# Shao-Group/aletsch

Measured on AMD Instinct MI355X. Metric: bundles/sec, higher is better.
Workload: dtype f64

## Files before the change

aletsch_amd/csrc/decomp_device.h:

```cpp
#pragma once
#include "decomp_common.h"
#ifdef ALD_EMU
#include <cstdio>
#include <cstdlib>
namespace ald { inline int32_t *emu_fail_line = nullptr; }
#endif

#ifndef ALD_CLASS_ID
#error "compile with -DALD_CLASS_ID=<0..13> (one translation unit per size class)"
#endif
#if defined(__HIP__) || defined(__clang__)
  #define ALD_UNROLL _Pragma("unroll")
#else
  #define ALD_UNROLL _Pragma("GCC unroll 16")
#endif
#define ALD_CAT2(a, b) a##b
#define ALD_CAT(a, b) ALD_CAT2(a, b)
#ifdef ALD_RAW_VARIANT
#define ALD_CLASS_NS ALD_CAT(ald_r, ALD_CLASS_ID)
#else
#define ALD_CLASS_NS ALD_CAT(ald_c, ALD_CLASS_ID)
#endif

namespace ALD_CLASS_NS {
using namespace ald;
#ifdef ALD_EMU_COUNT
static long g_cnt_router = 0, g_cnt_unsweep = 0, g_cnt_star[34] = {0}, g_cnt_rdeg[34] = {0}, g_cnt_build = 0, g_cnt_pre[3] = {0}, g_cnt_fix[8] = {0}, g_cnt_fix_declined = 0, g_cnt_x22[3] = {0}, g_cnt_x22s[5] = {0};
struct CntPrinter { ~CntPrinter() { if(g_cnt_unsweep) { fprintf(stderr, "[emu-count] class %d: unsplittable sweeps %ld router runs %ld (of which reach build(): %ld; prepared at level 0/1/2: %ld %ld %ld)\n", ALD_CLASS_ID, g_cnt_unsweep, g_cnt_router, g_cnt_build, g_cnt_pre[0], g_cnt_pre[1], g_cnt_pre[2]);
    fprintf(stderr, "[emu-count]   stars by fan size:"); for(int i = 0; i < 34; i++) if(g_cnt_star[i]) fprintf(stderr, " %d:%ld", i, g_cnt_star[i]); fprintf(stderr, "\n");
    fprintf(stderr, "[emu-count]   stars through the fixed-size form:"); for(int i = 0; i < 8; i++) if(g_cnt_fix[i]) fprintf(stderr, " %d:%ld", i, g_cnt_fix[i]); fprintf(stderr, " declined:%ld\n", g_cnt_fix_declined);
    fprintf(stderr, "[emu-count]   extends: %ld through the fixed 2x2 form: %ld declined: %ld\n", g_cnt_x22[2], g_cnt_x22[0], g_cnt_x22[1]);
    fprintf(stderr, "[emu-count]   fixed 2x2 form: strand to i' from o*: %ld to o' from i*: %ld to z from i*: %ld to z from o*: %ld insert_between acted: %ld\n", g_cnt_x22s[0], g_cnt_x22s[1], g_cnt_x22s[2], g_cnt_x22s[3], g_cnt_x22s[4]);
    fprintf(stderr, "[emu-count]   router runs by degree:"); for(int i = 0; i < 34; i++) if(g_cnt_rdeg[i]) fprintf(stderr, " %d:%ld", i, g_cnt_rdeg[i]); fprintf(stderr, "\n"); } } }; static CntPrinter g_cnt_printer;
#endif

enum { MAXV = ClassDims<ALD_CLASS_ID>::MAXV, MAXE = ClassDims<ALD_CLASS_ID>::MAXE, NW = ClassDims<ALD_CLASS_ID>::NW };
typedef uint16_t IDX;
static constexpr IDX NIL = (IDX)0xFFFF;
#if ALD_CLASS_ID == ALD_HUGE_CLASS
typedef uint32_t EID;
enum { EID_LIMIT = 0x7FFFFFF0 };
#else
typedef uint16_t EID;
enum { EID_LIMIT = 0xFFF0 };
#endif
typedef ColdLayoutT<MAXV, MAXE, NW, 0> CL;
#ifndef ALD_KEEP
  #define ALD_KEEP (ALD_CLASS_ID >= ALD_FIRST_GLOBAL_CLASS ? 1 : 0)
#endif
#ifndef ALD_KEEP_TRIV
  #define ALD_KEEP_TRIV ALD_KEEP
#endif
enum { LP = 16, ARENA_I = 96, ARENA_D = 48, SCR_I = 4 * LP + ARENA_I, SCR_D = 2 * LP + ARENA_D };

struct Hot {
    struct alignas(8) Link { IDX es, et, inx, onx; };
    struct alignas(16) EdgeHot { double w; Link lk; };
    EdgeHot  ed[MAXE];
    EID      eid[MAXE];
    struct alignas(8) VertexHot { IDX in_head, out_head, in_deg, out_deg; };
    VertexHot vx[MAXV];
    uint8_t  nz[MAXV];
    uint8_t  hflag[MAXE];
};
struct HotCtx {
    ALD_GLOBAL uint8_t *cold;
    ALD_GLOBAL const KernelArgs *args;
    double   ro_ratio;
    int32_t  ro_type, ro_degree, ro_npairs, tmp0;
    int32_t  ev_all;
#if ALD_KEEP
    uint32_t ev_dirty[(MAXV + 31) / 32];
  #if ALD_KEEP_TRIV
    int32_t  tv_all; uint32_t tv_dirty[(MAXV + 31) / 32];
  #endif
#endif
    int32_t  g, V0, gstrand;
    int32_t  nv, next_id, slot_hw, free_head, free_cnt, status, any_strand, hs_dirty, n_paths, n_iters, n_trace;
    uint32_t sp_used, hl_used; int32_t hl_n;
    int32_t  s_next;
    double   p_min_w, p_min_cov, p_ratio[8]; int32_t p_max_exons, p_trace_cap;
    int32_t  pw_lds, park_lds;
    int32_t  sinkp, special_linked;
    int32_t  maybe_triv;
    int32_t  maybe_broken;
    double   sw_best_r, sw_hit_r; int32_t sw_best_v, sw_hit, sw_vend, sw_dom_base; uint32_t sw_need_lo, sw_need_hi;
    int32_t  sw_ncand;
    int32_t  scr_i[SCR_I]; double scr_d[SCR_D];
#ifdef ALD_PROF
    unsigned long long prof[32];
#endif
};

#if ALD_CLASS_ID >= ALD_FIRST_GLOBAL_CLASS
#define ALD_MERGED_WALKS 1
#endif
#if defined(ALD_EMU)
static thread_local Hot g_H;
static thread_local HotCtx g_HC;
#define H g_H
#define HC g_HC
#elif ALD_CLASS_ID >= ALD_FIRST_GLOBAL_CLASS
__shared__ ALD_GLOBAL Hot *g_Hp;
__shared__ HotCtx g_HC;
#define H (*g_Hp)
#define HC g_HC
#define ALD_HOT_IN_SLAB 1
#else
__shared__ Hot g_H;
__shared__ HotCtx g_HC;
#define H g_H
#define HC g_HC
#endif

struct ColdVertex { double vw; int32_t lpos, rpos, vtype, v2v, memo, pad_; };
struct alignas(64) ColdEdge {
    double   med, eabd, econf, s0abd;
    uint64_t mask[NW];
    int32_t  mei, ecount, s0id;
    uint32_t sp_off, sp_len;
    uint8_t  estrand;
};
static_assert(sizeof(ColdVertex) == CL::VX_BYTES && sizeof(ColdEdge) == CL::ED_BYTES, "slab layout out of sync");
struct Cold {
    ALD_GLOBAL ColdVertex *vx;
    ALD_GLOBAL ColdEdge *ed;
    ALD_GLOBAL int32_t *sp_id; ALD_GLOBAL double *sp_abd;
    ALD_GLOBAL int32_t *hl, *hl_off, *hl_len, *hl_capk, *hl_cnt;
    ALD_GLOBAL int32_t *wi; ALD_GLOBAL double *wd;
    ALD_GLOBAL unsigned long long *po;
    static constexpr int32_t po_cap = CL::PO_CAP;
    static constexpr uint32_t sp_cap = CL::SP_CAP, hl_cap = CL::HL_CAP;
    static constexpr int32_t hl_maxlists = CL::HL_MAXLISTS, w_cap = CL::W_CAP;
};
ALD_INL Cold cold_view()
{
    ALD_GLOBAL uint8_t *b = HC.cold; Cold C;
    C.vx = (ALD_GLOBAL ColdVertex*)(b + CL::o_vx); C.ed = (ALD_GLOBAL ColdEdge*)(b + CL::o_ed);
    C.sp_id = (ALD_GLOBAL int32_t*)(b + CL::o_spid); C.sp_abd = (ALD_GLOBAL double*)(b + CL::o_spabd);
    C.hl = (ALD_GLOBAL int32_t*)(b + CL::o_hl); C.hl_off = (ALD_GLOBAL int32_t*)(b + CL::o_hloff); C.hl_len = (ALD_GLOBAL int32_t*)(b + CL::o_hllen);
    C.hl_capk = (ALD_GLOBAL int32_t*)(b + CL::o_hlcapk); C.hl_cnt = (ALD_GLOBAL int32_t*)(b + CL::o_hlcnt);
    C.wi = (ALD_GLOBAL int32_t*)(b + CL::o_wi); C.wd = (ALD_GLOBAL double*)(b + CL::o_wd);
    C.po = (ALD_GLOBAL unsigned long long*)(b + CL::o_po);
    return C;
}
#define COLD const Cold C = cold_view()

#if defined(ALD_PROF) && !defined(ALD_EMU)
  #define PROF_DECL unsigned long long prof_t_ = __builtin_readcyclecounter()
  #define PROF_ADD(k) do { unsigned long long t1_ = __builtin_readcyclecounter(); if(lane_id() == 0) HC.prof[k] += t1_ - prof_t_; prof_t_ = t1_; } while(0)
  #define PROF_RESET() (prof_t_ = __builtin_readcyclecounter())
#else
  #define PROF_DECL do {} while(0)
  #define PROF_ADD(k) do {} while(0)
  #define PROF_RESET() do {} while(0)
#endif
enum { PF_LOAD = 0, PF_BROKEN, PF_TRIV_EVAL, PF_TRIV_MUT, PF_SMALL_EVAL, PF_SMALL_MUT, PF_UNSPLIT, PF_COLLECT0, PF_G_BALANCE, PF_G_DP, PF_G_SPLITMERGE, PF_G_COLLECT, PF_FINISH,
       PF_T_BALANCE, PF_T_PAIRS, PF_T_SETUP, PF_T_MERGE_LOAD, PF_T_MERGE_ADD, PF_T_MERGE_ISECT, PF_T_MERGE_MASK, PF_T_MERGE_SUMS, PF_T_MERGE_KILL, PF_T_HS, PF_T_TAIL,
       PF_S5_DUP, PF_S5_BODY, PF_S5_RELINK, PF_S6_WALK, PF_S6_LINK, PF_S7, PF_SM_KILL, PF_SM_REEVAL, PF_COUNT };

ALD_INL void fail_(int st, int line)
{
#ifdef ALD_EMU
    if(HC.status == 0 && getenv("ALD_EMU_VERBOSE")) fprintf(stderr, "[emu] graph %d: status %d raised at decomp_device.h:%d\n", HC.g, st, line);
    if(HC.status == 0 && ald::emu_fail_line) ald::emu_fail_line[HC.g] = line;
#endif
    if(HC.status == 0) HC.status = st;
}
#define fail(st) fail_((st), __LINE__)
#define ALD_UNLIKELY(x) __builtin_expect(!!(x), 0)
ALD_FN void trace_emit(int code, int a, int b, double v)
{
    int cap = HC.p_trace_cap;
    ALD_GLOBAL const KernelArgs *A = HC.args;
    int k = HC.n_trace++;
    if(k < cap) { int64_t o = (int64_t)HC.g * cap + k; A->out.trace_codes[3 * o] = code; A->out.trace_codes[3 * o + 1] = a; A->out.trace_codes[3 * o + 2] = b; A->out.trace_vals[o] = v; }
}
#ifdef ALD_PROF
ALD_INL bool tracing_u() { return false; }
ALD_INL bool tracing() { return false; }
#else
ALD_INL bool tracing_u() { return uni(HC.p_trace_cap) > 0; }
ALD_INL bool tracing() { return HC.p_trace_cap > 0; }
#endif
ALD_INL void trace(int code, int a, int b, double v) { HC.n_iters++; if(tracing()) trace_emit(code, a, b, v); }
#ifndef ALD_NO_SEXT_LINKS
ALD_INL int slot_or_neg(IDX h) { return MAXE < 32768 ? (int)(int16_t)h : (h == NIL ? -1 : (int)h); }
#else
ALD_INL int slot_or_neg(IDX h) { return h == NIL ? -1 : (int)h; }
#endif
ALD_INL int u_first_in(int v) { return uni(slot_or_neg(H.vx[v].in_head)); }
ALD_INL int u_first_out(int v) { return uni(slot_or_neg(H.vx[v].out_head)); }
ALD_INL int u_next_in(int e) { return uni(slot_or_neg(H.ed[e].lk.inx)); }
ALD_INL int u_next_out(int e) { return uni(slot_or_neg(H.ed[e].lk.onx)); }
ALD_INL int first_in(int v) { return slot_or_neg(H.vx[v].in_head); }
ALD_INL int first_out(int v) { return slot_or_neg(H.vx[v].out_head); }
ALD_INL int next_in(int e) { return slot_or_neg(H.ed[e].lk.inx); }
ALD_INL int next_out(int e) { return slot_or_neg(H.ed[e].lk.onx); }
ALD_INL double in_weights(int v) { double w = 0; for(int e = first_in(v); e >= 0; e = next_in(e)) w += H.ed[e].w; return w; }
ALD_INL double out_weights(int v) { double w = 0; for(int e = first_out(v); e >= 0; e = next_out(e)) w += H.ed[e].w; return w; }

ALD_INL uint32_t tkey(uint32_t p) { return (int)p == HC.sinkp ? 0xFFFFu : p; }
ALD_INL int vlog(int p) { return p < HC.V0 - 1 ? p : (p == HC.sinkp ? HC.nv - 1 : p - 1); }
ALD_INL uint64_t lkw(int e) { return uni(*(const uint64_t*)&H.ed[e].lk); }
ALD_INL int lk_next(uint32_t f) { return slot_or_neg((IDX)f); }
ALD_INL void ev_mark(int v)
{
#if ALD_KEEP
  #ifdef ALD_EMU
    HC.ev_dirty[v >> 5] |= 1u << (v & 31);
    #if ALD_KEEP_TRIV
    HC.tv_dirty[v >> 5] |= 1u << (v & 31);
    #endif
  #else
    __hip_atomic_fetch_or(&HC.ev_dirty[v >> 5], 1u << (v & 31), __ATOMIC_RELAXED, __HIP_MEMORY_SCOPE_WAVEFRONT);
    #if ALD_KEEP_TRIV
    __hip_atomic_fetch_or(&HC.tv_dirty[v >> 5], 1u << (v & 31), __ATOMIC_RELAXED, __HIP_MEMORY_SCOPE_WAVEFRONT);
    #endif
  #endif
#else
    (void)v;
#endif
}
ALD_INL void star_tail_sync() { if(ALD_KEEP) wsync_mem(); else wsync(); }
ALD_INL void ev_mark_all()
{
#if ALD_KEEP
    HC.ev_all = 1;
    #if ALD_KEEP_TRIV
    HC.tv_all = 1;
    #endif
#endif
}
ALD_INL void ev_clear_marks(int vend)
{
#if ALD_KEEP
    const int words = (vend + 31) / 32;
    HC.ev_all = 0;
    for(int base = 0; base < words; base += ALD_WAVE) { const int k = base + lane_id(); HC.ev_dirty[k < words ? k : words - 1] = 0; }
#else
    (void)vend;
#endif
}
ALD_INL void tv_clear_marks(int nv_now)
{
#if ALD_KEEP && ALD_KEEP_TRIV
    const int words = (nv_now + 31) / 32;
    HC.tv_all = 0;
    for(int base = 0; base < words; base += ALD_WAVE) { const int k = base + lane_id(); HC.tv_dirty[k < words ? k : words - 1] = 0; }
#else
    (void)nv_now;
#endif
}
ALD_INL void ev_degree(int v, int before, int after, bool out)
{
#if ALD_KEEP
    ev_mark(v);
    if((before <= 1) == (after <= 1)) return;
    if(!HC.special_linked && (out ? v == 0 : v == HC.sinkp)) { ev_mark_all(); return; }
    int guard = MAXE;
    for(int e = out ? slot_or_neg(H.vx[v].out_head) : slot_or_neg(H.vx[v].in_head); e >= 0 && guard-- > 0; e = out ? slot_or_neg(H.ed[e].lk.onx) : slot_or_neg(H.ed[e].lk.inx))
        ev_mark(out ? (int)H.ed[e].lk.et : (int)H.ed[e].lk.es);
#else
    (void)v; (void)before; (void)after; (void)out;
#endif
}
ALD_INL void link_in(int v, int e)
{
    v = uni(v); e = uni(e);
    if(v == uni(HC.sinkp) && !uni(HC.special_linked)) { const int dg = uni((int)H.vx[v].in_deg); H.vx[v].in_deg = (IDX)(dg + 1); ev_degree(v, dg, dg + 1, false); return; }
    const uint32_t ks = uni(H.ed[e].lk.es), kid = uni(H.eid[e]);
    IDX *pp = &H.vx[v].in_head; IDX cur = *pp;
    for(int guard = MAXE; uni(cur != NIL) && guard > 0; guard--) {
        const uint64_t w = *(const uint64_t*)&H.ed[cur].lk; const uint32_t cs = (uint32_t)(w & 0xFFFF);
        bool stop = cs > ks; if(uni(cs == ks)) stop = H.eid[cur] > kid;
        if(uni(stop)) break;
        pp = &H.ed[cur].lk.inx; cur = (IDX)((w >> 32) & 0xFFFF);
    }
    H.ed[e].lk.inx = cur; *pp = (IDX)e;
    { const int dg = uni((int)H.vx[v].in_deg); H.vx[v].in_deg = (IDX)(dg + 1); ev_degree(v, dg, dg + 1, false); }
}
ALD_INL void link_out(int v, int e)
{
    v = uni(v); e = uni(e);
    if(v == 0 && !uni(HC.special_linked)) { const int dg = uni((int)H.vx[v].out_deg); H.vx[v].out_deg = (IDX)(dg + 1); ev_degree(v, dg, dg + 1, true); return; }
    const uint32_t sk = (uint32_t)uni(HC.sinkp);
    uint32_t kt = uni(H.ed[e].lk.et); const uint32_t kid = uni(H.eid[e]);
    if(kt == sk) kt = 0xFFFFu;
    IDX *pp = &H.vx[v].out_head; IDX cur = *pp;
    for(int guard = MAXE; uni(cur != NIL) && guard > 0; guard--) {
        const uint64_t w = *(const uint64_t*)&H.ed[cur].lk; uint32_t ct = (uint32_t)((w >> 16) & 0xFFFF); if(ct == sk) ct = 0xFFFFu;
        bool stop = ct > kt; if(uni(ct == kt)) stop = H.eid[cur] > kid;
        if(uni(stop)) break;
        pp = &H.ed[cur].lk.onx; cur = (IDX)(w >> 48);
    }
    H.ed[e].lk.onx = cur; *pp = (IDX)e;
    { const int dg = uni((int)H.vx[v].out_deg); H.vx[v].out_deg = (IDX)(dg + 1); ev_degree(v, dg, dg + 1, true); }
}
ALD_INL void link_out_after(int v, int e, int hint)
{
    v = uni(v); e = uni(e); hint = uni(hint);
    if(v == 0 && !uni(HC.special_linked)) { const int dg = uni((int)H.vx[v].out_deg); H.vx[v].out_deg = (IDX)(dg + 1); ev_degree(v, dg, dg + 1, true); return; }
    const uint32_t sk = (uint32_t)uni(HC.sinkp);
    uint32_t kt = uni(H.ed[e].lk.et); const uint32_t kid = uni(H.eid[e]);
    if(kt == sk) kt = 0xFFFFu;
    IDX *pp = &H.ed[hint].lk.onx; IDX cur = *pp;
    for(int guard = MAXE; uni(cur != NIL) && guard > 0; guard--) {
        const uint64_t w = *(const uint64_t*)&H.ed[cur].lk; uint32_t ct = (uint32_t)((w >> 16) & 0xFFFF); if(ct == sk) ct = 0xFFFFu;
        bool stop = ct > kt; if(uni(ct == kt)) stop = H.eid[cur] > kid;
        if(uni(stop)) break;
        pp = &H.ed[cur].lk.onx; cur = (IDX)(w >> 48);
    }
    H.ed[e].lk.onx = cur; *pp = (IDX)e;
    { const int dg = uni((int)H.vx[v].out_deg); H.vx[v].out_deg = (IDX)(dg + 1); ev_degree(v, dg, dg + 1, true); }
}
ALD_INL void unlink_in(int v, int e)
{
    v = uni(v); e = uni(e);
    if(v == uni(HC.sinkp) && !uni(HC.special_linked)) { const int dg = uni((int)H.vx[v].in_deg); H.vx[v].in_deg = (IDX)(dg - 1); ev_degree(v, dg, dg - 1, false); return; }
    IDX *pp = &H.vx[v].in_head; IDX cur = *pp; int guard = MAXE;
    while(uni((int)cur != e && cur != NIL) && guard-- > 0) { pp = &H.ed[cur].lk.inx; cur = *pp; }
    if(ALD_UNLIKELY(uni((int)cur != e))) { fail(ALD_ST_INVARIANT + ALD_INV_OTHER); return; }
    *pp = H.ed[e].lk.inx;
    { int dg = (int)uni(H.vx[v].in_deg) - 1; H.vx[v].in_deg = (IDX)dg; ev_degree(v, dg + 1, dg, false); if(dg <= 1) { HC.maybe_triv = 1; if(dg == 0) HC.maybe_broken = 1; } }
}
ALD_INL void unlink_out(int v, int e)
{
    v = uni(v); e = uni(e);
    if(v == 0 && !uni(HC.special_linked)) { const int dg = uni((int)H.vx[v].out_deg); H.vx[v].out_deg = (IDX)(dg - 1); ev_degree(v, dg, dg - 1, true); return; }
    IDX *pp = &H.vx[v].out_head; IDX cur = *pp; int guard = MAXE;
    while(uni((int)cur != e && cur != NIL) && guard-- > 0) { pp = &H.ed[cur].lk.onx; cur = *pp; }
    if(ALD_UNLIKELY(uni((int)cur != e))) { fail(ALD_ST_INVARIANT + ALD_INV_OTHER); return; }
    *pp = H.ed[e].lk.onx;
    { int dg = (int)uni(H.vx[v].out_deg) - 1; H.vx[v].out_deg = (IDX)dg; ev_degree(v, dg + 1, dg, true); if(dg <= 1) { HC.maybe_triv = 1; if(dg == 0) HC.maybe_broken = 1; } }
}
ALD_INL void relink_in(int v, int e, uint32_t ks)
{
    v = uni(v); e = uni(e);
    ev_mark(v);
    if(v == uni(HC.sinkp) && !uni(HC.special_linked)) return;
    int last = -1, pe = -1, ip = -1; bool seen = false, placed = false;
    int guard = MAXE;
    for(int cur = u_first_in(v); cur >= 0 && guard-- > 0; ) {
        uint64_t w = lkw(cur); int nx = lk_next((uint32_t)((w >> 32) & 0xFFFF));
        if(cur == e) { pe = last; seen = true; if(placed) break; }
        else { if(!placed && (uint32_t)(w & 0xFFFF) > ks) { ip = last; placed = true; if(seen) break; } last = cur; }
        cur = nx;
    }
    if(ALD_UNLIKELY(!seen)) { fail(ALD_ST_INVARIANT + ALD_INV_OTHER); return; }
    if(!placed) ip = last;
    if(ip == pe) return;
    IDX nxe = uni(H.ed[e].lk.inx);
    if(pe < 0) H.vx[v].in_head = nxe; else H.ed[pe].lk.inx = nxe;
    if(ip < 0) { H.ed[e].lk.inx = uni(H.vx[v].in_head); H.vx[v].in_head = (IDX)e; } else { H.ed[e].lk.inx = uni(H.ed[ip].lk.inx); H.ed[ip].lk.inx = (IDX)e; }
}
ALD_INL void relink_out(int v, int e, uint32_t kt)
{
    v = uni(v); e = uni(e);
    ev_mark(v);
    if(v == 0 && !uni(HC.special_linked)) return;
    const uint32_t sk = (uint32_t)uni(HC.sinkp);
    int last = -1, pe = -1, ip = -1; bool seen = false, placed = false;
    int guard = MAXE;
    for(int cur = u_first_out(v); cur >= 0 && guard-- > 0; ) {
        uint64_t w = lkw(cur); int nx = lk_next((uint32_t)(w >> 48));
        if(cur == e) { pe = last; seen = true; if(placed) break; }
        else { uint32_t ct = (uint32_t)((w >> 16) & 0xFFFF); if(ct == sk) ct = 0xFFFFu; if(!placed && ct > kt) { ip = last; placed = true; if(seen) break; } last = cur; }
        cur = nx;
    }
    if(ALD_UNLIKELY(!seen)) { fail(ALD_ST_INVARIANT + ALD_INV_OTHER); return; }
    if(!placed) ip = last;
    if(ip == pe) return;
    IDX nxe = uni(H.ed[e].lk.onx);
    if(pe < 0) H.vx[v].out_head = nxe; else H.ed[pe].lk.onx = nxe;
    if(ip < 0) { H.ed[e].lk.onx = uni(H.vx[v].out_head); H.vx[v].out_head = (IDX)e; } else { H.ed[e].lk.onx = uni(H.ed[ip].lk.onx); H.ed[ip].lk.onx = (IDX)e; }
}
ALD_INL void relink_in_lane(int v, int e, uint32_t ks)
{
    ev_mark(v);
    if(v == HC.sinkp && !HC.special_linked) return;
    int last = -1, pe = -1, ip = -1; bool seen = false, placed = false;
    int guard = MAXE;
    for(int cur = first_in(v); cur >= 0 && guard-- > 0; ) {
        const uint64_t w = *(const uint64_t*)&H.ed[cur].lk; const int nx = lk_next((uint32_t)((w >> 32) & 0xFFFF));
        if(cur == e) { pe = last; seen = true; if(placed) break; }
        else { if(!placed && (uint32_t)(w & 0xFFFF) > ks) { ip = last; placed = true; if(seen) break; } last = cur; }
        cur = nx;
    }
    if(ALD_UNLIKELY(!seen)) { fail(ALD_ST_INVARIANT + ALD_INV_OTHER); return; }
    if(!placed) ip = last;
    if(ip == pe) return;
    const IDX nxe = H.ed[e].lk.inx;
    if(pe < 0) H.vx[v].in_head = nxe; else H.ed[pe].lk.inx = nxe;
    if(ip < 0) { H.ed[e].lk.inx = H.vx[v].in_head; H.vx[v].in_head = (IDX)e; } else { H.ed[e].lk.inx = H.ed[ip].lk.inx; H.ed[ip].lk.inx = (IDX)e; }
}
ALD_INL void relink_out_lane(int v, int e, uint32_t kt)
{
    ev_mark(v);
    if(v == 0 && !HC.special_linked) return;
    const uint32_t sk = (uint32_t)HC.sinkp;
    int last = -1, pe = -1, ip = -1; bool seen = false, placed = false;
    int guard = MAXE;
    for(int cur = first_out(v); cur >= 0 && guard-- > 0; ) {
        const uint64_t w = *(const uint64_t*)&H.ed[cur].lk; const int nx = lk_next((uint32_t)(w >> 48));
        if(cur == e) { pe = last; seen = true; if(placed) break; }
        else { uint32_t ct = (uint32_t)((w >> 16) & 0xFFFF); if(ct == sk) ct = 0xFFFFu; if(!placed && ct > kt) { ip = last; placed = true; if(seen) break; } last = cur; }
        cur = nx;
    }
    if(ALD_UNLIKELY(!seen)) { fail(ALD_ST_INVARIANT + ALD_INV_OTHER); return; }
    if(!placed) ip = last;
    if(ip == pe) return;
    const IDX nxe = H.ed[e].lk.onx;
    if(pe < 0) H.vx[v].out_head = nxe; else H.ed[pe].lk.onx = nxe;
    if(ip < 0) { H.ed[e].lk.onx = H.vx[v].out_head; H.vx[v].out_head = (IDX)e; } else { H.ed[e].lk.onx = H.ed[ip].lk.onx; H.ed[ip].lk.onx = (IDX)e; }
}
ALD_INL void clear_vertex(int x)
{
    ev_mark(x);
#if defined(ALD_EMU)
    H.vx[x].in_head = NIL; H.vx[x].out_head = NIL; H.vx[x].in_deg = 0; H.vx[x].out_deg = 0; H.nz[x] = 0;
#else
    unsigned lo = 0xFFFFFFFFu, hi = 0u;
    asm volatile("" : "+v"(lo), "+v"(hi));
    static_assert(sizeof(Hot::VertexHot) == 8 && NIL == 0xFFFF, "vertex record layout");
    union { uint64_t u; Hot::VertexHot v; } z; z.u = ((uint64_t)hi << 32) | lo;
    H.vx[x] = z.v;
    H.nz[x] = 0;
#endif
}
ALD_INL int free_slots() { return uni(HC.free_cnt) + (MAXE - uni(HC.slot_hw)); }
ALD_INL int add_edge_i(int s, int t)
{
    s = uni(s); t = uni(t);
    int e; int fh = uni(HC.free_head), hw = uni(HC.slot_hw);
    if(fh >= 0) { e = fh; IDX nx = uni(H.ed[e].lk.onx); HC.free_head = nx == NIL ? -1 : (int)nx; HC.free_cnt--; }
    else if(hw < MAXE) { e = hw; HC.slot_hw = hw + 1; }
    else { fail(ALD_ST_CAPACITY); return -1; }
    int id = uni(HC.next_id); HC.next_id = id + 1;
    if(ALD_UNLIKELY(id >= EID_LIMIT)) { fail(ALD_ST_CAPACITY); return -1; }
    H.ed[e].lk.es = (IDX)s; H.ed[e].lk.et = (IDX)t; H.eid[e] = (EID)id; H.hflag[e] = 0; H.ed[e].w = 0;
    link_out(s, e); link_in(t, e);
    return e;
}
ALD_INL void kill_edge_i(int e)
{
    e = uni(e);
    unlink_out(uni(H.ed[e].lk.es), e); unlink_in(uni(H.ed[e].lk.et), e);
    H.ed[e].lk.es = NIL;
    { int fh = uni(HC.free_head); H.ed[e].lk.onx = fh < 0 ? NIL : (IDX)fh; HC.free_head = e; HC.free_cnt = uni(HC.free_cnt) + 1; }
}
ALD_INL void kill_edge_wave(int e)
{
    e = uni(e);
    const uint64_t w = *(const uint64_t*)&H.ed[e].lk;
    const bool special = HC.special_linked != 0; const int sinkp = HC.sinkp;
    for(int side = lane_id(); side < 2; side += ALD_WAVE) {
        const bool out = (side == 0);
        const int v = out ? (int)(w & 0xFFFF) : (int)((w >> 16) & 0xFFFF);
        const IDX nxe = out ? (IDX)(w >> 48) : (IDX)((w >> 32) & 0xFFFF);
        const bool counted = !special && (out ? v == 0 : v == sinkp);
        IDX *deg = out ? &H.vx[v].out_deg : &H.vx[v].in_deg;
        if(!counted) {
            IDX *pp = out ? &H.vx[v].out_head : &H.vx[v].in_head; IDX cur = *pp; int guard = MAXE;
            while((int)cur != e && cur != NIL && guard-- > 0) { pp = out ? &H.ed[cur].lk.onx : &H.ed[cur].lk.inx; cur = *pp; }
            if(ALD_UNLIKELY((int)cur != e)) { fail(ALD_ST_INVARIANT + ALD_INV_OTHER); continue; }
            *pp = nxe;
        }
        const int dg = (int)*deg - 1; *deg = (IDX)dg;
        ev_degree(v, dg + 1, dg, out);
        if(!counted && dg <= 1) { HC.maybe_triv = 1; if(dg == 0) HC.maybe_broken = 1; }
    }
    wsync();
    if(lane_id() == 0) {
        H.ed[e].lk.es = NIL;
        const int fh = uni(HC.free_head); H.ed[e].lk.onx = fh < 0 ? NIL : (IDX)fh; HC.free_head = e; HC.free_cnt = uni(HC.free_cnt) + 1;
    }
}
ALD_FN int add_edge(int s, int t) { return add_edge_i(uni(s), uni(t)); }
ALD_FN void kill_edge(int e) { kill_edge_i(uni(e)); }
ALD_FN void move_edge(int e, int x, int y)
{
    e = uni(e); x = uni(x); y = uni(y);
    unlink_out(uni(H.ed[e].lk.es), e); unlink_in(uni(H.ed[e].lk.et), e);
    H.ed[e].lk.es = (IDX)x; H.ed[e].lk.et = (IDX)y;
    link_out(x, e); link_in(y, e);
}

ALD_INL void strand_degree(int v, int vs[6])
{
    COLD;
    for(int k = 0; k < 6; k++) vs[k] = 0;
    for(int e = first_in(v); e >= 0; e = next_in(e)) vs[C.ed[e].estrand]++;
    for(int e = first_out(v); e >= 0; e = next_out(e)) vs[C.ed[e].estrand + 3]++;
}
ALD_INL bool mixed_strand_vertex(int v)
{
    if(!HC.any_strand) return false;
    int vs[6]; strand_degree(v, vs);
    return (vs[1] + vs[4] >= 1) && (vs[2] + vs[5] >= 1);
}
ALD_INL void borrow_edge_strand(const Cold &C, int e1, int e2) { int s2 = C.ed[e2].estrand; if(s2 == 0) return; C.ed[e1].estrand = (uint8_t)s2; }

ALD_FN bool intersect_samples(int e1, int e2, int z)
{
    e1 = uni(e1); e2 = uni(e2); z = uni(z);
    COLD;
    const uint32_t n1 = uni(C.ed[e1].sp_len), n2 = uni(C.ed[e2].sp_len);
    if(n1 == 1 && n2 == 1) {
        int a = uni(C.ed[e1].s0id), b = uni(C.ed[e2].s0id); double x = uni(C.ed[e1].s0abd), y = uni(C.ed[e2].s0abd);
        if(a == b) { double c = (y < x) ? y : x; C.ed[z].sp_off = 0; C.ed[z].sp_len = 1; C.ed[z].ecount = 1; C.ed[z].eabd = 0.0 + c; C.ed[z].s0id = a; C.ed[z].s0abd = c; }
        else { C.ed[z].sp_off = 0; C.ed[z].sp_len = 0; C.ed[z].ecount = 0; C.ed[z].eabd = 0; C.ed[z].s0id = 0; C.ed[z].s0abd = 0; }
        return true;
    }
    const uint32_t o1 = uni(C.ed[e1].sp_off), o2 = uni(C.ed[e2].sp_off);
    const int i1 = uni(C.ed[e1].s0id), i2 = uni(C.ed[e2].s0id); const double a1 = uni(C.ed[e1].s0abd), a2 = uni(C.ed[e2].s0abd);
    const uint32_t need = n1 < n2 ? n1 : n2;
    const uint32_t o = HC.sp_used;
    if(ALD_UNLIKELY(o + need > C.sp_cap)) { fail(ALD_ST_CAPACITY); return false; }
    uint32_t i = 0, j = 0, k = 0; double abd = 0; int first_id = 0; double first_abd = 0;
    while(i < n1 && j < n2) {
        int a = n1 == 1 ? i1 : uni(C.sp_id[o1 + i]), b = n2 == 1 ? i2 : uni(C.sp_id[o2 + j]);
        if(a < b) i++; else if(b < a) j++;
        else { double x = n1 == 1 ? a1 : uni(C.sp_abd[o1 + i]), y = n2 == 1 ? a2 : uni(C.sp_abd[o2 + j]); double c = (y < x) ? y : x;
               C.sp_id[o + k] = a; C.sp_abd[o + k] = c; abd += c; if(k == 0) { first_id = a; first_abd = c; } k++; i++; j++; }
    }
    C.ed[z].sp_len = k; C.ed[z].ecount = (int32_t)k; C.ed[z].eabd = abd; C.ed[z].s0id = first_id; C.ed[z].s0abd = first_abd;
    if(k >= 2) { C.ed[z].sp_off = o; HC.sp_used = o + k; } else C.ed[z].sp_off = 0;
    return true;
}
ALD_FN double common_abd(int e1, int e2)
{
    e1 = uni(e1); e2 = uni(e2);
    COLD;
    const uint32_t o1 = uni(C.ed[e1].sp_off), n1 = uni(C.ed[e1].sp_len), o2 = uni(C.ed[e2].sp_off), n2 = uni(C.ed[e2].sp_len);
    const int i1 = uni(C.ed[e1].s0id), i2 = uni(C.ed[e2].s0id); const double a1 = uni(C.ed[e1].s0abd), a2 = uni(C.ed[e2].s0abd);
    uint32_t i = 0, j = 0; double c = 0;
    while(i < n1 && j < n2) {
        int a = n1 == 1 ? i1 : uni(C.sp_id[o1 + i]), b = n2 == 1 ? i2 : uni(C.sp_id[o2 + j]);
        if(a < b) i++; else if(b < a) j++;
        else { double x = n1 == 1 ? a1 : uni(C.sp_abd[o1 + i]), y = n2 == 1 ? a2 : uni(C.sp_abd[o2 + j]); double mn = (y < x) ? y : x, mx = (x < y) ? y : x; c += 0.99 * mn + 0.01 * mx; i++; j++; }
    }
    return c;
}

ALD_FN void hs_refresh_flags()
{
    if(!HC.hs_dirty) return;
    HC.maybe_triv = 1; ev_mark_all();
    COLD;
    for(int e = 0; e < HC.slot_hw; e++) H.hflag[e] = 0;
    int nl = HC.hl_n;
    for(int k = 0; k < nl; k++) {
        ALD_GLOBAL int32_t *v = C.hl + uni(C.hl_off[k]); int n = uni(C.hl_len[k]);
        for(int i = 0; i < n; i++) {
            int e = v[i]; if(e < 0) continue;
            uint8_t f = HF_OCC;
            if(i >= 1 && v[i - 1] != -1) f |= HF_LEXT;
            if(i + 1 < n && v[i + 1] != -1) f |= HF_REXT;
            H.hflag[e] |= f;
        }
    }
    HC.hs_dirty = 0;
}
ALD_FN void hs_remove_lists(int e)
{
    e = uni(e);
    int nl = HC.hl_n;
    COLD;
    for(int k = 0; k < nl; k++) { ALD_GLOBAL int32_t *v = C.hl + uni(C.hl_off[k]); int n = uni(C.hl_len[k]); for(int i = 0; i < n; i++) if(v[i] == e) { v[i] = -1; HC.hs_dirty = 1; } }
}
ALD_FN void hs_replace1_lists(int x, int e)
{
    x = uni(x); e = uni(e);
    int nl = HC.hl_n;
    COLD;
    for(int k = 0; k < nl; k++) { ALD_GLOBAL int32_t *v = C.hl + uni(C.hl_off[k]); int n = uni(C.hl_len[k]); for(int i = 0; i < n; i++) if(v[i] == x) { v[i] = e; HC.hs_dirty = 1; } }
}
ALD_FN void hs_replace2_lists(int x, int y, int e)
{
    x = uni(x); y = uni(y); e = uni(e);
    int nl = HC.hl_n;
    COLD;
    for(int k = 0; k < nl; k++) {
        ALD_GLOBAL int32_t *v = C.hl + uni(C.hl_off[k]); int n = uni(C.hl_len[k]); int w = 0;
        for(int i = 0; i < n; i++) {
            if(i + 1 < n && v[i] == x && v[i + 1] == y) { v[w++] = e; i++; HC.hs_dirty = 1; }
            else v[w++] = v[i];
        }
        C.hl_len[k] = w;
    }
}
ALD_FN void hs_insert_between_lists(int x, int y, int e)
{
    x = uni(x); y = uni(y); e = uni(e);
    int nl = HC.hl_n;
    COLD;
    for(int k = 0; k < nl; k++) {
        int n = uni(C.hl_len[k]); ALD_GLOBAL int32_t *v = C.hl + uni(C.hl_off[k]);
        int cnt = 0;
        for(int i = 0; i + 1 < n; i++) if(v[i] == x && v[i + 1] == y) cnt++;
        if(cnt == 0) continue;
        if(n + cnt > uni(C.hl_capk[k])) {
            uint32_t ncap = (uint32_t)(n + cnt) * 2u + 4u, o = HC.hl_used;
            if(ALD_UNLIKELY(o + ncap > C.hl_cap)) { fail(ALD_ST_CAPACITY); return; }
            for(int i = 0; i < n; i++) C.hl[o + i] = v[i];
            HC.hl_used = o + ncap; C.hl_off[k] = (int32_t)o; C.hl_capk[k] = (int32_t)ncap; v = C.hl + o;
        }
        int w = n + cnt - 1;
        for(int i = n - 1; i >= 0; i--) {
            v[w--] = v[i];
            if(i >= 1 && v[i - 1] == x && v[i] == y) v[w--] = e;
        }
        C.hl_len[k] = n + cnt; HC.hs_dirty = 1;
    }
}
ALD_INL void hs_remove(int e) { if(uni(HC.hl_n) != 0) hs_remove_lists(e); }
ALD_INL void hs_replace1(int x, int e) { if(uni(HC.hl_n) != 0) hs_replace1_lists(x, e); }
ALD_INL void hs_replace2(int x, int y, int e) { if(uni(HC.hl_n) != 0) hs_replace2_lists(x, y, e); }
ALD_INL void hs_insert_between(int x, int y, int e) { if(uni(HC.hl_n) != 0) hs_insert_between_lists(x, y, e); }
ALD_FN bool hs_dominate(int e, int side)
{
    e = uni(e); side = uni(side);
    COLD;
    int nl = HC.hl_n;
    ALD_GLOBAL int32_t *x1 = C.wi, *x2 = C.wi + C.w_cap / 4; int n1 = 0, n2 = 0; const int cap = C.w_cap / 8;
    for(int k = 0; k < nl; k++) {
        ALD_GLOBAL int32_t *v = C.hl + uni(C.hl_off[k]); int n = uni(C.hl_len[k]);
        if(side == 2) {
            for(int i = 0; i + 1 < n; i++) {
                if(v[i] != e) continue;
                if(v[i + 1] == -1) continue;
                int a = v[i + 1], b = (i + 2 < n) ? v[i + 2] : -1;
                if(i == 0 || v[i - 1] == -1) { if(n1 < cap) { x1[2 * n1] = a; x1[2 * n1 + 1] = b; n1++; } else fail(ALD_ST_CAPACITY); }
                else { if(n2 + 2 <= cap) { x2[2 * n2] = a; x2[2 * n2 + 1] = -1; n2++; if(i + 2 < n) { x2[2 * n2] = a; x2[2 * n2 + 1] = b; n2++; } } else fail(ALD_ST_CAPACITY); }
            }
        } else {
            for(int i = 1; i < n; i++) {
                if(v[i] != e) continue;
                if(v[i - 1] == -1) continue;
                int a = v[i - 1], b = (i - 2 >= 0) ? v[i - 2] : -1;
                if(i == n - 1 || v[i + 1] == -1) { if(n1 < cap) { x1[2 * n1] = a; x1[2 * n1 + 1] = b; n1++; } else fail(ALD_ST_CAPACITY); }
                else { if(n2 + 2 <= cap) { x2[2 * n2] = a; x2[2 * n2 + 1] = -1; n2++; if(i - 2 >= 0) { x2[2 * n2] = a; x2[2 * n2 + 1] = b; n2++; } } else fail(ALD_ST_CAPACITY); }
            }
        }
    }
    for(int i = 0; i < n1; i++) { bool f = false; for(int j = 0; j < n2 && !f; j++) f = (x2[2 * j] == x1[2 * i] && x2[2 * j + 1] == x1[2 * i + 1]); if(!f) return false; }
    return true;
}

ALD_FN int split_edge(int ei, double w)
{
    ei = uni(ei); w = uni(w);
    if(ALD_UNLIKELY(!(w >= HC.p_min_w - kSMIN))) { fail(ALD_ST_INVARIANT + ALD_INV_WEIGHT); return -1; }
    double ww = uni(H.ed[ei].w);
    if(fabs(ww - w) <= kSMIN) return ei;
    int s = uni(H.ed[ei].lk.es), t = uni(H.ed[ei].lk.et);
    int p2 = add_edge(s, t);
    if(p2 < 0) return -1;
    COLD;
    double www = ww - w;
    double mw = HC.p_min_w;
    if(www <= mw) www = mw;
    H.ed[ei].w = www; H.ed[p2].w = w;
    C.ed[p2].estrand = uni(C.ed[ei].estrand); C.ed[p2].ecount = uni(C.ed[ei].ecount); C.ed[p2].eabd = uni(C.ed[ei].eabd); C.ed[p2].econf = uni(C.ed[ei].econf);
    C.ed[p2].sp_off = uni(C.ed[ei].sp_off); C.ed[p2].sp_len = uni(C.ed[ei].sp_len); C.ed[p2].s0id = uni(C.ed[ei].s0id); C.ed[p2].s0abd = uni(C.ed[ei].s0abd);
    for(int k = 0; k < NW; k++) C.ed[p2].mask[k] = uni(C.ed[ei].mask[k]);
    C.ed[p2].mei = uni(C.ed[ei].mei); C.ed[p2].med = uni(C.ed[ei].med) * w / ww;
    return p2;
}
ALD_INL int merge_adjacent_edges_i(int x, int y, double ww)
{
    const double mw = HC.p_min_w;
    if(ALD_UNLIKELY(!(ww >= mw - kSMIN))) { fail(ALD_ST_INVARIANT + ALD_INV_WEIGHT); return -1; }
    if(x < 0 || y < 0) return -1;
    if(H.ed[x].lk.et != uni(H.ed[y].lk.es)) { int t = x; x = y; y = t; }
    const int xs = uni(H.ed[x].lk.es), xt = uni(H.ed[x].lk.et), yt = uni(H.ed[y].lk.et);
    if((int)uni(H.ed[y].lk.es) != xt) return -1;
    PROF_DECL;
    COLD;
    const double wx = uni(H.ed[x].w), wy = uni(H.ed[y].w);
    const bool sx = !(fabs(wx - ww) <= kSMIN), sy = !(fabs(wy - ww) <= kSMIN);
    const double medx = uni(C.ed[x].med), medy = uni(C.ed[y].med), cx = uni(C.ed[x].econf), cy = uni(C.ed[y].econf), vwt = uni(C.vx[xt].vw);
    const int meix = uni(C.ed[x].mei), meiy = uni(C.ed[y].mei), cntx = uni(C.ed[x].ecount), cnty = uni(C.ed[y].ecount), lt = uni(C.vx[xt].lpos), rt = uni(C.vx[xt].rpos), ov = uni(C.vx[xt].v2v);
    const int stx = uni(C.ed[x].estrand), sty = uni(C.ed[y].estrand);
    if(ALD_UNLIKELY(uni(HC.next_id) >= EID_LIMIT)) { fail(ALD_ST_CAPACITY); return -1; }
    if(sx) { HC.next_id++; double r = wx - ww; if(r <= mw) r = mw; H.ed[x].w = r; }
    if(sy) { HC.next_id++; double r = wy - ww; if(r <= mw) r = mw; H.ed[y].w = r; }
    const double wx0 = sx ? ww : wx, wy0 = sy ? ww : wy;
    const double medx1 = sx ? medx * ww / wx : medx, medy1 = sy ? medy * ww / wy : medy;
    PROF_ADD(PF_T_MERGE_LOAD);
    int n = add_edge_i(xs, yt);
    PROF_ADD(PF_T_MERGE_ADD);
    if(n < 0) return -1;
    if(ALD_UNLIKELY(!(fabs(wx0 - wy0) <= kSMIN))) { fail(ALD_ST_INVARIANT + ALD_INV_MERGE_EQUAL); return -1; }
    H.ed[n].w = wx0 * 0.5 + wy0 * 0.5;
    if(ALD_UNLIKELY(!(cntx > 0 && cnty > 0))) { fail(ALD_ST_INVARIANT + ALD_INV_COUNT); return -1; }
    if(!intersect_samples(x, y, n)) return -1;
    PROF_ADD(PF_T_MERGE_ISECT);
    C.ed[n].econf = cx + cy;
    C.ed[n].estrand = (uint8_t)(sty != 0 ? sty : stx);
    for(int k = 0; k < NW; k++) C.ed[n].mask[k] = uni(C.ed[x].mask[k]) | uni(C.ed[y].mask[k]);
// ... 280 lines not shown
            if(m1 > m2) { if(A) fw[0] = fw[0] + m1 - m2; else wcen = wcen + m1 - m2; }
            else if(m1 < m2) { if(A) wcen = wcen + m2 - m1; else fw[0] = fw[0] + m2 - m1; }
            const double wc = wcen;
            for(int j = 0; j < n; j++) { double w2 = fw[j]; fw[j] = A ? (wc <= w2 ? wc : w2) : (w2 <= wc ? w2 : wc); }
        }
        int small = 0;
#ifndef ALD_STAR_NO_SMALL
        if(!bad && n <= STAR_SMALL) {
            small = 1;
            for(int i = 0; i < n; i++) { int k = i; const uint32_t id = uni(H.eid[fe[i]]); while(k > 0 && (uint32_t)uni(H.eid[fe[ord[k - 1]]]) > id) { ord[k] = ord[k - 1]; k--; } ord[k] = i; }
            double mdc = 0;
            for(int q = 0; q < n; q++) { inv[ord[q]] = q; const double w = fw[ord[q]]; if(ALD_UNLIKELY(!(w >= mw - kSMIN))) bad = ALD_ST_INVARIANT + ALD_INV_WEIGHT; mdc = (q == 0) ? w : mdc + w; }
            dctx[0] = mdc;
            for(int j = 0; j < n; j++) H.ed[fe[j]].w = fw[j];
        }
#endif
        ctx[SW_N] = n; ctx[SW_C] = c; ctx[SW_FAR] = A ? (int)uni(H.ed[c].lk.es) : (int)uni(H.ed[c].lk.et); ctx[SW_FAIL] = bad; ctx[SW_FAILQ] = -1; ctx[SW_SERIAL] = 0; ctx[SW_SMALL] = small;
    }
    wsync();
    const int n = uni(ctx[SW_N]), c = uni(ctx[SW_C]), far = uni(ctx[SW_FAR]);
#ifdef ALD_EMU_COUNT
    g_cnt_star[n < 33 ? n : 33]++;
#endif
    if(uni(ctx[SW_FAIL])) { if(lane == 0) fail(ctx[SW_FAIL]); wsync(); return; }
    PROF_ADD(PF_T_BALANCE);
    if(!uni(ctx[SW_SMALL])) {
    for(int j = lane; j < n; j += ALD_WAVE) {
        const uint32_t id = H.eid[fe[j]]; int r = 0;
        for(int k = 0; k < n; k++) r += ((uint32_t)H.eid[fe[k]] < id) ? 1 : 0;
        ord[r] = j; inv[j] = r;
    }
    wsync();
    if(lane == 0) {
        double mdc = 0; int bad = 0;
        for(int q = 0; q < n; q++) { double w = fw[ord[q]]; if(ALD_UNLIKELY(!(w >= mw - kSMIN))) bad = ALD_ST_INVARIANT + ALD_INV_WEIGHT; mdc = (q == 0) ? w : mdc + w; }
        dctx[0] = mdc;
        if(bad) ctx[SW_FAIL] = bad;
    }
    for(int j = lane; j < n; j += ALD_WAVE) H.ed[fe[j]].w = fw[j];
    wsync();
    if(uni(ctx[SW_FAIL])) { if(lane == 0) fail(ctx[SW_FAIL]); wsync(); return; }
    }
    PROF_ADD(PF_T_SETUP);
    const int id0 = uni(HC.next_id);
    const int meic = uni(meic_v), cntc = uni(cntc_v), stc = uni(stc_v), idc = uni(idc_v);
    const uint32_t nsc = uni(nsc_v);
    const int lt = uni(lt_v), rt = uni(rt_v), ov = uni(ov_v);
    #define SW_REPLAY(q_, wcur_, sc_, rem_, nid_, dead_) \
        double wcur_ = dctx[0], rem_ = 0; bool sc_ = false, dead_ = false; int nid_ = id0; \
        for(int qq = 0; qq <= (q_); qq++) { \
            if(qq > 0) { if(!sc_) dead_ = true; wcur_ = rem_; nid_ += 1; } \
            const double w2_ = fw[ord[qq]]; \
            sc_ = !(fabs(wcur_ - w2_) <= kSMIN); \
            rem_ = wcur_; if(sc_) { nid_ += 1; rem_ = wcur_ - w2_; if(rem_ <= mw) rem_ = mw; } \
        }
    double pf_med = 0, pf_conf = 0, pf_abd = 0; int pf_mei = 0, pf_st = 0, pf_cnt = 0, pf_id = 0; uint32_t pf_ns = 0; uint64_t pf_mask0 = 0;
    double rp_wcur = 0; bool rp_sc = false, rp_dead = false; int rp_nid = 0;
    for(int q = lane; q < n; q += ALD_WAVE) {
        SW_REPLAY(q, wcur, sc, rem, nid, dead);
        const int j = ord[q]; const double ww = fw[j];
        rp_wcur = wcur; rp_sc = sc; rp_dead = dead; rp_nid = nid;
#ifndef ALD_EMU
        { const int f = fe[j]; pf_med = C.ed[f].med; pf_conf = C.ed[f].econf; pf_abd = C.ed[f].s0abd; pf_mei = C.ed[f].mei; pf_st = C.ed[f].estrand; pf_cnt = C.ed[f].ecount;
          pf_id = C.ed[f].s0id; pf_ns = C.ed[f].sp_len; pf_mask0 = C.ed[f].mask[0]; }
#endif
        double sfan = 0;
        for(int k = 0; k < n; k++) if(inv[k] >= q) sfan += fw[k];
        double sc_side = 0; sc_side += sc ? rem : wcur; if(sc) sc_side += ww;
        sq[q] = A ? (sc_side + sfan) * 0.5 : (sfan + sc_side) * 0.5;
        oth[q] = A ? (int)H.ed[fe[j]].lk.et : (int)H.ed[fe[j]].lk.es;
    }
    wsync();
    PROF_ADD(PF_T_MERGE_LOAD);
    if(lane == 0) {
        double vwt = vw_early, wcur = dctx[0]; bool sc = false;
        for(int q = 0; q < n; q++) {
            const double ww = fw[ord[q]];
            sc = !(fabs(wcur - ww) <= kSMIN);
            const double wc0 = sc ? ww : wcur;
            const double r1 = A ? vwt * (wc0 + ww) * 0.5 / sq[q] : vwt * (ww + wc0) * 0.5 / sq[q];
            vwt = vwt - r1; sq[q] = r1;
            if(sc) { double rem = wcur - ww; if(rem <= mw) rem = mw; wcur = rem; }
        }
        C.vx[x].vw = vwt;
        ctx[SW_SERIAL] = sc ? 0 : 1;
    }
    wsync();
    PROF_ADD(PF_T_MERGE_SUMS);
    bool dup = false;
    for(int q = lane; q < n; q += ALD_WAVE) { const int o = oth[q]; for(int k = 0; k < q; k++) if(oth[k] == o) dup = true; }
    const bool any_dup = wballot(dup) != 0;
    bool multi = false, broken = false;
#ifdef ALD_PROF
    { unsigned long long t1_ = __builtin_readcyclecounter(); if(lane_id() == 0) HC.prof[PF_S5_DUP] += t1_ - prof_t_; }
    unsigned long long prof_s5_ = __builtin_readcyclecounter();
#endif
    for(int q = lane; q < n; q += ALD_WAVE) {
#ifdef ALD_EMU
        SW_REPLAY(q, wcur, sc, rem, nid, dead);
        (void)rem;
#else
        const double wcur = rp_wcur; const bool sc = rp_sc, dead = rp_dead; const int nid = rp_nid;
#endif
        const int j = ord[q], f = fe[j]; const double ww = fw[j];
        const double wc0 = sc ? ww : wcur;
        const double medc1 = sc ? medc * ww / wcur : medc;
        const double r1 = sq[q];
#ifdef ALD_EMU
        pf_med = C.ed[f].med; pf_conf = C.ed[f].econf; pf_abd = C.ed[f].s0abd; pf_mei = C.ed[f].mei; pf_st = C.ed[f].estrand; pf_cnt = C.ed[f].ecount;
        pf_id = C.ed[f].s0id; pf_ns = C.ed[f].sp_len; pf_mask0 = C.ed[f].mask[0];
#endif
        const double medf = pf_med, cf = pf_conf;
        const int meif = pf_mei, stf = pf_st, cntf = pf_cnt;
        const uint32_t nsf = pf_ns; const int idf = pf_id; const double abf = pf_abd;
        {
            int code = 0;
            if(dead) code = ALD_ST_INVARIANT + ALD_INV_DEGREE;
            else if(nid - (sc ? 1 : 0) >= EID_LIMIT) code = ALD_ST_CAPACITY;
            else if(!(cntc > 0 && cntf > 0)) code = ALD_ST_INVARIANT + ALD_INV_COUNT;
            inv[q] = code; if(ALD_UNLIKELY(code)) broken = true;
        }
        if(nsc == 1 && nsf == 1) {
            if(idf == idc) { const double xa = A ? abc : abf, ya = A ? abf : abc; const double mn = (ya < xa) ? ya : xa; C.ed[f].sp_off = 0; C.ed[f].ecount = 1; C.ed[f].eabd = 0.0 + mn; C.ed[f].s0abd = mn; }
            else { C.ed[f].sp_off = 0; C.ed[f].sp_len = 0; C.ed[f].ecount = 0; C.ed[f].eabd = 0; C.ed[f].s0id = 0; C.ed[f].s0abd = 0; }
        } else multi = true;
        C.ed[f].econf = A ? cc + cf : cf + cc;
        { const int sty = A ? stf : stc, stx = A ? stc : stf; C.ed[f].estrand = (uint8_t)(sty != 0 ? sty : stx); }
        for(int k = 0; k < NW; k++) { uint64_t mk = (NW <= 2 ? cmask_pf[NW <= 2 ? k : 0] : C.ed[c].mask[k]) | (k == 0 ? pf_mask0 : C.ed[f].mask[k]); if(ov >= 0 && (ov >> 6) == k) mk |= (1ull << (ov & 63)); C.ed[f].mask[k] = mk; }
        const int mi = A ? rt - lt + meic + meif : rt - lt + meif + meic;
        C.ed[f].med = A ? mi * r1 + medc1 + medf : mi * r1 + medf + medc1; C.ed[f].mei = mi;
        H.eid[f] = (EID)nid; H.ed[f].w = A ? wc0 * 0.5 + ww * 0.5 : ww * 0.5 + wc0 * 0.5;
        if(A) H.ed[f].lk.es = (IDX)far; else H.ed[f].lk.et = (IDX)far;
#ifdef ALD_PROF
        { unsigned long long t1_ = __builtin_readcyclecounter(); if(lane_id() == 0) HC.prof[PF_S5_BODY] += t1_ - prof_s5_; prof_s5_ = t1_; }
#endif
        if(!any_dup) { if(A) relink_in_lane(oth[q], f, (uint32_t)far); else relink_out_lane(oth[q], f, tkey((uint32_t)far)); }
#ifdef ALD_PROF
        { unsigned long long t1_ = __builtin_readcyclecounter(); if(lane_id() == 0) HC.prof[PF_S5_RELINK] += t1_ - prof_s5_; prof_s5_ = t1_; }
#endif
    }
    const bool any_multi = wballot(multi) != 0;
    if(ALD_UNLIKELY(wballot(broken) != 0)) {
        wsync();
        if(lane == 0) for(int q = 0; q < n; q++) if(inv[q]) {
            int code = inv[q];
            if(code == ALD_ST_INVARIANT + ALD_INV_COUNT) for(int qq = 0; qq <= q; qq++) if(!(fw[ord[qq]] <= DBL_MAX)) code = ALD_ST_INVARIANT + ALD_INV_MERGE_EQUAL;
            fail(code); break;
        }
        wsync();
        return;
    }
    const bool counted = A ? (far == 0 && !uni(HC.special_linked)) : (far == (int)uni(HC.sinkp) && !uni(HC.special_linked));
    const bool consumed = uni(ctx[SW_SERIAL]) != 0;
    if(lane == 0 && consumed) { if(A) unlink_out(far, c); else unlink_in(far, c); }
    wsync();
    PROF_ADD(PF_T_MERGE_MASK);
    if(ALD_UNLIKELY(!consumed)) { if(lane == 0) fail(ALD_ST_INVARIANT + (!(dctx[0] <= DBL_MAX) ? ALD_INV_MERGE_EQUAL : ALD_INV_DEGREE)); wsync(); return; }
    int32_t *pred = inv, *succ = (int32_t*)sq, *srt = (int32_t*)sq + STAR_MAX;
    if(!counted) {
        for(int q = lane; q < n; q += ALD_WAVE) {
            const uint32_t key = A ? tkey((uint32_t)oth[q]) : (uint32_t)oth[q];
            int last = -1, cur = A ? first_out(far) : first_in(far), guard = MAXE;
            while(cur >= 0 && guard-- > 0) {
                const uint64_t w = *(const uint64_t*)&H.ed[cur].lk;
                const uint32_t kc = A ? tkey((uint32_t)((w >> 16) & 0xFFFF)) : (uint32_t)(w & 0xFFFF);
                if(kc > key) break;
                last = cur; cur = A ? lk_next((uint32_t)(w >> 48)) : lk_next((uint32_t)((w >> 32) & 0xFFFF));
            }
            int r = 0;
            for(int k = 0; k < n; k++) { const uint32_t kk = A ? tkey((uint32_t)oth[k]) : (uint32_t)oth[k]; r += (kk < key || (kk == key && k < q)) ? 1 : 0; }
            pred[q] = last; succ[q] = cur; srt[r] = q;
        }
        wsync();
#ifdef ALD_PROF
        { unsigned long long t1_ = __builtin_readcyclecounter(); if(lane_id() == 0) HC.prof[PF_S6_WALK] += t1_ - prof_t_; }
#endif
        for(int r = lane; r < n; r += ALD_WAVE) {
            const int q = srt[r], f = fe[ord[q]];
            const bool first_of_gap = (r == 0) || pred[srt[r - 1]] != pred[q], last_of_gap = (r + 1 >= n) || pred[srt[r + 1]] != pred[q];
            const IDX nx = last_of_gap ? (succ[q] < 0 ? NIL : (IDX)succ[q]) : (IDX)fe[ord[srt[r + 1]]];
            if(A) H.ed[f].lk.onx = nx; else H.ed[f].lk.inx = nx;
            if(first_of_gap) { if(pred[q] < 0) { if(A) H.vx[far].out_head = (IDX)f; else H.vx[far].in_head = (IDX)f; } else { if(A) H.ed[pred[q]].lk.onx = (IDX)f; else H.ed[pred[q]].lk.inx = (IDX)f; } }
        }
    }
    star_tail_sync();
#ifdef ALD_PROF
    unsigned long long prof_s7_ = __builtin_readcyclecounter();
#endif
    if(lane == 0) {
        { const int dg = A ? (int)uni(H.vx[far].out_deg) : (int)uni(H.vx[far].in_deg); if(A) H.vx[far].out_deg = (IDX)(dg + n); else H.vx[far].in_deg = (IDX)(dg + n); ev_degree(far, dg, dg + n, A); }
        if(any_dup || any_multi || uni(HC.hl_n) != 0) for(int q = 0; q < n; q++) {
            const int f = fe[ord[q]];
            if(any_dup) { if(A) relink_in(oth[q], f, (uint32_t)far); else relink_out(oth[q], f, tkey((uint32_t)far)); }
            if(any_multi) { const uint32_t nsf = uni(C.ed[f].sp_len); if(!(nsc == 1 && nsf == 1)) { if(!(A ? intersect_samples(c, f, f) : intersect_samples(f, c, f))) break; } }
            if(A) hs_replace2(c, f, f); else hs_replace2(f, c, f);
            if(n == 1) hs_replace1(c, f);
        }
        HC.next_id = (int)uni(H.eid[fe[ord[n - 1]]]) + 1;
        if(n >= 2) hs_remove(c);
        H.ed[c].lk.es = NIL; H.hflag[c] = 0;
        { int fh = uni(HC.free_head); H.ed[c].lk.onx = fh < 0 ? NIL : (IDX)fh; HC.free_head = c; HC.free_cnt = uni(HC.free_cnt) + 1; }
        clear_vertex(x);
    }
    wsync();
#ifdef ALD_PROF
    { unsigned long long t1_ = __builtin_readcyclecounter(); if(lane_id() == 0) HC.prof[PF_S7] += t1_ - prof_s7_; }
#endif
    PROF_ADD(PF_T_MERGE_ADD);
#if defined(ALD_PROF) && defined(ALD_PROF_STAR_BY_SIZE)
    { unsigned long long t1_ = __builtin_readcyclecounter(); if(lane_id() == 0) HC.prof[n == 1 ? PF_T_PAIRS : n == 2 ? PF_T_MERGE_ISECT : n == 3 ? PF_T_MERGE_KILL : n == 4 ? PF_S6_LINK : PF_FINISH] += t1_ - prof_star0_; }
#endif
    #undef SW_REPLAY
}
ALD_INL void star_wave_in(int x) { star_wave_body<true>(uni(x)); }
ALD_INL void star_wave_out(int x) { star_wave_body<false>(uni(x)); }
#ifndef ALD_EMU
template<bool A> ALD_INL void star_reg(int x)
{
    COLD;
    PROF_DECL;
    const int lane = lane_id();
    const double mw = HC.p_min_w;
#if defined(ALD_PROF) && defined(ALD_PROF_STAR_BY_SIZE)
    const unsigned long long prof_star0_ = __builtin_readcyclecounter();
#endif
    const Hot::VertexHot vrx = H.vx[x];
    const int c = uni(slot_or_neg(A ? vrx.in_head : vrx.out_head));
    const int n = uni((int)(A ? vrx.out_deg : vrx.in_deg));
    int f = c;
    { int e = uni(slot_or_neg(A ? vrx.out_head : vrx.in_head));
      for(int k = 0; k < n && e >= 0; k++) { if(lane == k) f = e; e = A ? u_next_out(e) : u_next_in(e); } }
    const bool act = lane < n;
    const double w0 = H.ed[f].w; const uint64_t lw = *(const uint64_t*)&H.ed[f].lk; const int id = (int)H.eid[f];
    const int oth = A ? (int)((lw >> 16) & 0xFFFF) : (int)(lw & 0xFFFF);
    const uint64_t lwc = lkw(c);
    const int far = A ? (int)(lwc & 0xFFFF) : (int)((lwc >> 16) & 0xFFFF);
    double wcen = H.ed[c].w;
    bool badw = !(wcen >= mw - kSMIN) || wballot(act && !(w0 >= mw - kSMIN)) != 0;
    double sfan0 = 0;
    for(int k = 0; k < n; k++) sfan0 += wread(w0, k);
    double fw;
    {
        double scen0 = 0; scen0 += wcen;
        const double w_in = A ? scen0 : sfan0, w_out = A ? sfan0 : scen0;
        const double bw = sqrt(w_in * w_out);
        const double r_in = bw / w_in, r_out = bw / w_out;
        double m_cen = 0, m_fan = 0;
        { double wy = wcen * (A ? r_in : r_out); if(wy < mw) { m_cen += mw - wy; wy = mw; } wcen = wy; }
        fw = w0 * (A ? r_out : r_in);
        const bool clamped = act && fw < mw; const double deficit = mw - fw;
        if(clamped) fw = mw;
        { uint64_t m = wballot(clamped); while(m) { const int l = ffs64(m); m &= m - 1; m_fan += wread(deficit, l); } }
        const double m1 = A ? m_cen : m_fan, m2 = A ? m_fan : m_cen;
        if(m1 > m2) { if(A) { if(lane == 0) fw = fw + m1 - m2; } else wcen = wcen + m1 - m2; }
        else if(m1 < m2) { if(A) wcen = wcen + m2 - m1; else { if(lane == 0) fw = fw + m2 - m1; } }
        const double wc = wcen;
        fw = A ? (wc <= fw ? wc : fw) : (fw <= wc ? fw : wc);
    }
    PROF_ADD(PF_T_BALANCE);
    int inv = 0;
    for(int k = 0; k < n; k++) { const int idk = wread(id, k); inv += ((uint32_t)idk < (uint32_t)id) ? 1 : 0; }
    double mdc = 0;
    for(int q = 0; q < n; q++) {
        const int src = ffs64(wballot(act && inv == q));
        const double pw = wread(fw, src < 0 ? 0 : src);
        if(!(pw >= mw - kSMIN)) badw = true;
        mdc = (q == 0) ? pw : mdc + pw;
    }
    if(ALD_UNLIKELY(uni(badw))) { if(lane == 0) fail(ALD_ST_INVARIANT + ALD_INV_WEIGHT); wsync(); return; }
    PROF_ADD(PF_T_SETUP);
    const double medc = C.ed[c].med, cc = C.ed[c].econf, abc = C.ed[c].s0abd, vw0 = C.vx[x].vw;
    const int meic_v = C.ed[c].mei, cntc_v = C.ed[c].ecount, stc_v = C.ed[c].estrand, idc_v = C.ed[c].s0id;
    const uint32_t nsc_v = C.ed[c].sp_len;
    const int lt_v = C.vx[x].lpos, rt_v = C.vx[x].rpos, ov_v = C.vx[x].v2v;
    uint64_t cmask_pf[NW <= 2 ? NW : 1];
    if(NW <= 2) for(int k = 0; k < NW; k++) cmask_pf[k] = C.ed[c].mask[k];
    const double pf_med = C.ed[f].med, pf_conf = C.ed[f].econf, pf_abd = C.ed[f].s0abd;
    const int pf_mei = C.ed[f].mei, pf_st = C.ed[f].estrand, pf_cnt = C.ed[f].ecount, pf_id = C.ed[f].s0id;
    const uint32_t pf_ns = C.ed[f].sp_len; const uint64_t pf_mask0 = C.ed[f].mask[0];
    double mysfan = 0;
    for(int k = 0; k < n; k++) { const double fwk = wread(fw, k); const int invk = wread(inv, k); if(invk >= inv) mysfan += fwk; }
    const int id0 = uni(HC.next_id);
    double vwt = vw0, wcur = mdc, rem = 0; bool sc = false; int nid = id0;
    int failq = -1, failcode = 0;
    double my_wcur = 0, my_r1 = 0; bool my_sc = false; int my_nid = 0;
    for(int q = 0; q < n; q++) {
        const int src0 = ffs64(wballot(act && inv == q)), src = src0 < 0 ? 0 : src0;
        const double ww = wread(fw, src);
        if(q > 0) { if(!sc && failq < 0) { failq = q; failcode = ALD_ST_INVARIANT + ALD_INV_DEGREE; } wcur = rem; nid += 1; }
        sc = uni(!(fabs(wcur - ww) <= kSMIN));
        rem = wcur; if(sc) { nid += 1; rem = wcur - ww; if(rem <= mw) rem = mw; }
        if(failq < 0 && nid - (sc ? 1 : 0) >= EID_LIMIT) { failq = q; failcode = ALD_ST_CAPACITY; }
        const double sfan = wread(mysfan, src);
        double sc_side = 0; sc_side += sc ? rem : wcur; if(sc) sc_side += ww;
        const double sum = A ? (sc_side + sfan) * 0.5 : (sfan + sc_side) * 0.5;
        const double wc0 = sc ? ww : wcur;
        const double r1 = A ? vwt * (wc0 + ww) * 0.5 / sum : vwt * (ww + wc0) * 0.5 / sum;
        vwt = vwt - r1;
        if(lane == src) { my_wcur = wcur; my_sc = sc; my_nid = nid; my_r1 = r1; }
    }
    const bool consumed = !sc;
    const int nid_last = nid;
    PROF_ADD(PF_T_MERGE_SUMS);
    const int meic = uni(meic_v), cntc = uni(cntc_v), stc = uni(stc_v), idc = uni(idc_v);
    const uint32_t nsc = uni(nsc_v);
    const int lt = uni(lt_v), rt = uni(rt_v), ov = uni(ov_v);
    {
        int cq = -1;
        if(!(cntc > 0)) cq = 0;
        else { uint64_t m = wballot(act && !(pf_cnt > 0)); while(m) { const int l = ffs64(m); m &= m - 1; const int ql = wread(inv, l); if(cq < 0 || ql < cq) cq = ql; } }
        int code = 0;
        if(failq >= 0 && (cq < 0 || failq <= cq)) code = failcode; else if(cq >= 0) code = ALD_ST_INVARIANT + ALD_INV_COUNT;
        if(ALD_UNLIKELY(code != 0)) {
            if(code == ALD_ST_INVARIANT + ALD_INV_COUNT && !(rem <= DBL_MAX)) {
                for(int q = 0; q <= cq; q++) { const int s0 = ffs64(wballot(act && inv == q)); const double pw = wread(fw, s0 < 0 ? 0 : s0); if(!(pw <= DBL_MAX)) code = ALD_ST_INVARIANT + ALD_INV_MERGE_EQUAL; }
            }
            if(lane == 0) { C.vx[x].vw = vwt; fail(code); } wsync(); return;
        }
    }
    if(lane == 0) C.vx[x].vw = vwt;
    if(ALD_UNLIKELY(!consumed)) { if(lane == 0) fail(ALD_ST_INVARIANT + (!(rem <= DBL_MAX) ? ALD_INV_MERGE_EQUAL : ALD_INV_DEGREE)); wsync(); return; }
    bool dup = false;
    for(int k = 0; k < n; k++) { const int othk = wread(oth, k); if(act && lane != k && othk == oth) dup = true; }
    const bool any_dup = wballot(dup) != 0;
    int32_t *fem = (int32_t*)HC.scr_i, *othm = fem + STAR_MAX, *pred = fem + 2 * STAR_MAX, *succ = fem + 3 * STAR_MAX, *srt = (int32_t*)HC.scr_d;
    bool multi = false;
    if(act) {
        const double ww = fw, wc0 = my_sc ? ww : my_wcur;
        const double medc1 = my_sc ? medc * ww / my_wcur : medc;
        if(nsc == 1 && pf_ns == 1) {
            if(pf_id == idc) { const double xa = A ? abc : pf_abd, ya = A ? pf_abd : abc; const double mn = (ya < xa) ? ya : xa; C.ed[f].sp_off = 0; C.ed[f].ecount = 1; C.ed[f].eabd = 0.0 + mn; C.ed[f].s0abd = mn; }
            else { C.ed[f].sp_off = 0; C.ed[f].sp_len = 0; C.ed[f].ecount = 0; C.ed[f].eabd = 0; C.ed[f].s0id = 0; C.ed[f].s0abd = 0; }
        } else multi = true;
        C.ed[f].econf = A ? cc + pf_conf : pf_conf + cc;
        { const int sty = A ? pf_st : stc, stx = A ? stc : pf_st; C.ed[f].estrand = (uint8_t)(sty != 0 ? sty : stx); }
        for(int k = 0; k < NW; k++) { uint64_t mk = (NW <= 2 ? cmask_pf[NW <= 2 ? k : 0] : C.ed[c].mask[k]) | (k == 0 ? pf_mask0 : C.ed[f].mask[k]); if(ov >= 0 && (ov >> 6) == k) mk |= (1ull << (ov & 63)); C.ed[f].mask[k] = mk; }
        const int mi = A ? rt - lt + meic + pf_mei : rt - lt + pf_mei + meic;
        C.ed[f].med = A ? mi * my_r1 + medc1 + pf_med : mi * my_r1 + pf_med + medc1; C.ed[f].mei = mi;
        H.eid[f] = (EID)my_nid; H.ed[f].w = A ? wc0 * 0.5 + ww * 0.5 : ww * 0.5 + wc0 * 0.5;
        if(A) H.ed[f].lk.es = (IDX)far; else H.ed[f].lk.et = (IDX)far;
        if(!any_dup) { if(A) relink_in_lane(oth, f, (uint32_t)far); else relink_out_lane(oth, f, tkey((uint32_t)far)); }
        fem[inv] = f; othm[inv] = oth;
    }
    const bool any_multi = wballot(multi) != 0;
    PROF_ADD(PF_T_MERGE_LOAD);
    const bool counted = A ? (far == 0 && !uni(HC.special_linked)) : (far == (int)uni(HC.sinkp) && !uni(HC.special_linked));
    if(lane == 0) { if(A) unlink_out(far, c); else unlink_in(far, c); }
    wsync();
    PROF_ADD(PF_T_MERGE_MASK);
    if(!counted) {
        const uint32_t key = A ? tkey((uint32_t)oth) : (uint32_t)oth;
        int r = 0;
        for(int k = 0; k < n; k++) { const uint32_t kk = (uint32_t)wread((int)key, k); const int invk = wread(inv, k); r += (kk < key || (kk == key && invk < inv)) ? 1 : 0; }
        if(act) {
            int last = -1, cur = A ? first_out(far) : first_in(far), guard = MAXE;
            while(cur >= 0 && guard-- > 0) {
                const uint64_t w = *(const uint64_t*)&H.ed[cur].lk;
                const uint32_t kc = A ? tkey((uint32_t)((w >> 16) & 0xFFFF)) : (uint32_t)(w & 0xFFFF);
                if(kc > key) break;
                last = cur; cur = A ? lk_next((uint32_t)(w >> 48)) : lk_next((uint32_t)((w >> 32) & 0xFFFF));
            }
            pred[inv] = last; succ[inv] = cur; srt[r] = inv;
        }
        wsync();
#if defined(ALD_PROF) && !defined(ALD_PROF_STAR_BY_SIZE)
        PROF_ADD(PF_S6_WALK);
#endif
        for(int r2 = lane; r2 < n; r2 += ALD_WAVE) {
            const int q = srt[r2], fq = fem[q];
            const bool first_of_gap = (r2 == 0) || pred[srt[r2 - 1]] != pred[q], last_of_gap = (r2 + 1 >= n) || pred[srt[r2 + 1]] != pred[q];
            const IDX nx = last_of_gap ? (succ[q] < 0 ? NIL : (IDX)succ[q]) : (IDX)fem[srt[r2 + 1]];
            if(A) H.ed[fq].lk.onx = nx; else H.ed[fq].lk.inx = nx;
            if(first_of_gap) { if(pred[q] < 0) { if(A) H.vx[far].out_head = (IDX)fq; else H.vx[far].in_head = (IDX)fq; } else { if(A) H.ed[pred[q]].lk.onx = (IDX)fq; else H.ed[pred[q]].lk.inx = (IDX)fq; } }
        }
    }
    star_tail_sync();
#if defined(ALD_PROF) && !defined(ALD_PROF_STAR_BY_SIZE)
    PROF_ADD(PF_S6_LINK);
#endif
    if(lane == 0) {
        { const int dg = A ? (int)uni(H.vx[far].out_deg) : (int)uni(H.vx[far].in_deg); if(A) H.vx[far].out_deg = (IDX)(dg + n); else H.vx[far].in_deg = (IDX)(dg + n); ev_degree(far, dg, dg + n, A); }
        if(any_dup || any_multi || uni(HC.hl_n) != 0) for(int q = 0; q < n; q++) {
            const int fq = fem[q];
            if(any_dup) { if(A) relink_in(othm[q], fq, (uint32_t)far); else relink_out(othm[q], fq, tkey((uint32_t)far)); }
            if(any_multi) { const uint32_t nsf = uni(C.ed[fq].sp_len); if(!(nsc == 1 && nsf == 1)) { if(!(A ? intersect_samples(c, fq, fq) : intersect_samples(fq, c, fq))) break; } }
            if(A) hs_replace2(c, fq, fq); else hs_replace2(fq, c, fq);
            if(n == 1) hs_replace1(c, fq);
        }
        HC.next_id = nid_last + 1;
        if(n >= 2) hs_remove(c);
        H.ed[c].lk.es = NIL; H.hflag[c] = 0;
        { int fh = uni(HC.free_head); H.ed[c].lk.onx = fh < 0 ? NIL : (IDX)fh; HC.free_head = c; HC.free_cnt = uni(HC.free_cnt) + 1; }
        clear_vertex(x);
    }
    wsync();
    PROF_ADD(PF_T_MERGE_ADD);
#if defined(ALD_PROF) && defined(ALD_PROF_STAR_BY_SIZE)
    { unsigned long long t1_ = __builtin_readcyclecounter(); if(lane_id() == 0) HC.prof[n == 1 ? PF_T_PAIRS : n == 2 ? PF_T_MERGE_ISECT : n == 3 ? PF_T_MERGE_KILL : n == 4 ? PF_S6_LINK : PF_FINISH] += t1_ - prof_star0_; }
#endif
}
#endif
#ifndef ALD_STARFIX_MAX
  #if ((ALD_CLASS_ID >= 2 && ALD_CLASS_ID <= 9) || ALD_CLASS_ID == 11 || ALD_CLASS_ID == 12) && !defined(ALD_STARFIX_ROOMY_OFF)
    #define ALD_STARFIX_MAX 4
  #else
    #define ALD_STARFIX_MAX 2
  #endif
#endif
template<int K, int N, class T> struct PickFrom { ALD_INL T get(const T (&a)[N], int i, T v) { return PickFrom<K + 1, N, T>::get(a, i, i == K ? a[K] : v); } };
template<int N, class T> struct PickFrom<N, N, T> { ALD_INL T get(const T (&)[N], int, T v) { return v; } };
template<int N, class T> ALD_INL T pick(const T (&a)[N], int i) { return PickFrom<1, N, T>::get(a, i, a[0]); }
#ifdef ALD_STARFIX_CALL
template<bool A, int N> ALD_FN bool star_fixed(int x)
#else
template<bool A, int N> ALD_INL bool star_fixed(int x)
#endif
{
    COLD;
    PROF_DECL;
    const int lane = lane_id();
    const double mw = HC.p_min_w;
    const Hot::VertexHot vrx = H.vx[x];
    const int c = uni(slot_or_neg(A ? vrx.in_head : vrx.out_head));
    int bad = (c < 0) ? 1 : 0;
    const int cs = c >= 0 ? c : 0;
    int fe[N], oth[N]; double fw[N]; uint32_t id[N];
    {
        int e = slot_or_neg(A ? vrx.out_head : vrx.in_head);
        ALD_UNROLL for(int k = 0; k < N; k++) {
            if(e < 0) bad = 1;
            const int es = e >= 0 ? e : 0;
            const double w = H.ed[es].w; const uint64_t lw = *(const uint64_t*)&H.ed[es].lk;
            fe[k] = es; fw[k] = w; id[k] = H.eid[es];
            oth[k] = A ? (int)((lw >> 16) & 0xFFFF) : (int)(lw & 0xFFFF);
            e = A ? lk_next((uint32_t)(lw >> 48)) : lk_next((uint32_t)((lw >> 32) & 0xFFFF));
        }
        if(e >= 0) bad = 1;
    }
    const uint64_t lwc = *(const uint64_t*)&H.ed[cs].lk;
    const int far = uni(A ? (int)(lwc & 0xFFFF) : (int)((lwc >> 16) & 0xFFFF));
    const int c_next = A ? lk_next((uint32_t)(lwc >> 48)) : lk_next((uint32_t)((lwc >> 32) & 0xFFFF));
    bool dupf = false;
    ALD_UNROLL for(int k = 0; k < N; k++) { ALD_UNROLL for(int k2 = 0; k2 < N; k2++) if(k2 < k && oth[k] == oth[k2]) dupf = true; }
    dupf = uni(dupf);
    double wcen = H.ed[cs].w;
    if(!(wcen >= mw - kSMIN)) bad = 1;
    double sfan0 = 0;
    ALD_UNROLL for(int k = 0; k < N; k++) { if(!(fw[k] >= mw - kSMIN)) bad = 1; sfan0 += fw[k]; }
    {
        double scen0 = 0; scen0 += wcen;
        const double w_in = A ? scen0 : sfan0, w_out = A ? sfan0 : scen0;
        const double bw = sqrt(w_in * w_out);
        const double r_in = bw / w_in, r_out = bw / w_out;
        double m_cen = 0, m_fan = 0;
        { double wy = wcen * (A ? r_in : r_out); if(wy < mw) { m_cen += mw - wy; wy = mw; } wcen = wy; }
        ALD_UNROLL for(int k = 0; k < N; k++) { double wy = fw[k] * (A ? r_out : r_in); if(wy < mw) { m_fan += mw - wy; wy = mw; } fw[k] = wy; }
        const double m1 = A ? m_cen : m_fan, m2 = A ? m_fan : m_cen;
        if(m1 > m2) { if(A) fw[0] = fw[0] + m1 - m2; else wcen = wcen + m1 - m2; }
        else if(m1 < m2) { if(A) wcen = wcen + m2 - m1; else fw[0] = fw[0] + m2 - m1; }
        const double wc = wcen;
        ALD_UNROLL for(int k = 0; k < N; k++) { const double w2 = fw[k]; fw[k] = A ? (wc <= w2 ? wc : w2) : (w2 <= wc ? w2 : wc); }
    }
    const double medc = C.ed[cs].med, cc = C.ed[cs].econf, abc = C.ed[cs].s0abd, vw0 = C.vx[x].vw;
    const int meic_v = C.ed[cs].mei, cntc_v = C.ed[cs].ecount, stc_v = C.ed[cs].estrand, idc_v = C.ed[cs].s0id;
    const uint32_t nsc_v = C.ed[cs].sp_len;
    const int lt_v = C.vx[x].lpos, rt_v = C.vx[x].rpos, ov_v = C.vx[x].v2v;
    uint64_t cmask_pf[NW <= 2 ? NW : 1];
    if(NW <= 2) { ALD_UNROLL for(int k = 0; k < (NW <= 2 ? NW : 1); k++) cmask_pf[k] = C.ed[cs].mask[k]; }
#ifndef ALD_EMU
    double pf_med, pf_conf, pf_abd; int pf_mei, pf_st, pf_cnt, pf_id; uint32_t pf_ns; uint64_t pf_mask0;
    { const int f = pick<N>(fe, lane < N ? lane : 0); pf_med = C.ed[f].med; pf_conf = C.ed[f].econf; pf_abd = C.ed[f].s0abd; pf_mei = C.ed[f].mei; pf_st = C.ed[f].estrand;
      pf_cnt = C.ed[f].ecount; pf_id = C.ed[f].s0id; pf_ns = C.ed[f].sp_len; pf_mask0 = C.ed[f].mask[0]; }
#endif
    int inv[N];
    ALD_UNROLL for(int k = 0; k < N; k++) { int r = 0; ALD_UNROLL for(int k2 = 0; k2 < N; k2++) r += (id[k2] < id[k]) ? 1 : 0; inv[k] = r; }
    double pw[N]; int fq[N], oq[N];
    ALD_UNROLL for(int q = 0; q < N; q++) { double w = fw[0]; int f = fe[0], o = oth[0]; ALD_UNROLL for(int k = 1; k < N; k++) if(inv[k] == q) { w = fw[k]; f = fe[k]; o = oth[k]; } pw[q] = w; fq[q] = f; oq[q] = o; }
    double mdc = 0;
    ALD_UNROLL for(int q = 0; q < N; q++) { if(!(pw[q] >= mw - kSMIN)) bad = 1; mdc = (q == 0) ? pw[q] : mdc + pw[q]; }
    const int id0 = uni(HC.next_id);
    double wcur_q[N], rem_q[N]; int sc_q[N], nid_q[N];
    {
        double wcur = mdc, rem = 0; bool sc = false; int nid = id0;
        ALD_UNROLL for(int q = 0; q < N; q++) {
            if(q > 0) { if(!sc) bad = 1; wcur = rem; nid += 1; }
            sc = !(fabs(wcur - pw[q]) <= kSMIN);
            rem = wcur; if(sc) { nid += 1; rem = wcur - pw[q]; if(rem <= mw) rem = mw; }
            if(nid - (sc ? 1 : 0) >= EID_LIMIT) bad = 1;
            wcur_q[q] = wcur; rem_q[q] = rem; sc_q[q] = sc ? 1 : 0; nid_q[q] = nid;
        }
        if(sc) bad = 1;
    }
    double r1_q[N]; double vwt = vw0;
    ALD_UNROLL for(int q = 0; q < N; q++) {
        double sfan = 0;
        ALD_UNROLL for(int k = 0; k < N; k++) if(inv[k] >= q) sfan += fw[k];
        const bool sc = sc_q[q] != 0; const double ww = pw[q], wcur = wcur_q[q];
        double sc_side = 0; sc_side += sc ? rem_q[q] : wcur; if(sc) sc_side += ww;
        const double sum = A ? (sc_side + sfan) * 0.5 : (sfan + sc_side) * 0.5;
        const double wc0 = sc ? ww : wcur;
        const double r1 = A ? vwt * (wc0 + ww) * 0.5 / sum : vwt * (ww + wc0) * 0.5 / sum;
        vwt = vwt - r1; r1_q[q] = r1;
    }
    const bool counted = uni(A ? (far == 0 && !HC.special_linked) : (far == HC.sinkp && !HC.special_linked));
    uint32_t key[N]; int pred[N], succ[N]; int pc = -1;
    ALD_UNROLL for(int k = 0; k < N; k++) { key[k] = A ? tkey((uint32_t)oth[k]) : (uint32_t)oth[k]; pred[k] = -1; succ[k] = -1; }
    if(!counted) {
        int placed[N]; ALD_UNROLL for(int k = 0; k < N; k++) placed[k] = 0;
        bool seen_c = false; int last = -1, guard = MAXE;
        int cur = A ? first_out(far) : first_in(far);
        while(uni(cur >= 0) && guard-- > 0) {
            const uint64_t w = *(const uint64_t*)&H.ed[cur].lk;
            const int nx = A ? lk_next((uint32_t)(w >> 48)) : lk_next((uint32_t)((w >> 32) & 0xFFFF));
            if(cur == cs) { pc = last; seen_c = true; }
            else {
                const uint32_t kc = A ? tkey((uint32_t)((w >> 16) & 0xFFFF)) : (uint32_t)(w & 0xFFFF);
                ALD_UNROLL for(int k = 0; k < N; k++) if(!placed[k] && kc > key[k]) { placed[k] = 1; pred[k] = last; succ[k] = cur; }
                last = cur;
            }
            bool all = seen_c; ALD_UNROLL for(int k = 0; k < N; k++) all = all && placed[k];
            if(uni(all)) break;
            cur = nx;
        }
        ALD_UNROLL for(int k = 0; k < N; k++) if(!placed[k]) pred[k] = last;
        if(!seen_c || guard <= 0) bad = 1;
    }
    const int meic = uni(meic_v), cntc = uni(cntc_v), stc = uni(stc_v), idc = uni(idc_v), lt = uni(lt_v), rt = uni(rt_v), ov = uni(ov_v);
    const uint32_t nsc = uni(nsc_v);
    if(!(cntc > 0)) bad = 1;
    {
        bool cnt_bad = false;
#ifdef ALD_EMU
        for(int k = 0; k < N; k++) if(!(C.ed[fe[k]].ecount > 0)) cnt_bad = true;
#else
        cnt_bad = lane < N && !(pf_cnt > 0);
#endif
#ifdef ALD_EMU_COUNT
        if(cnt_bad || bad) g_cnt_fix_declined++; else { g_cnt_star[N]++; g_cnt_fix[N]++; }
#endif
        if(wballot(cnt_bad) != 0 || uni(bad) != 0) return false;
    }
    bool multi = false;
    for(int j = lane; j < N; j += ALD_WAVE) {
        const int q = pick<N>(inv, j), f = pick<N>(fe, j), o = pick<N>(oth, j);
        const double ww = pick<N>(fw, j), wcur = pick<N>(wcur_q, q), r1 = pick<N>(r1_q, q);
        const bool sc = pick<N>(sc_q, q) != 0; const int nid = pick<N>(nid_q, q);
        const double wc0 = sc ? ww : wcur;
        const double medc1 = sc ? medc * ww / wcur : medc;
#ifdef ALD_EMU
        const double pf_med = C.ed[f].med, pf_conf = C.ed[f].econf, pf_abd = C.ed[f].s0abd; const int pf_mei = C.ed[f].mei, pf_st = C.ed[f].estrand, pf_id = C.ed[f].s0id;
        const uint32_t pf_ns = C.ed[f].sp_len; const uint64_t pf_mask0 = C.ed[f].mask[0];
#endif
        if(nsc == 1 && pf_ns == 1) {
            if(pf_id == idc) { const double xa = A ? abc : pf_abd, ya = A ? pf_abd : abc; const double mn = (ya < xa) ? ya : xa; C.ed[f].sp_off = 0; C.ed[f].ecount = 1; C.ed[f].eabd = 0.0 + mn; C.ed[f].s0abd = mn; }
            else { C.ed[f].sp_off = 0; C.ed[f].sp_len = 0; C.ed[f].ecount = 0; C.ed[f].eabd = 0; C.ed[f].s0id = 0; C.ed[f].s0abd = 0; }
        } else multi = true;
        C.ed[f].econf = A ? cc + pf_conf : pf_conf + cc;
        { const int sty = A ? pf_st : stc, stx = A ? stc : pf_st; C.ed[f].estrand = (uint8_t)(sty != 0 ? sty : stx); }
        for(int k = 0; k < NW; k++) { uint64_t mk = (NW <= 2 ? cmask_pf[NW <= 2 ? k : 0] : C.ed[cs].mask[k]) | (k == 0 ? pf_mask0 : C.ed[f].mask[k]); if(ov >= 0 && (ov >> 6) == k) mk |= (1ull << (ov & 63)); C.ed[f].mask[k] = mk; }
        const int mi = A ? rt - lt + meic + pf_mei : rt - lt + pf_mei + meic;
        C.ed[f].med = A ? mi * r1 + medc1 + pf_med : mi * r1 + pf_med + medc1; C.ed[f].mei = mi;
        H.eid[f] = (EID)nid; H.ed[f].w = A ? wc0 * 0.5 + ww * 0.5 : ww * 0.5 + wc0 * 0.5;
        if(A) H.ed[f].lk.es = (IDX)far; else H.ed[f].lk.et = (IDX)far;
        if(!dupf) { if(A) relink_in_lane(o, f, (uint32_t)far); else relink_out_lane(o, f, tkey((uint32_t)far)); }
        if(!counted) {
            const uint32_t kj = pick<N>(key, j); const int pj = pick<N>(pred, j), sj = pick<N>(succ, j);
            int rj = 0; ALD_UNROLL for(int k = 0; k < N; k++) rj += (key[k] < kj || (key[k] == kj && inv[k] < q)) ? 1 : 0;
            int prv_pred = -2, nxt_pred = -2, nxt_f = -1;
            ALD_UNROLL for(int k = 0; k < N; k++) { int rk = 0; ALD_UNROLL for(int k2 = 0; k2 < N; k2++) rk += (key[k2] < key[k] || (key[k2] == key[k] && inv[k2] < inv[k])) ? 1 : 0;
                if(rk == rj - 1) prv_pred = pred[k]; if(rk == rj + 1) { nxt_pred = pred[k]; nxt_f = fe[k]; } }
            const bool first_of_gap = prv_pred != pj, last_of_gap = nxt_pred != pj;
            const IDX nx = last_of_gap ? (sj < 0 ? NIL : (IDX)sj) : (IDX)nxt_f;
            if(A) H.ed[f].lk.onx = nx; else H.ed[f].lk.inx = nx;
            if(first_of_gap) { if(pj < 0) { if(A) H.vx[far].out_head = (IDX)f; else H.vx[far].in_head = (IDX)f; } else { if(A) H.ed[pj].lk.onx = (IDX)f; else H.ed[pj].lk.inx = (IDX)f; } }
        }
    }
    const bool any_multi = wballot(multi) != 0;
    star_tail_sync();
    if(lane == 0) {
        IDX *deg = A ? &H.vx[far].out_deg : &H.vx[far].in_deg;
        const int dg = (int)*deg - 1;
        if(!counted) {
            bool taken = false; ALD_UNROLL for(int k = 0; k < N; k++) if(pred[k] == pc) taken = true;
            if(!taken) { const IDX nx = c_next < 0 ? NIL : (IDX)c_next; if(pc < 0) { if(A) H.vx[far].out_head = nx; else H.vx[far].in_head = nx; } else { if(A) H.ed[pc].lk.onx = nx; else H.ed[pc].lk.inx = nx; } }
            if(dg <= 1) { HC.maybe_triv = 1; if(dg == 0) HC.maybe_broken = 1; }
        }
        *deg = (IDX)(dg + N); ev_degree(far, dg + 1, dg + N, A);
        C.vx[x].vw = vwt;
        if(dupf || any_multi || uni(HC.hl_n) != 0) {
            ALD_UNROLL for(int q = 0; q < N; q++) {
                const int f = uni(fq[q]);
                if(dupf) { if(A) relink_in(uni(oq[q]), f, (uint32_t)far); else relink_out(uni(oq[q]), f, tkey((uint32_t)far)); }
                if(any_multi) { const uint32_t nsf = uni(C.ed[f].sp_len); if(!(uni(nsc) == 1 && nsf == 1)) { if(!(A ? intersect_samples(cs, f, f) : intersect_samples(f, cs, f))) break; } }
                if(A) hs_replace2(cs, f, f); else hs_replace2(f, cs, f);
            }
        }
        HC.next_id = nid_q[N - 1] + 1;
        hs_remove(cs);
        H.ed[cs].lk.es = NIL; H.hflag[cs] = 0;
        { int fh = uni(HC.free_head); H.ed[cs].lk.onx = fh < 0 ? NIL : (IDX)fh; HC.free_head = cs; HC.free_cnt = uni(HC.free_cnt) + 1; }
        clear_vertex(x);
    }
    wsync();
    PROF_ADD(PF_T_MERGE_ADD);
    return true;
}
template<bool A> ALD_INL bool star_fixed_any(int x, int n)
{
#if ALD_STARFIX_MAX >= 2
    if(n == 2) return uni(star_fixed<A, 2>(x));
#endif
#if ALD_STARFIX_MAX >= 3
    if(n == 3) return uni(star_fixed<A, 3>(x));
#endif
#if ALD_STARFIX_MAX >= 4
    if(n == 4) return uni(star_fixed<A, 4>(x));
#endif
    return false;
}
ALD_INL void decompose_trivial_vertex_wave(int x)
{
    x = uni(x);
    const int nin = uni(H.vx[x].in_deg), nout = uni(H.vx[x].out_deg);
#if ALD_STARFIX_MAX >= 2
    if(nin == 1 && nout >= 2 && nout <= ALD_STARFIX_MAX) { if(star_fixed_any<true>(x, nout)) return; }
    else if(nout == 1 && nin >= 2 && nin <= ALD_STARFIX_MAX) { if(star_fixed_any<false>(x, nin)) return; }
#endif
#ifdef ALD_STAR_SEQ_MAX
    if((nin == 1 && nout >= 1 && nout <= ALD_STAR_SEQ_MAX) || (nout == 1 && nin >= 1 && nin <= ALD_STAR_SEQ_MAX)) { if(lane_id() == 0) decompose_trivial_vertex(x); wsync(); return; }
#endif
#if !defined(ALD_EMU) && !defined(ALD_STAR_SCRATCH_FORM)
    if(nin == 1 && nout >= 1 && nout <= STAR_MAX) star_reg<true>(x);
    else if(nout == 1 && nin >= 1 && nin <= STAR_MAX) star_reg<false>(x);
#else
    if(nin == 1 && nout >= 1 && nout <= STAR_MAX) star_wave_in(x);
    else if(nout == 1 && nin >= 1 && nin <= STAR_MAX) star_wave_out(x);
#endif
    else { if(lane_id() == 0) decompose_trivial_vertex(x); wsync(); }
}

template<bool SMALL> ALD_INL void decompose_vertex_extend_body(int root, int n)
{
    COLD;
    const Pairs P = pairs_at(SMALL, false);
    int32_t *a = P.a, *b = P.b; double *w = P.w;
    const int deg = (int)uni(H.vx[root].in_deg) + (int)uni(H.vx[root].out_deg);
    const Arena AR = arena_at(SMALL);
    if(ALD_UNLIKELY(4 * deg > AR.cap_i || deg > AR.cap_d || deg > C.w_cap / 16)) { fail(ALD_ST_CAPACITY); return; }
    int nloc = 0; int32_t *loc_e = AR.i;
    for(int e = u_first_in(root); e >= 0; e = u_next_in(e)) { loc_e[nloc++] = e; }
    int nin = nloc;
    for(int e = u_first_out(root); e >= 0; e = u_next_out(e)) { loc_e[nloc++] = e; }
    int32_t *mdeg = AR.i + deg;
    int32_t *evx = AR.i + 2 * deg;
    double *mweight = AR.d;
    for(int i = 0; i < nloc; i++) { mdeg[i] = 0; evx[i] = -1; mweight[i] = 0; }
    const double mw = HC.p_min_w;
    double total_weight = 0;
    for(int i = 0; i < n; i++) {
        if(ALD_UNLIKELY(!(w[i] >= mw - kSMIN))) { fail(ALD_ST_INVARIANT + ALD_INV_WEIGHT); return; }
        int u1 = PLOC(a[i]), u2 = PLOC(b[i]);
        total_weight += w[i];
        if(mdeg[u1] == 0) mweight[u1] = w[i]; else mweight[u1] += w[i];
        if(mdeg[u2] == 0) mweight[u2] = w[i]; else mweight[u2] += w[i];
        mdeg[u1]++; mdeg[u2]++;
    }
    int rlen = uni(C.vx[root].rpos) - uni(C.vx[root].lpos);
    double vertex_weight = uni(C.vx[root].vw) * rlen;
    for(int i = 0; i < nloc; i++) mweight[i] = mweight[i] / total_weight * vertex_weight;
    int m = HC.nv, nn = m;
    for(int i = 0; i < nloc; i++) { if(ALD_UNLIKELY(mdeg[i] == 0)) { fail(ALD_ST_INVARIANT + ALD_INV_OTHER); return; } if(mdeg[i] >= 2) evx[i] = nn++; }
    int newedges = 0;
    for(int i = 0; i < n; i++) { int u1 = PLOC(a[i]), u2 = PLOC(b[i]); if(mdeg[u1] == 1 && mdeg[u2] == 1) evx[u1] = nn++; else if(mdeg[u1] >= 2 && mdeg[u2] >= 2) newedges++; }
    if(ALD_UNLIKELY(nn > MAXV || free_slots() < newedges)) { fail(ALD_ST_CAPACITY); return; }
    HC.maybe_broken = 1; HC.maybe_triv = 1; ev_mark_all();
    for(int i = m; i < nn; i++) { H.vx[i].in_head = NIL; H.vx[i].out_head = NIL; H.vx[i].in_deg = 0; H.vx[i].out_deg = 0; H.nz[i] = 1; C.vx[i].vw = 0; C.vx[i].lpos = 0; C.vx[i].rpos = 0; C.vx[i].vtype = -1; C.vx[i].v2v = -1; }
    HC.nv = nn;
    for(int i = 0; i < nin; i++) {
        int k = evx[i]; if(k < 0) continue; int e = loc_e[i];
        int p = uni(C.vx[uni(H.ed[e].lk.es)].rpos);
        move_edge(e, uni(H.ed[e].lk.es), k); C.vx[k].lpos = p; C.vx[k].rpos = p; C.vx[k].vtype = -1; C.vx[k].vw = 0; C.vx[k].v2v = -2;
    }
    for(int i = nin; i < nloc; i++) {
        int k = evx[i]; if(k < 0) continue; int e = loc_e[i];
        int p = uni(C.vx[uni(H.ed[e].lk.et)].lpos);
        move_edge(e, k, uni(H.ed[e].lk.et)); C.vx[k].lpos = p; C.vx[k].rpos = p; C.vx[k].vtype = -1; C.vx[k].vw = 0; C.vx[k].v2v = -2;
    }
    int rv = uni(C.vx[root].v2v);
    for(int i = 0; i < n; i++) {
        int e1 = PSLOT(a[i]), e2 = PSLOT(b[i]); int u1 = PLOC(a[i]), u2 = PLOC(b[i]); double ww = w[i];
        if(mdeg[u1] == 1 && mdeg[u2] >= 2) {
            borrow_edge_strand(C, e1, e2);
            move_edge(e1, uni(H.ed[e1].lk.es), evx[u2]);
            if(rv >= 0) C.ed[e1].mask[(rv >> 6)] |= (1ull << (rv & 63));
            C.ed[e1].med += mweight[u1]; C.ed[e1].mei += rlen;
        } else if(mdeg[u2] == 1) {
            if(ALD_UNLIKELY(evx[u1] < 0)) { fail(ALD_ST_INVARIANT + ALD_INV_OTHER); return; }
            borrow_edge_strand(C, e2, e1);
            move_edge(e2, evx[u1], uni(H.ed[e2].lk.et));
            if(rv >= 0) C.ed[e2].mask[(rv >> 6)] |= (1ull << (rv & 63));
            C.ed[e2].med += mweight[u2]; C.ed[e2].mei += rlen;
        } else {
            int z = add_edge(evx[u1], evx[u2]);
            if(z < 0) return;
            H.ed[z].w = ww;
            if(ALD_UNLIKELY(!(C.ed[e1].ecount > 0 && uni(C.ed[e2].ecount) > 0))) { fail(ALD_ST_INVARIANT + ALD_INV_COUNT); return; }
            if(!intersect_samples(e1, e2, z)) return;
            if(ALD_UNLIKELY(C.ed[z].ecount <= 0)) { fail(ALD_ST_INVARIANT + ALD_INV_COUNT); return; }
            C.ed[z].econf = 0; C.ed[z].estrand = 0;
            for(int k = 0; k < NW; k++) C.ed[z].mask[k] = 0;
            if(rv >= 0) C.ed[z].mask[(rv >> 6)] |= (1ull << (rv & 63));
            C.ed[z].med = ww / total_weight * vertex_weight; C.ed[z].mei = rlen;
            borrow_edge_strand(C, z, e1); borrow_edge_strand(C, z, e2);
            hs_insert_between(e1, e2, z);
            if(HC.status) return;
        }
    }
    if(ALD_UNLIKELY(H.vx[root].in_deg != 0 || uni(H.vx[root].out_deg) != 0)) { fail(ALD_ST_INVARIANT + ALD_INV_DEGREE); return; }
    H.nz[root] = 0;
    double jump = HC.p_ratio[7];
    if(jump > 1.0) {
        int32_t *order = (int32_t*)(C.wi + 3 * (C.w_cap / 8)); int no = 0;
        for(int part = 0; part < 2; part++) {
            int lo = part == 0 ? 0 : nin, hi = part == 0 ? nin : nloc; int first = no;
            for(int i = lo; i < hi; i++) if(evx[i] >= 0) {
                int k = evx[i]; uint32_t id = uni(H.eid[loc_e[i]]); int j = no - 1;
                while(j >= first && uni(H.eid[mdeg[j]]) > id) { order[j + 1] = order[j]; mdeg[j + 1] = mdeg[j]; j--; }
                order[j + 1] = k; mdeg[j + 1] = loc_e[i]; no++;
            }
        }
        for(int q = 0; q < no; q++) { resolve_single_trivial_vertex(order[q], jump); if(HC.status) return; }
    }
}

ALD_FN void decompose_vertex_extend_small(int root, int n) { decompose_vertex_extend_body<true>(uni(root), uni(n)); }
template<bool LDS> ALD_INL void copy_pairs(bool from_parked, bool to_parked, int n)
{
    const Pairs S = pairs_at(LDS, from_parked), D = pairs_at(LDS, to_parked);
    for(int i = 0; i < n; i++) { D.a[i] = S.a[i]; D.b[i] = S.b[i]; D.w[i] = S.w[i]; }
}
ALD_FN void decompose_vertex_extend_any(int root, int n)
{
    root = uni(root); n = uni(n);
    if(uni(HC.pw_lds) != 0) {
        const Pairs S = pairs_at(true, false), D = pairs_at(false, false);
        if(ALD_UNLIKELY(n > D.cap)) { fail(ALD_ST_CAPACITY); return; }
        for(int i = 0; i < n; i++) { D.a[i] = S.a[i]; D.b[i] = S.b[i]; D.w[i] = S.w[i]; }
        HC.pw_lds = 0;
    }
    decompose_vertex_extend_body<false>(root, n);
}
ALD_INL void decompose_vertex_extend(int root, int n)
{
    root = uni(root); n = uni(n);
    const int deg = (int)uni(H.vx[root].in_deg) + (int)uni(H.vx[root].out_deg);
    if(uni(HC.pw_lds) != 0 && 4 * deg <= ARENA_I && deg <= ARENA_D && !(uni(HC.p_ratio[7]) > 1.0)) decompose_vertex_extend_small(root, n);
    else decompose_vertex_extend_any(root, n);
}
#ifndef ALD_NO_EXTEND22
ALD_FN bool intersect_would_hold(int e1, int e2)
{
    e1 = uni(e1); e2 = uni(e2);
    COLD;
    const uint32_t n1 = uni(C.ed[e1].sp_len), n2 = uni(C.ed[e2].sp_len);
    const int i1 = uni(C.ed[e1].s0id), i2 = uni(C.ed[e2].s0id);
    if(n1 == 1 && n2 == 1) return i1 == i2;
    const uint32_t o1 = uni(C.ed[e1].sp_off), o2 = uni(C.ed[e2].sp_off);
    const uint32_t need = n1 < n2 ? n1 : n2;
    if(uni(HC.sp_used) + need > C.sp_cap) return false;
    uint32_t i = 0, j = 0, k = 0;
    while(i < n1 && j < n2) {
        int a = n1 == 1 ? i1 : uni(C.sp_id[o1 + i]), b = n2 == 1 ? i2 : uni(C.sp_id[o2 + j]);
        if(a < b) i++; else if(b < a) j++; else { k++; i++; j++; }
    }
    return k > 0;
}
ALD_FN bool extend_22(int root)
{
    root = uni(root);
    COLD;
    const int lane = lane_id();
    int bad = 0;
    if(uni(HC.pw_lds) == 0 || uni(HC.p_ratio[7]) > 1.0) bad = 1;
    const Hot::VertexHot vrx = H.vx[root];
    int ge[4], gfar[4];
    {
        int e = slot_or_neg(vrx.in_head);
        ALD_UNROLL for(int k = 0; k < 2; k++) {
            if(e < 0) bad = 1;
            const int es = e >= 0 ? e : 0; const uint64_t lw = *(const uint64_t*)&H.ed[es].lk;
            ge[k] = es; gfar[k] = (int)(lw & 0xFFFF); e = lk_next((uint32_t)((lw >> 32) & 0xFFFF));
        }
        if(e >= 0) bad = 1;
        e = slot_or_neg(vrx.out_head);
        ALD_UNROLL for(int k = 2; k < 4; k++) {
            if(e < 0) bad = 1;
            const int es = e >= 0 ? e : 0; const uint64_t lw = *(const uint64_t*)&H.ed[es].lk;
            ge[k] = es; gfar[k] = (int)((lw >> 16) & 0xFFFF); e = lk_next((uint32_t)(lw >> 48));
        }
        if(e >= 0) bad = 1;
    }
    const int lt_v = C.vx[root].lpos, rt_v = C.vx[root].rpos, rv_v = C.vx[root].v2v; const double vw_v = C.vx[root].vw;
#ifndef ALD_EMU
    double pf_med, pf_abd; int pf_mei, pf_st, pf_cnt, pf_id, pf_pos; uint32_t pf_ns; uint64_t pf_mask0;
    { const int l4 = lane < 4 ? lane : 0; const int f = pick<4>(ge, l4), fv = pick<4>(gfar, l4);
      pf_med = C.ed[f].med; pf_abd = C.ed[f].s0abd; pf_mei = C.ed[f].mei; pf_st = C.ed[f].estrand; pf_cnt = C.ed[f].ecount; pf_id = C.ed[f].s0id; pf_ns = C.ed[f].sp_len; pf_mask0 = C.ed[f].mask[0];
      pf_pos = l4 < 2 ? C.vx[fv].rpos : C.vx[fv].lpos; }
#endif
    const Pairs P = pairs_at(true, false);
    const int a0 = P.a[0], a1 = P.a[1], a2 = P.a[2], b0 = P.b[0], b1 = P.b[1], b2 = P.b[2];
    const double w0 = P.w[0], w1 = P.w[1], w2 = P.w[2];
    const int la0 = PLOC(a0), la1 = PLOC(a1), la2 = PLOC(a2), lb0 = PLOC(b0) - 2, lb1 = PLOC(b1) - 2, lb2 = PLOC(b2) - 2;
    if((unsigned)la0 > 1u || (unsigned)la1 > 1u || (unsigned)la2 > 1u || (unsigned)lb0 > 1u || (unsigned)lb1 > 1u || (unsigned)lb2 > 1u) bad = 1;
    if(PSLOT(a0) != (la0 ? ge[1] : ge[0]) || PSLOT(a1) != (la1 ? ge[1] : ge[0]) || PSLOT(a2) != (la2 ? ge[1] : ge[0])) bad = 1;
    if(PSLOT(b0) != (lb0 ? ge[3] : ge[2]) || PSLOT(b1) != (lb1 ? ge[3] : ge[2]) || PSLOT(b2) != (lb2 ? ge[3] : ge[2])) bad = 1;
    const int c0 = uni((la0 << 1) | lb0), c1 = uni((la1 << 1) | lb1), c2 = uni((la2 << 1) | lb2);
    if(c0 == c1 || c0 == c2 || c1 == c2) bad = 1;
    const int cm = (6 - c0 - c1 - c2) & 3;
    const int ip = cm >> 1, op = 2 + (cm & 1), is = 1 - ip, os = 5 - op;
    const int cz = (is << 1) | (os - 2), ci = (ip << 1) | (os - 2), co = (is << 1) | (op - 2);
    const double mw = HC.p_min_w;
    if(!(w0 >= mw - kSMIN) || !(w1 >= mw - kSMIN) || !(w2 >= mw - kSMIN)) bad = 1;
    double total_weight = 0; total_weight += w0; total_weight += w1; total_weight += w2;
    const double wz = c0 == cz ? w0 : (c1 == cz ? w1 : w2), wi = c0 == ci ? w0 : (c1 == ci ? w1 : w2), wo = c0 == co ? w0 : (c1 == co ? w1 : w2);
    const int m = uni(HC.nv), fh = uni(HC.free_head), hw = uni(HC.slot_hw), id = uni(HC.next_id);
    if(m + 2 > MAXV || (fh < 0 && hw >= MAXE) || id >= EID_LIMIT) bad = 1;
    const int z = fh >= 0 ? fh : (hw < MAXE ? hw : 0);
    const bool dupi = uni(gfar[0] == gfar[1]), dupo = uni(gfar[2] == gfar[3]);
    const int rlen = uni(rt_v) - uni(lt_v), rv = uni(rv_v);
    const double vertex_weight = uni(vw_v) * rlen;
#ifdef ALD_EMU
    const int e_is = ge[is], e_os = ge[os], e_ip = ge[ip], e_op = ge[op];
    const int st_is = C.ed[e_is].estrand, st_os = C.ed[e_os].estrand, cnt_is = C.ed[e_is].ecount, cnt_os = C.ed[e_os].ecount, id_is = C.ed[e_is].s0id, id_os = C.ed[e_os].s0id;
    const uint32_t ns_is = C.ed[e_is].sp_len, ns_os = C.ed[e_os].sp_len; const double abd_is = C.ed[e_is].s0abd, abd_os = C.ed[e_os].s0abd;
#else
    const int e_is = uni(pick<4>(ge, is)), e_os = uni(pick<4>(ge, os)), e_ip = uni(pick<4>(ge, ip)), e_op = uni(pick<4>(ge, op));
    const int st_is = wread(pf_st, is), st_os = wread(pf_st, os), cnt_is = wread(pf_cnt, is), cnt_os = wread(pf_cnt, os), id_is = wread(pf_id, is), id_os = wread(pf_id, os);
    const uint32_t ns_is = (uint32_t)wread((int)pf_ns, is), ns_os = (uint32_t)wread((int)pf_ns, os); const double abd_is = wread(pf_abd, is), abd_os = wread(pf_abd, os);
#endif
    if(!(cnt_is > 0 && cnt_os > 0)) bad = 1;
    const bool inline_sp = (ns_is == 1 && ns_os == 1);
    if(inline_sp) { if(id_is != id_os) bad = 1; }
    else if(!bad && !uni(intersect_would_hold(e_is, e_os))) bad = 1;
    const bool zfirst = uni(pick<4>(gfar, op) == uni(HC.sinkp));
#ifdef ALD_EMU_COUNT
    if(bad) g_cnt_x22[1]++; else { g_cnt_x22[0]++; if(st_os != 0) g_cnt_x22s[0]++; if(st_is != 0) g_cnt_x22s[1]++; if(st_os == 0 && st_is != 0) g_cnt_x22s[2]++; if(st_os != 0 && st_is == 0) g_cnt_x22s[3]++; }
#endif
    if(wballot(bad != 0) != 0) return false;
    for(int j = lane; j < 4; j += ALD_WAVE) {
        const bool in_side = j < 2, star = (j == is) || (j == os);
        const int e = pick<4>(ge, j), fv = pick<4>(gfar, j);
        const int nvx = in_side ? (star ? m : m + 1) : (star ? m + 1 : m);
#ifdef ALD_EMU
        const double pf_med = C.ed[e].med; const int pf_mei = C.ed[e].mei, pf_pos = in_side ? C.vx[fv].rpos : C.vx[fv].lpos; const uint64_t pf_mask0 = C.ed[e].mask[0];
#endif
        if(star) {
            C.vx[nvx].lpos = pf_pos; C.vx[nvx].rpos = pf_pos; C.vx[nvx].vtype = -1; C.vx[nvx].vw = 0; C.vx[nvx].v2v = -2;
        } else {
            const int sp = in_side ? st_os : st_is;
            if(sp != 0) C.ed[e].estrand = (uint8_t)sp;
            if(rv >= 0) { const int k = rv >> 6; C.ed[e].mask[k] = (k == 0 ? pf_mask0 : C.ed[e].mask[k]) | (1ull << (rv & 63)); }
            const double mweight = (in_side ? wi : wo) / total_weight * vertex_weight;
            C.ed[e].med = pf_med + mweight; C.ed[e].mei = pf_mei + rlen;
        }
        if(in_side) {
            H.ed[e].lk.inx = star ? NIL : (IDX)z;
            if(!dupi) { H.ed[e].lk.et = (IDX)nvx; relink_out_lane(fv, e, (uint32_t)nvx); }
        } else {
            H.ed[e].lk.onx = (star || zfirst) ? NIL : (IDX)z;
            if(!dupo) { H.ed[e].lk.es = (IDX)nvx; relink_in_lane(fv, e, (uint32_t)nvx); }
        }
    }
    star_tail_sync();
    if(lane == 0) {
        if(dupi) { ALD_UNROLL for(int k = 0; k < 2; k++) { const int nk = (k == is) ? m : m + 1; H.ed[ge[k]].lk.et = (IDX)nk; relink_out(gfar[k], ge[k], (uint32_t)nk); } }
        if(dupo) { ALD_UNROLL for(int k = 2; k < 4; k++) { const int nk = (k == os) ? m + 1 : m; H.ed[ge[k]].lk.es = (IDX)nk; relink_in(gfar[k], ge[k], (uint32_t)nk); } }
        if(fh >= 0) { const IDX nx = uni(H.ed[z].lk.onx); HC.free_head = nx == NIL ? -1 : (int)nx; HC.free_cnt = uni(HC.free_cnt) - 1; }
        else HC.slot_hw = hw + 1;
        HC.next_id = id + 1;
        H.ed[z].lk.es = (IDX)m; H.ed[z].lk.et = (IDX)(m + 1); H.ed[z].lk.inx = NIL; H.ed[z].lk.onx = zfirst ? (IDX)e_op : NIL;
        H.eid[z] = (EID)id; H.hflag[z] = 0; H.ed[z].w = wz;
        H.vx[m].in_head = (IDX)e_is; H.vx[m].out_head = zfirst ? (IDX)z : (IDX)e_op; H.vx[m].in_deg = 1; H.vx[m].out_deg = 2; H.nz[m] = 1;
        H.vx[m + 1].in_head = (IDX)e_ip; H.vx[m + 1].out_head = (IDX)e_os; H.vx[m + 1].in_deg = 2; H.vx[m + 1].out_deg = 1; H.nz[m + 1] = 1;
        HC.nv = m + 2; HC.maybe_broken = 1; HC.maybe_triv = 1; ev_mark_all();
        if(inline_sp) { const double c = (abd_os < abd_is) ? abd_os : abd_is; C.ed[z].sp_off = 0; C.ed[z].sp_len = 1; C.ed[z].ecount = 1; C.ed[z].eabd = 0.0 + c; C.ed[z].s0id = id_is; C.ed[z].s0abd = c; }
        else intersect_samples(e_is, e_os, z);
        C.ed[z].econf = 0; C.ed[z].estrand = (uint8_t)(st_os != 0 ? st_os : st_is);
        for(int k = 0; k < NW; k++) C.ed[z].mask[k] = (rv >= 0 && (rv >> 6) == k) ? (1ull << (rv & 63)) : 0ull;
        C.ed[z].med = wz / total_weight * vertex_weight; C.ed[z].mei = rlen;
#ifdef ALD_EMU_COUNT
        { const int32_t d0 = HC.hs_dirty; HC.hs_dirty = 0; hs_insert_between(e_is, e_os, z); if(HC.hs_dirty) g_cnt_x22s[4]++; HC.hs_dirty |= d0; }
#else
        hs_insert_between(e_is, e_os, z);
#endif
        clear_vertex(root);
    }
    wsync();
    return true;
}
#endif
ALD_FN void decompose_vertex_extend_wave(int root, int n)
{
    root = uni(root); n = uni(n);
#ifdef ALD_EMU_COUNT
    g_cnt_x22[2]++;
#endif
#ifndef ALD_NO_EXTEND22
    if(n == 3 && uni(H.vx[root].in_deg) == 2 && uni(H.vx[root].out_deg) == 2) { if(uni(extend_22(root))) return; }
#endif
    if(lane_id() == 0) decompose_vertex_extend(root, n);
    wsync();
}

ALD_INL int classify_trivial_fastpath(int x, bool fast)
{
    int d1 = H.vx[x].in_deg, d2 = H.vx[x].out_deg;
    if(d1 != 1 && d2 != 1) return -1;
    int e1 = first_in(x), e2 = first_out(x);
    if(d1 == 1) { int s = H.ed[e1].lk.es; if(H.vx[s].out_deg == 1) return 1; if(fast) { if(!(H.hflag[e1] & HF_OCC)) return 1; return -2; } }
    if(d2 == 1) { int t = H.ed[e2].lk.et; if(H.vx[t].in_deg == 1) return 1; if(fast) { if(!(H.hflag[e2] & HF_OCC)) return 1; return -2; } }
    return 2;
}
ALD_FN int classify_trivial_vertex(int x, bool fast)
{
    x = uni(x); fast = uni(fast);
    int d1 = uni(H.vx[x].in_deg), d2 = uni(H.vx[x].out_deg);
    if(d1 != 1 && d2 != 1) return -1;
    int e1 = u_first_in(x), e2 = u_first_out(x);
    if(d1 == 1) { int s = uni(H.ed[e1].lk.es); if(H.vx[s].out_deg == 1) return 1; if(fast && hs_dominate(e1, 1)) return 1; }
    if(d2 == 1) { int t = uni(H.ed[e2].lk.et); if(H.vx[t].in_deg == 1) return 1; if(fast && hs_dominate(e2, 2)) return 1; }
    return 2;
}
ALD_INL double compute_balance_ratio(int v, bool &ok)
{
#ifndef ALD_MERGED_WALKS
    double w1 = in_weights(v), w2 = out_weights(v);
#else
    double w1 = 0, w2 = 0;
    {
        int a = first_in(v), b = first_out(v);
        while((a >= 0) | (b >= 0)) {
            const int ea = a >= 0 ? a : 0, eb = b >= 0 ? b : 0;
            const double wa = H.ed[ea].w, wb = H.ed[eb].w; const IDX na = H.ed[ea].lk.inx, nb = H.ed[eb].lk.onx;
            if(a >= 0) { w1 += wa; a = na == NIL ? -1 : (int)na; }
            if(b >= 0) { w2 += wb; b = nb == NIL ? -1 : (int)nb; }
        }
    }
#endif
    ok = (w1 >= kSMIN) && (w2 >= kSMIN);
    if(w1 >= w2) return w1 / w2; else return w2 / w1;
}
ALD_FN bool resolve_single_trivial_vertex(int i, double jump_ratio)
{
    i = uni(i); jump_ratio = uni(jump_ratio);
    if(H.vx[i].in_deg == 0 || H.vx[i].out_deg == 0) return false;
    if(H.vx[i].in_deg >= 2 && H.vx[i].out_deg >= 2) return false;
    if(mixed_strand_vertex(i)) return false;
    if(classify_trivial_vertex(i, false) != 1) return false;
    bool ok; double r = compute_balance_ratio(i, ok);
    if(ALD_UNLIKELY(!ok)) { fail(ALD_ST_INVARIANT + ALD_INV_WEIGHT); return false; }
    if(r >= jump_ratio) return false;
    trace(OP_TRIVIAL_FAST, vlog(i), 0, r);
    decompose_trivial_vertex(i);
    return true;
}
ALD_INL int eval_smallest(int i, double &r)
{
    int hin, hout;
    {
        const Hot::VertexHot vr = H.vx[i];
        const int nzv = H.nz[i] & NZ_MEMBER, d1 = vr.in_deg, d2 = vr.out_deg;
        if((nzv == 0) | (d1 <= 1) | (d2 <= 1)) return -1;
        hin = slot_or_neg(vr.in_head); hout = slot_or_neg(vr.out_head);
    }
    int e1 = -1, e2 = -1; double sum1 = 0, sum2 = 0, min1 = DBL_MAX, min2 = DBL_MAX;
#ifndef ALD_MERGED_WALKS
    for(int e = hin; e >= 0; e = next_in(e)) { double w = H.ed[e].w; sum1 += w; if(w > min1) continue; min1 = w; e1 = e; }
    for(int e = hout; e >= 0; e = next_out(e)) { double w = H.ed[e].w; sum2 += w; if(w > min2) continue; min2 = w; e2 = e; }
#else
    {
        int a = hin, b = hout;
        while((a >= 0) | (b >= 0)) {
            const int ea = a >= 0 ? a : 0, eb = b >= 0 ? b : 0;
            const double wa = H.ed[ea].w, wb = H.ed[eb].w; const IDX na = H.ed[ea].lk.inx, nb = H.ed[eb].lk.onx;
            if(a >= 0) { sum1 += wa; if(!(wa > min1)) { min1 = wa; e1 = a; } a = na == NIL ? -1 : (int)na; }
            if(b >= 0) { sum2 += wb; if(!(wb > min2)) { min2 = wb; e2 = b; } b = nb == NIL ? -1 : (int)nb; }
        }
    }
#endif
    if(e1 < 0 || e2 < 0) return -1;
    if(!(sum1 >= kSMIN) || !(sum2 >= kSMIN)) return -3;
    double r1 = min1 / sum1, r2 = min2 / sum2;
    int e; if(r1 < r2) { r = r1; e = e1; } else { r = r2; e = e2; }
    int s = H.ed[e].lk.es, t = H.ed[e].lk.et;
    uint8_t f = H.hflag[e];
    { const int ods = H.vx[s].out_deg, idt = H.vx[t].in_deg; if((ods <= 1) | (idt <= 1)) return -1; }
    if((f & HF_REXT) && (f & HF_LEXT)) return -1;
    if(t == i && (f & HF_REXT)) return -1;
    if(s == i && (f & HF_LEXT)) return -1;
    if(HC.any_strand) {
        COLD;
        int z = C.ed[e].estrand;
        if(z >= 1) { int vs[6]; strand_degree(i, vs); if(s == i && vs[0] + vs[z] <= 1) return -1; if(t == i && vs[3] + vs[z + 3] <= 1) return -1; }
    }
    return e;
}

ALD_INL bool resolve_broken_vertex()
{
    if(!uni(HC.maybe_broken)) return false;
    const int lane = lane_id();
    int vend = HC.nv; int x = -1;
    for(int base = 0; base < vend && x < 0; base += ALD_WAVE) {
        int i = base + lane;
        const bool inr = (i >= 1) & (i < vend) & (i != HC.sinkp); const int ii = inr ? i : 0;
        const Hot::VertexHot vr = H.vx[ii];
        const int nzv = H.nz[ii] & NZ_MEMBER, d1 = vr.in_deg, d2 = vr.out_deg;
        bool p = inr & (nzv != 0) & !((d1 >= 1) & (d2 >= 1));
        uint64_t m = wballot(p);
        if(m) x = base + ffs64(m);
    }
    if(x < 0) { wsync(); if(lane == 0) HC.maybe_broken = 0; wsync(); return false; }
    if(lane == 0) {
        if(H.vx[x].in_deg + H.vx[x].out_deg == 0) fail(ALD_ST_INVARIANT + ALD_INV_OTHER);
        else {
            HC.maybe_triv = 1;
            trace(OP_BROKEN, vlog(x), H.vx[x].in_deg + H.vx[x].out_deg, 0);
            int guard = MAXE;
            while(first_in(x) >= 0 && guard-- > 0) { int e = first_in(x); kill_edge(e); hs_remove(e); }
            while(first_out(x) >= 0 && guard-- > 0) { int e = first_out(x); kill_edge(e); hs_remove(e); }
            H.nz[x] = 0; ev_mark(x);
        }
    }
    wsync();
    return true;
}

ALD_INL int nth_set_bit(uint64_t m, int r)
{
    int pos = 0;
    ALD_UNROLL for(int w = 32; w >= 1; w >>= 1) {
        const uint64_t low = m & ((1ull << w) - 1ull); const int c = (int)__builtin_popcountll(low);
        if(r >= c) { r -= c; m >>= w; pos += w; } else m = low;
    }
    return pos;
}
ALD_INL int classify_with_ratio(int i, bool inr, double &r, bool &bad)
{
    int cls = -9; r = 0; bad = false;
    const int ii = inr ? i : 0;
    const Hot::VertexHot vr = H.vx[ii];
    const int nzv = H.nz[ii] & NZ_MEMBER, d1 = vr.in_deg, d2 = vr.out_deg; const IDX h1 = vr.in_head, h2 = vr.out_head;
    bool elig = inr & (nzv != 0) & (d1 >= 1) & (d2 >= 1) & !((d1 >= 2) & (d2 >= 2));
    if(HC.any_strand) elig = elig && !mixed_strand_vertex(i);
    const int e1 = (elig & (h1 != NIL)) ? (int)h1 : 0, e2 = (elig & (h2 != NIL)) ? (int)h2 : 0;
    const IDX sv = H.ed[e1].lk.es, tv = H.ed[e2].lk.et; const uint8_t f1 = H.hflag[e1], f2 = H.hflag[e2];
    const int s_ = (elig & (sv != NIL)) ? (int)sv : 0, t_ = (elig & (tv != NIL)) ? (int)tv : 0;
    const int ods = H.vx[s_].out_deg, idt = H.vx[t_].in_deg;
    if(elig) {
        if(d1 == 1 && ods == 1) cls = 1;
        else if(d1 == 1) cls = (f1 & HF_OCC) ? -2 : 1;
        else if(d2 == 1 && idt == 1) cls = 1;
        else if(d2 == 1) cls = (f2 & HF_OCC) ? -2 : 1;
        else cls = 2;
        bool ok; r = compute_balance_ratio(i, ok); bad = !ok;
    }
    return cls;
}
enum { SC_NONE = 0, SC_HIT = 1, SC_STOP = 2, SC_NEED = 3, SC_BAD = 4 };
enum { EV_NC_ = MAXV / ALD_WAVE };
#ifdef ALD_SCAN_INLINE
ALD_INL int scan_trivial(int start, int mode, int type, double jump_ratio)
#else
ALD_FN int scan_trivial(int start, int mode, int type, double jump_ratio)
#endif
{
    start = uni(start); mode = uni(mode); type = uni(type); jump_ratio = uni(jump_ratio);
    const int lane = lane_id();
    const bool fast = (mode == 1);
    const double now_thr = (mode == 1) ? 1.02 : jump_ratio;
    const int vend = HC.sw_vend;
    double best_r = HC.sw_best_r; int best_v = HC.sw_best_v;
    const int dom_base = HC.sw_dom_base;
    int code = SC_NONE, hit = -1; double hit_r = 0;
    int ncand = 0;
    double frr = DBL_MAX; int fvv = -1;
#if ALD_KEEP_TRIV
    ALD_GLOBAL double *kr = (ALD_GLOBAL double*)(HC.cold + CL::o_tvr); ALD_GLOBAL int32_t *kc = (ALD_GLOBAL int32_t*)(HC.cold + CL::o_tvc);
    const bool kept = (mode == 1);
    if(kept) {
        const int nv_now = uni(HC.nv);
  #if defined(ALD_EMU) && defined(ALD_EMU_CHECK)
        if(HC.tv_all == 0) for(int v = 1; v < nv_now; v++) {
            if((HC.tv_dirty[v >> 5] >> (v & 31)) & 1u) continue;
            double r2; bool b2; const int c2 = classify_with_ratio(v, true, r2, b2); const int kc_ = kc[v]; const double kr_ = kr[v];
            if((c2 & 0xFF) != (kc_ & 0xFF) || (int)b2 != ((kc_ >> 8) & 1) || (c2 != -9 && memcmp(&r2, &kr_, 8) != 0)) { fprintf(stderr, "[check] graph %d: stale trivial-scan record of vertex %d: kept (%d, %.17g), fresh (%d, %.17g)\n", HC.g, v, kc_, kr_, c2, r2); abort(); }
        }
  #endif
        if(uni(HC.tv_all) != 0) {
            for(int b0 = 0; b0 < nv_now; b0 += ALD_WAVE) { const int v = b0 + lane; const bool in = v >= 1 && v < nv_now; double r2; bool b2; const int c2 = classify_with_ratio(v, in, r2, b2); if(v < nv_now) { kr[v] = r2; kc[v] = (c2 & 0xFF) | (b2 ? 0x100 : 0); } }
        } else {
  #ifdef ALD_EMU
            for(int v = 1; v < nv_now; v++) if((HC.tv_dirty[v >> 5] >> (v & 31)) & 1u) { double r2; bool b2; const int c2 = classify_with_ratio(v, true, r2, b2); kr[v] = r2; kc[v] = (c2 & 0xFF) | (b2 ? 0x100 : 0); }
  #else
            int total = 0;
            for(int w = 0; w < (nv_now + 31) / 32; w++) total += (int)__builtin_popcount(uni(HC.tv_dirty[w]));
            for(int b0 = 0; b0 < total; b0 += ALD_WAVE) {
                const int k = b0 + lane; int run = 0, vtx = -1;
                for(int w = 0; w < (nv_now + 31) / 32; w++) {
                    const uint32_t m = uni(HC.tv_dirty[w]); const int pc = (int)__builtin_popcount(m);
                    if(k >= run && k < run + pc) vtx = 32 * w + nth_set_bit((uint64_t)m, k - run);
                    run += pc;
                }
                const bool in = vtx >= 1 && vtx < nv_now;
                double r2; bool b2; const int c2 = classify_with_ratio(vtx, in, r2, b2);
                if(in) { kr[vtx] = r2; kc[vtx] = (c2 & 0xFF) | (b2 ? 0x100 : 0); }
            }
  #endif
        }
        wsync_mem();
        tv_clear_marks(nv_now);
        wsync();
    }
#else
    const bool kept = false;
#endif
#if ALD_KEEP_TRIV
    constexpr int KNC = (EV_NC_ <= 16) ? EV_NC_ : 1;
    double pr_[KNC]; int pc_[KNC];
    if(kept && EV_NC_ <= 16) {
        ALD_UNROLL for(int c = 0; c < KNC; c++) {
            const int i = c * ALD_WAVE + lane; const bool in = (i >= start) & (i < vend);
            pr_[c] = in ? kr[i] : 0.0; pc_[c] = in ? kc[i] : (-9 & 0xFF);
        }
    }
#endif
    for(int base = (start / ALD_WAVE) * ALD_WAVE; base < vend; base += ALD_WAVE) {
        int i = base + lane;
        int cls = -9; double r = 0; bool bad = false; bool kbad = false;
#if ALD_KEEP_TRIV
        if(kept) {
            const bool inr = (i >= start) & (i < vend);
            int kc_ = (-9 & 0xFF); double kr_ = 0;
            if(EV_NC_ <= 16) { const int cq = base / ALD_WAVE; ALD_UNROLL for(int c = 0; c < KNC; c++) if(c == cq) { kc_ = pc_[c]; kr_ = pr_[c]; } }
            else if(inr) { kc_ = kc[i]; kr_ = kr[i]; }
            if(inr) { r = kr_; cls = (int)(int8_t)(kc_ & 0xFF); kbad = (kc_ & 0x100) != 0; }
        } else
#endif
        {
            const bool inr = (i >= start) & (i < vend); const int ii = inr ? i : 0;
            const Hot::VertexHot vr = H.vx[ii];
            const int nzv = H.nz[ii] & NZ_MEMBER, d1 = vr.in_deg, d2 = vr.out_deg; const IDX h1 = vr.in_head, h2 = vr.out_head;
            bool elig = inr & (nzv != 0) & (d1 >= 1) & (d2 >= 1) & !((d1 >= 2) & (d2 >= 2));
            if(HC.any_strand) elig = elig && !mixed_strand_vertex(i);
            const int e1 = (elig & (h1 != NIL)) ? (int)h1 : 0, e2 = (elig & (h2 != NIL)) ? (int)h2 : 0;
            const IDX sv = H.ed[e1].lk.es, tv = H.ed[e2].lk.et; const uint8_t f1 = H.hflag[e1], f2 = H.hflag[e2];
            const int s_ = (elig & (sv != NIL)) ? (int)sv : 0, t_ = (elig & (tv != NIL)) ? (int)tv : 0;
            const int ods = H.vx[s_].out_deg, idt = H.vx[t_].in_deg;
            if(elig) {
                if(d1 == 1 && ods == 1) cls = 1;
                else if(d1 == 1 && fast) cls = (f1 & HF_OCC) ? -2 : 1;
                else if(d2 == 1 && idt == 1) cls = 1;
                else if(d2 == 1 && fast) cls = (f2 & HF_OCC) ? -2 : 1;
                else cls = 2;
            }
        }
        if(cls == -2 && base == dom_base) cls = HC.scr_i[lane];
        uint64_t need = wballot(cls == -2);
        if(need) { if(lane == 0) { HC.sw_dom_base = base; HC.sw_need_lo = (uint32_t)need; HC.sw_need_hi = (uint32_t)(need >> 32); } code = SC_NEED; break; }
        bool cand = (cls == type);
        ncand += (int)__builtin_popcountll(wballot(cand));
        if(cand) { if(kept) bad = kbad; else { bool ok; r = compute_balance_ratio(i, ok); if(!ok) bad = true; } }
        {
            if(wballot(bad)) {
                const uint64_t badm = wballot(bad);
                const uint64_t ev = wballot(cand && !bad && (r < now_thr || (mode == 1 && r < jump_ratio)));
                if(!(ev & ((1ull << ffs64(badm)) - 1))) { code = SC_BAD; break; }
            }
        }
        uint64_t now = wballot(cand && r < now_thr);
        uint64_t stp = (mode == 1) ? wballot(cand && !(r < now_thr) && r < jump_ratio) : 0ull;
        if(stp && (!now || ffs64(stp) < ffs64(now))) {
            int l = ffs64(stp); best_v = base + l; best_r = wread(r, l); code = SC_STOP; break;
        }
        int lim = now ? ffs64(now) : ALD_WAVE;
        if(mode == 1 && cand && lane < lim && (fvv < 0 || !(frr < r))) { frr = r; fvv = i; }
        if(now) { hit = base + ffs64(now); hit_r = wread(r, ffs64(now)); code = SC_HIT; break; }
    }
    if(mode == 1 && code != SC_STOP && code != SC_BAD) {
        double rr = frr; int vv = fvv;
        wave_argmin(rr, vv);
        if(vv >= 0 && !(best_r < rr)) { best_r = rr; best_v = vv; }
    }
    if(lane == 0) { HC.sw_best_r = best_r; HC.sw_best_v = best_v; HC.sw_hit = hit; HC.sw_hit_r = hit_r; HC.sw_ncand = (start == 1 && code == SC_NONE) ? ncand : -1; }
    wsync();
    return code;
}
ALD_INL void check_no_trivial_candidate()
{
#if defined(ALD_EMU) && defined(ALD_EMU_CHECK)
    for(int v = 1; v < HC.nv; v++) {
        const int d1 = H.vx[v].in_deg, d2 = H.vx[v].out_deg;
        if(!(H.nz[v] & NZ_MEMBER) || d1 < 1 || d2 < 1 || (d1 >= 2 && d2 >= 2) || mixed_strand_vertex(v)) continue;
        if(classify_trivial_vertex(v, true) == 1) { fprintf(stderr, "[check] graph %d: trivial-vertex scan skipped while vertex %d (degrees %d, %d) is a type-1 candidate\n", HC.g, v, d1, d2); abort(); }
    }
#endif
}
ALD_INL bool sweep_trivial_body(int mode, int type, double jump_ratio, int &fired, const bool tr);
ALD_INL bool sweep_trivial(int mode, int type, double jump_ratio)
{
    int fired = 0; const bool tr = tracing_u();
    const bool rv = sweep_trivial_body(mode, type, jump_ratio, fired, tr);
    if(fired && lane_id() == 0) HC.n_iters += fired;
    return rv;
}
ALD_INL bool sweep_trivial_body(int mode, int type, double jump_ratio, int &fired, const bool tr)
{
    mode = uni(mode); type = uni(type); jump_ratio = uni(jump_ratio);
    const int lane = lane_id();
    PROF_DECL;
    const int hsd_q = HC.hs_dirty, strand_q = HC.any_strand, triv_q = HC.maybe_triv, nv_q = HC.nv;
    const bool skippable = (mode == 1 && type == 1 && !uni(strand_q));
    if(skippable && !uni(hsd_q) && !uni(triv_q)) { check_no_trivial_candidate(); return false; }
    if(lane == 0) { if(uni(hsd_q)) hs_refresh_flags(); HC.sw_vend = nv_q; HC.sw_best_r = DBL_MAX; HC.sw_best_v = -1; HC.sw_dom_base = -1; }
    wsync();
    if(skippable && !uni(HC.maybe_triv)) { check_no_trivial_candidate(); return false; }
    bool flag = false;
    int start = 1;
    for(;;) {
        int target = -1; bool last = false;
        while(start < uni(HC.sw_vend)) {
            int code = uni(scan_trivial(start, mode, type, jump_ratio));
            PROF_ADD(PF_TRIV_EVAL);
            if(code == SC_NEED) {
                if(lane == 0) {
                    uint64_t need = (uint64_t)HC.sw_need_lo | ((uint64_t)HC.sw_need_hi << 32); const int base = HC.sw_dom_base;
                    while(need) { int l = ffs64(need); need &= need - 1; HC.scr_i[l] = classify_trivial_vertex(base + l, mode == 1); }
                }
                wsync();
                if(uni(HC.sw_dom_base) > start) start = uni(HC.sw_dom_base);
                continue;
            }
            if(code == SC_BAD) { if(lane == 0) fail(ALD_ST_INVARIANT + ALD_INV_WEIGHT); wsync(); return true; }
            if(code == SC_HIT) target = uni(HC.sw_hit);
            break;
        }
        if(target < 0) {
            if(flag) return true;
            if(mode == 0) return false;
            if(uni(HC.sw_best_v) < 0) { if(skippable) { if(lane == 0) HC.maybe_triv = 0; wsync(); } return false; }
            target = uni(HC.sw_best_v); last = true;
#ifndef ALD_NO_TRIV_CLEAR
            if(skippable && uni(HC.sw_ncand) == 1) { if(lane == 0) HC.maybe_triv = 0; wsync(); }
#endif
        }
        fired++;
        if(tr && lane == 0) { if(last) trace_emit(OP_TRIVIAL_BEST, vlog(target), type, HC.sw_best_r); else trace_emit(mode == 1 ? OP_TRIVIAL_NOW : OP_TRIVIAL_FAST, vlog(target), mode == 1 ? type : 0, HC.sw_hit_r); }
        decompose_trivial_vertex_wave(target);
        if(last) { wsync(); PROF_ADD(PF_TRIV_MUT); return true; }
        if(lane == 0) {
            if(uni(HC.hs_dirty)) hs_refresh_flags();
            HC.sw_dom_base = -1;
        }
        wsync();
        PROF_ADD(PF_TRIV_MUT);
        flag = true;
        if(HC.status) return true;
        start = target + 1;
    }
}

ALD_INL bool back_to_cascade()
{
    const int a = HC.status, b = HC.maybe_broken, c = HC.maybe_triv, d = HC.hs_dirty;
    return uni(a | b | c | d) != 0;
}
enum { EV_NC = MAXV / ALD_WAVE };
ALD_INL bool sweep_smallest_body(double max_ratio, int &fired, const bool tr);
ALD_INL bool sweep_smallest(double max_ratio)
{
    int fired = 0; const bool tr = tracing_u();
    const bool rv = sweep_smallest_body(max_ratio, fired, tr);
    if(fired && lane_id() == 0) HC.n_iters += fired;
    return rv;
}
ALD_INL bool sweep_smallest_body(double max_ratio, int &fired, const bool tr)
{
    max_ratio = uni(max_ratio);
    const int lane = lane_id();
    const int vend = uni(HC.nv);
    constexpr int NC = EV_NC;
    if(vend > NC * ALD_WAVE) { if(lane == 0) fail(ALD_ST_CAPACITY); wsync(); return true; }
    PROF_DECL;
    if(lane == 0 && uni(HC.hs_dirty)) hs_refresh_flags();
    wsync();
    double cr[NC]; int ce[NC];
    const int nch0 = (vend + ALD_WAVE - 1) / ALD_WAVE;
#if ALD_KEEP
    ALD_GLOBAL double *mr = (ALD_GLOBAL double*)(HC.cold + CL::o_evr); ALD_GLOBAL int32_t *me = (ALD_GLOBAL int32_t*)(HC.cold + CL::o_eve);
    const bool stale_all = uni(HC.ev_all) != 0;
  #if defined(ALD_EMU) && defined(ALD_EMU_CHECK)
    { static long n_entry = 0, n_all = 0, n_marked = 0, n_live = 0; static struct P { long *a, *b, *c, *d; ~P() { if(*a && getenv("ALD_EMU_VERBOSE")) fprintf(stderr, "[emu-ev] class %d: %ld sweep entries, %.1f %% with everything stale, else %.1f marked of %.1f vertices\n", ALD_CLASS_ID, *a, 100.0 * *b / *a, (double)*c / ((*a - *b) ? (*a - *b) : 1), (double)*d / *a); } } pr{&n_entry, &n_all, &n_marked, &n_live};
      n_entry++; n_live += vend; if(stale_all) n_all++; else for(int i = 1; i < vend; i++) if((HC.ev_dirty[i >> 5] >> (i & 31)) & 1u) n_marked++; }
    if(!stale_all) for(int i = 1; i < vend; i++) {
        if((HC.ev_dirty[i >> 5] >> (i & 31)) & 1u) continue;
        double r = 0; const int e = eval_smallest(i, r); const double kr_ = mr[i]; const int ke_ = me[i];
        if(e != ke_ || (e >= 0 && memcmp(&r, &kr_, 8) != 0)) { fprintf(stderr, "[check] graph %d: stale smallest-edge evaluation of vertex %d: kept (%d, %.17g), fresh (%d, %.17g)\n", HC.g, i, ke_, kr_, e, r); abort(); }
    }
  #endif
    if(!stale_all) {
  #ifdef ALD_EMU
        for(int i = 1; i < vend; i++) if((HC.ev_dirty[i >> 5] >> (i & 31)) & 1u) { double r = 0; const int e = eval_smallest(i, r); mr[i] = r; me[i] = e; }
  #else
        int total = 0;
        for(int w = 0; w < (vend + 31) / 32; w++) total += (int)__builtin_popcount(uni(HC.ev_dirty[w]));
        for(int base = 0; base < total; base += ALD_WAVE) {
            const int k = base + lane; int run = 0, vtx = -1;
            for(int w = 0; w < (vend + 31) / 32; w++) {
                const uint32_t m = uni(HC.ev_dirty[w]); const int pc = (int)__builtin_popcount(m);
                if(k >= run && k < run + pc) vtx = 32 * w + nth_set_bit((uint64_t)m, k - run);
                run += pc;
            }
            if(vtx >= 1 && vtx < vend) { double r = 0; const int e = eval_smallest(vtx, r); mr[vtx] = r; me[vtx] = e; }
        }
  #endif
        wsync_mem();
        if(NC <= 16) { ALD_UNROLL for(int c = 0; c < (NC <= 16 ? NC : 1); c++) { const bool in = c < nch0; cr[c] = in ? mr[c * ALD_WAVE + lane] : 0.0; ce[c] = in ? me[c * ALD_WAVE + lane] : -1; } }
        else for(int c = 0; c < nch0; c++) { cr[c] = mr[c * ALD_WAVE + lane]; ce[c] = me[c * ALD_WAVE + lane]; }
    }
    else if(NC <= 16) { ALD_UNROLL for(int c = 0; c < (NC <= 16 ? NC : 1); c++) { cr[c] = 0; ce[c] = -1; } }
    auto keep = [&]() {
        if(NC <= 16) { ALD_UNROLL for(int c = 0; c < (NC <= 16 ? NC : 1); c++) if(c < nch0) { mr[c * ALD_WAVE + lane] = cr[c]; me[c * ALD_WAVE + lane] = ce[c]; } }
        else for(int c = 0; c < nch0; c++) { mr[c * ALD_WAVE + lane] = cr[c]; me[c * ALD_WAVE + lane] = ce[c]; }
    };
#else
    const bool stale_all = true;
    if(NC <= 16) { ALD_UNROLL for(int c = 0; c < (NC <= 16 ? NC : 1); c++) { cr[c] = 0; ce[c] = -1; } }
    auto keep = [&]() {};
#endif
    constexpr bool REG = (NC <= 16);
    auto cput = [&](int c, double r, int e) { if(!REG) { cr[c] = r; ce[c] = e; } else { ALD_UNROLL for(int k = 0; k < NC; k++) if(k == c) { cr[k] = r; ce[k] = e; } } };
    auto cget_e = [&](int c) -> int { if(!REG) return ce[c]; int v = -1; ALD_UNROLL for(int k = 0; k < NC; k++) if(k == c) v = ce[k]; return v; };
    auto eval_chunk = [&](int c, bool every, int ds, int dt) {
        int i = c * ALD_WAVE + lane; double r = 0; int e = -1; bool mine = i >= 1 && i < vend && (every || i == ds || i == dt);
        if(mine) e = eval_smallest(i, r);
        if(!REG) { if(mine) { cr[c] = r; ce[c] = e; } }
        else { ALD_UNROLL for(int k = 0; k < NC; k++) if(k == c && mine) { cr[k] = r; ce[k] = e; } }
    };
    if(stale_all) { for(int c = 0; c < nch0; c++) eval_chunk(c, true, -1, -1); }
#if ALD_KEEP
    wsync();
    ev_clear_marks(vend);
    wsync();
#endif
    PROF_ADD(PF_T_MERGE_KILL);
    const bool may_chain = !(uni(HC.p_ratio[7]) > 1.0) && !uni(HC.any_strand);
    auto sweeps = [&]() -> bool {
    bool any = false;
    int guard = MAXE + 8;
    while(guard-- > 0) {
        bool flag = false;
        double best_r = max_ratio; int best_e = -1, best_v = -1;
        int start = 1;
        while(start < vend) {
            int hit = -1, hit_e = -1; double hit_r = 0;
            {
            const int c0 = start / ALD_WAVE; bool badw = false;
            ALD_UNROLL for(int c = 0; c < NC; c++) {
                if(c < c0 || c * ALD_WAVE >= vend || hit >= 0 || badw) continue;
                const int i = c * ALD_WAVE + lane;
                const int e = (i >= start && i < vend) ? ce[c] : -1;
                const uint64_t badm = wballot(e == -3);
                const uint64_t now = wballot(e >= 0 && cr[c] < 0.01);
                if(ALD_UNLIKELY(badm != 0) && (!now || ffs64(badm) < ffs64(now))) { badw = true; continue; }
                if(now) { const int l = ffs64(now); hit = c * ALD_WAVE + l; hit_e = wread(e, l); hit_r = wread(cr[c], l); }
            }
            if(badw) { if(lane == 0) fail(ALD_ST_INVARIANT + ALD_INV_WEIGHT); wsync(); return true; }
            {
                const int lim = hit >= 0 ? hit : vend;
                double rr = DBL_MAX; int vv = -1;
                ALD_UNROLL for(int c = 0; c < NC; c++) {
                    if(c < c0 || c * ALD_WAVE >= lim) continue;
                    const int i = c * ALD_WAVE + lane;
                    if(i >= start && i < lim && ce[c] >= 0 && (vv < 0 || !(rr < cr[c]))) { rr = cr[c]; vv = i; }
                }
                wave_argmin(rr, vv);
                if(vv >= 0 && !(best_r < rr)) { best_r = rr; best_v = vv; best_e = wread(cget_e(vv / ALD_WAVE), vv % ALD_WAVE); }
            }
            }
            PROF_ADD(PF_SMALL_EVAL);
            if(hit < 0) break;
            const int ds = H.ed[hit_e].lk.es, dt = H.ed[hit_e].lk.et;
            fired++;
            if(tr && lane == 0) trace_emit(OP_SMALL_NOW, (int)H.eid[hit_e], vlog(hit), hit_r);
            kill_edge_wave(hit_e);
            if(lane == 0) hs_remove(hit_e);
            wsync();
            const bool all = uni(HC.hs_dirty) != 0 || (int)uni(H.vx[ds].out_deg) <= 1 || (int)uni(H.vx[dt].in_deg) <= 1;
            if(uni(HC.hs_dirty)) { if(lane == 0) hs_refresh_flags(); wsync(); }
#if ALD_KEEP
            if(all) { wsync(); ev_clear_marks(vend); wsync(); }
#endif
            if(NC <= 2) { for(int c = 0; c < NC; c++) { int i = c * ALD_WAVE + lane; if(i >= 1 && i < vend && (all || i == ds || i == dt)) { cr[c] = 0; ce[c] = eval_smallest(i, cr[c]); } } }
            else if(all) { const int nch = (vend + ALD_WAVE - 1) / ALD_WAVE; for(int c = 0; c < nch; c++) eval_chunk(c, true, -1, -1); }
            else {
                const int c1 = uni(ds) / ALD_WAVE, c2 = uni(dt) / ALD_WAVE;
                eval_chunk(c1, false, ds, dt);
                if(c2 != c1) eval_chunk(c2, false, ds, dt);
            }
            PROF_ADD(PF_SMALL_MUT);
            flag = true;
            start = hit + 1;
        }
        if(!flag) {
            if(best_e < 0) return any;
            const int ds = H.ed[best_e].lk.es, dt = H.ed[best_e].lk.et;
            fired++;
            if(tr && lane == 0) trace_emit(OP_SMALLEST, (int)H.eid[best_e], vlog(best_v), best_r);
            kill_edge_wave(best_e);
            if(lane == 0) hs_remove(best_e);
// ... 797 lines not shown
            }
        }
        if(!bad) {
            const int i0 = io[n], i1 = io[n + 1];
            int q = i1 - 1; while(q >= i0 && (H.hflag[ie[q]] & RAW_DEAD)) q--;
            if(q >= i0) {
                int pa = ie[q]; const int v0 = H.ed[pa].lk.es; int32_t p1 = C.vx[v0].rpos, p2 = p1; int k1 = v0, k2 = v0; int live = 0;
                for(int z = i0; z < i1; z++) if(!(H.hflag[ie[z]] & RAW_DEAD)) live++;
                if(live > 1) for(q--; q >= i0 && !bad; q--) {
                    const int pb = ie[q]; if(H.hflag[pb] & RAW_DEAD) continue;
                    const int vi = H.ed[pb].lk.es; const int32_t p = C.vx[vi].rpos; const double wb = H.ed[pb].w;
                    bool b = raw_continuous(C, vo, vi, k2);
                    if(p > p2) { bad = 1; break; }
                    if(p2 - p > dist) b = false;
                    if(!b) { p1 = p; p2 = p; k1 = vi; k2 = vi; pa = pb; continue; }
                    tmap[2 * nt] = p; tmap[2 * nt + 1] = p1; nt++;
                    for(int j = vi; j < k1; j++) {
                        const int pc = raw_edge(vo, j, j + 1);
                        if(pc < 0) { bad = 1; break; }
                        const double wc = H.ed[pc].w; H.ed[pc].w = wc + wb; C.vx[j + 1].vw = wc + wb;
                    }
                    if(bad) break;
                    H.ed[pa].w += wb;
                    H.hflag[pb] |= RAW_DEAD; removed++;
                    k2 = vi; p2 = p;
                }
            }
        }
        if(bad) fail(ALD_ST_INVARIANT + ALD_INV_OTHER);
        HC.scr_i[0] = ns; HC.scr_i[1] = nt; HC.scr_i[2] = removed;
    }
    wsync_mem();
    if(uni(HC.status)) return false;
    const int ns = uni(HC.scr_i[0]), nt = uni(HC.scr_i[1]), removed = uni(HC.scr_i[2]);
    if(removed) {
        ALD_GLOBAL int32_t *flag = C.wi, *nrank = C.wi + E;
        for(int k = lane; k < E; k += ALD_WAVE) flag[H.eid[k]] = (H.hflag[k] & RAW_DEAD) ? 0 : 1;
        wsync_mem();
        int base = 0;
        for(int r0 = 0; r0 < E; r0 += ALD_WAVE) {
            const int r = r0 + lane; const bool f = r < E && flag[r] != 0;
            const uint64_t m = wballot(f);
#ifdef ALD_EMU
            if(r < E) nrank[r] = base;
#else
            if(r < E) nrank[r] = base + __builtin_popcountll(m & ((1ull << lane) - 1));
#endif
            base += __builtin_popcountll(m);
        }
        wsync_mem();
        for(int k = lane; k < E; k += ALD_WAVE) if(!(H.hflag[k] & RAW_DEAD)) H.eid[k] = (EID)nrank[H.eid[k]];
        wsync_mem();
        if(lane == 0) {
            for(int k = 0; k < E; k++) if(H.hflag[k] & RAW_DEAD) { H.hflag[k] = 0; kill_edge_i(k); }
            HC.next_id = base;
            for(int i = 1; i < n; i++) if(H.vx[i].in_deg == 0 && H.vx[i].out_deg == 0) H.nz[i] = 0;
        }
        wsync_mem();
    }
    ALD_GLOBAL int32_t *tv = C.wi + RAW_TV;
    ALD_GLOBAL int32_t *tv_off = tv + 1, *tv_cnt = tv + 1 + RAW_TV_CAP + 1;
    ALD_GLOBAL int32_t *vtx = (ALD_GLOBAL int32_t*)C.wd;
    if(NPH > RAW_TV_CAP) { if(lane == 0) fail(ALD_ST_CAPACITY); wsync_mem(); return false; }
    if(NPH == 0) { if(lane == 0) { tv[0] = 0; tv_off[0] = 0; } wsync_mem(); return true; }
    bool unsorted = false;
    for(int i = 1 + lane; i < n; i += ALD_WAVE) { if(C.vx[i].lpos > C.vx[i + 1].lpos) unsorted = true; if(i + 1 < n && C.vx[i].rpos > C.vx[i + 1].rpos) unsorted = true; }
    if(lane == 0 && n >= 2 && C.vx[0].rpos > C.vx[1].rpos) unsorted = true;
    const bool sorted = wballot(unsorted) == 0;
    ALD_GLOBAL const int32_t *smap = C.wi + RAW_SMAP, *tmap = C.wi + RAW_TMAP;
    auto lfind = [&](int32_t p) -> int {
        if(sorted) { int lo = 1, hi = n + 1; while(lo < hi) { const int mid = (lo + hi) >> 1; if(C.vx[mid].lpos < p) lo = mid + 1; else hi = mid; } return (lo <= n && C.vx[lo].lpos == p) ? lo : -1; }
        for(int i = 1; i <= n; i++) if(C.vx[i].lpos == p) return i;
        return -1; };
    auto rfind = [&](int32_t q) -> int {
        if(sorted) { int lo = 0, hi = n; while(lo < hi) { const int mid = (lo + hi) >> 1; if(C.vx[mid].rpos < q) lo = mid + 1; else hi = mid; } return (lo < n && C.vx[lo].rpos == q) ? lo : -1; }
        for(int i = 0; i < n; i++) if(C.vx[i].rpos == q) return i;
        return -1; };
    int total = 0; bool assert_hit = false;
    for(int p0 = 0; p0 < NPH; p0 += ALD_WAVE) {
        const int p = p0 + lane; int len = -1;
        if(p < NPH) {
            const int a0 = pho[p], m = pho[p + 1] - a0, ne = m / 2; len = 0; int prev = -1; bool backwards = false;
            for(int k = 0; k < ne && len >= 0; k++) {
                int32_t x = phc[a0 + 2 * k], y = phc[a0 + 2 * k + 1];
                if(k == 0) for(int z = 0; z < ns; z++) if(smap[2 * z] == x) { x = smap[2 * z + 1]; break; }
                if(k == ne - 1) for(int z = 0; z < nt; z++) if(tmap[2 * z] == y) { y = tmap[2 * z + 1]; break; }
                if(x < 0 || y < 0 || x >= y) { len = -1; break; }
                const int a = lfind(x), b = rfind(y);
                if(a < 0 || b < 0 || a > b || !raw_continuous(C, vo, a, b)) { len = -1; break; }
                if(a <= prev) backwards = true;
                prev = b; len += b - a + 1;
            }
            if(len >= 0 && backwards) assert_hit = true;
        }
        if(p < NPH) HC.scr_i[8 + lane] = len;
        wsync_mem();
        if(lane == 0) { const int cnt = (NPH - p0) < ALD_WAVE ? (NPH - p0) : ALD_WAVE; int run = total; for(int l = 0; l < cnt; l++) { tv_off[p0 + l] = run; const int x = HC.scr_i[8 + l]; tv_cnt[p0 + l] = x < 0 ? -1 : 0; if(x > 0) run += x; } HC.scr_i[7] = run; }
        wsync_mem();
        total = uni(HC.scr_i[7]);
    }
    if(wballot(assert_hit)) { if(lane == 0) fail(ALD_ST_INVARIANT + ALD_INV_OTHER); wsync_mem(); return false; }
    if(total > RAW_VTX_CAP) { if(lane == 0) fail(ALD_ST_CAPACITY); wsync_mem(); return false; }
    if(lane == 0) tv_off[NPH] = total;
    wsync_mem();
    for(int p = lane; p < NPH; p += ALD_WAVE) {
        if(tv_cnt[p] < 0) continue;
        const int a0 = pho[p], m = pho[p + 1] - a0, ne = m / 2; int w = tv_off[p];
        for(int k = 0; k < ne; k++) {
            int32_t x = phc[a0 + 2 * k], y = phc[a0 + 2 * k + 1];
            if(k == 0) for(int z = 0; z < ns; z++) if(smap[2 * z] == x) { x = smap[2 * z + 1]; break; }
            if(k == ne - 1) for(int z = 0; z < nt; z++) if(tmap[2 * z] == y) { y = tmap[2 * z + 1]; break; }
            const int a = lfind(x), b = rfind(y);
            for(int j = a; j <= b; j++) vtx[w++] = j;
        }
    }
    wsync_mem();
    for(int p = lane; p < NPH; p += ALD_WAVE) {
        if(tv_cnt[p] < 0) continue;
        const int o = tv_off[p], len = tv_off[p + 1] - o; int rep = p;
        for(int q = 0; q < p && rep == p; q++) {
            if(tv_cnt[q] < 0 || tv_off[q + 1] - tv_off[q] != len) continue;
            bool eq = true; for(int k = 0; k < len && eq; k++) eq = vtx[tv_off[q] + k] == vtx[o + k];
            if(eq) rep = q;
        }
        if(rep != p) tv_cnt[p] = -2 - rep;
    }
    wsync_mem();
    for(int p = lane; p < NPH; p += ALD_WAVE) {
        if(tv_cnt[p] != 0) continue;
        int c = phn[p];
        for(int q = p + 1; q < NPH; q++) if(tv_cnt[q] == -2 - p) c += phn[q];
        tv_cnt[p] = c;
    }
    wsync_mem();
    for(int p = lane; p < NPH; p += ALD_WAVE) if(tv_cnt[p] < 0) tv_cnt[p] = 0;
    if(lane == 0) tv[0] = NPH;
    wsync_mem();
    return true;
}
#else
enum { RAW_TV = 0, RAW_TV_CAP = 0 };
#endif

ALD_FN bool load_graph()
{
    COLD;
    const int lane = lane_id();
    ALD_GLOBAL const KernelArgs *A = HC.args;
    const int g = HC.g;
    int V = A->in.g_nv[g], E = A->in.g_ne[g], NP = A->in.g_np[g];
    int64_t ov = A->in.off_v[g], ovo = ov + g, oe = A->in.off_e[g], oeo = oe + g, os = A->in.off_s[g], op = A->in.off_p[g], opo = op + g, opv = A->in.off_pv[g];
    if(lane == 0) {
        HC.V0 = V; HC.gstrand = (int)(unsigned char)A->in.graph_strand[g];
        HC.sinkp = V - 1; HC.special_linked = 0; HC.maybe_broken = 1; HC.maybe_triv = 1; ev_mark_all();
        HC.nv = V; HC.next_id = E; HC.slot_hw = E; HC.free_head = -1; HC.free_cnt = 0; HC.status = 0; HC.any_strand = 0; HC.hs_dirty = 1;
        HC.n_paths = 0; HC.n_iters = 0; HC.n_trace = 0; HC.sp_used = 0; HC.hl_used = 0; HC.hl_n = 0;
    }
    wsync();
    if(V + 1 > MAXV || E > MAXE || V > NW * 64 || V < 2) { if(lane == 0) HC.status = ALD_ST_CAPACITY; wsync(); return false; }
    int64_t ns = A->in.edge_sample_offset[oeo + E];
    if(ns > (int64_t)C.sp_cap) { if(lane == 0) HC.status = ALD_ST_CAPACITY; wsync(); return false; }
    ALD_GLOBAL const int32_t *vo = A->in.vertex_offset + ovo, *io = A->in.in_offset + ovo, *ie = A->in.in_edge + oe;
    for(int i = lane; i < V; i += ALD_WAVE) {
        int o0 = vo[i], o1 = vo[i + 1], i0 = io[i], i1 = io[i + 1];
        H.vx[i].out_head = (o1 > o0 && i != 0) ? (IDX)o0 : NIL; H.vx[i].out_deg = (IDX)(o1 - o0);
        H.vx[i].in_head = (i1 > i0 && i != V - 1) ? (IDX)ie[i0] : NIL; H.vx[i].in_deg = (IDX)(i1 - i0);
        H.nz[i] = (i >= 1 && i < V - 1 && (o1 - o0) + (i1 - i0) > 0) ? 1 : 0;
        for(int k = o0; k < o1; k++) { H.ed[k].lk.es = (IDX)i; H.ed[k].lk.onx = (k + 1 < o1) ? (IDX)(k + 1) : NIL; }
        for(int k = i0; k < i1; k++) { H.ed[ie[k]].lk.inx = (k + 1 < i1) ? (IDX)ie[k + 1] : NIL; }
        C.vx[i].vw = A->in.vertex_weight[ov + i]; C.vx[i].lpos = A->in.vertex_lpos[ov + i]; C.vx[i].rpos = A->in.vertex_rpos[ov + i];
        C.vx[i].vtype = A->in.vertex_type[ov + i]; C.vx[i].v2v = i;
    }
    bool strand = false, listed = false;
    ALD_GLOBAL const int32_t *so = A->in.edge_sample_offset + oeo;
    ALD_GLOBAL const int32_t *rank = A->in.edge_rank;
    for(int k = lane; k < E; k += ALD_WAVE) {
        H.ed[k].lk.et = (IDX)A->in.edge_target[oe + k]; H.ed[k].w = A->in.edge_weight[oe + k]; H.eid[k] = rank ? (EID)rank[oe + k] : (EID)k; H.hflag[k] = 0;
        uint8_t st = A->in.edge_strand[oe + k]; C.ed[k].estrand = st; if(st) strand = true;
        C.ed[k].med = 0; C.ed[k].mei = 0; C.ed[k].econf = 0; C.ed[k].eabd = A->in.edge_abd[oe + k];
        C.ed[k].sp_off = (uint32_t)so[k]; C.ed[k].sp_len = (uint32_t)(so[k + 1] - so[k]); C.ed[k].ecount = A->in.edge_count[oe + k];
        if(so[k + 1] - so[k] >= 2) listed = true;
        if(so[k + 1] > so[k]) { C.ed[k].s0id = A->in.sample_id[os + so[k]]; C.ed[k].s0abd = A->in.sample_abd[os + so[k]]; } else { C.ed[k].s0id = 0; C.ed[k].s0abd = 0; }
        for(int q = 0; q < NW; q++) C.ed[k].mask[q] = 0;
    }
    if(wballot(listed)) for(int64_t k = lane; k < ns; k += ALD_WAVE) { C.sp_id[k] = A->in.sample_id[os + k]; C.sp_abd[k] = A->in.sample_abd[os + k]; }
    uint64_t sb = wballot(strand);
    if(sb && lane == 0) HC.any_strand = 1;
    if(lane == 0) HC.sp_used = (uint32_t)ns;
    wsync();
    const int rawdist = A->in.g_rawdist ? uni(A->in.g_rawdist[g]) : -1;
    if(rawdist >= 0) {
#ifdef ALD_RAW_VARIANT
        const int64_t orp = A->in.off_rp[g], orc = A->in.off_rc[g];
        if(!uni(pre_assemble_device(rawdist, V, E, vo, io, ie, (int)(A->in.off_rp[g + 1] - orp), A->in.rphase_offset + orp + g, A->in.rphase_coord + orc, A->in.rphase_count + orp))) { wsync(); return false; }
#else
        if(lane == 0) HC.status = ALD_ST_INVARIANT + ALD_INV_OTHER;
        wsync(); return false;
#endif
    }
    if(lane == 0) {
        if(rawdist < 0) build_phasing_lists(vo, V, NP, A->in.phasing_offset + opo, A->in.phasing_vertex + opv, A->in.phasing_count + op);
        else build_phasing_lists(vo, V, uni(C.wi[RAW_TV + 0]), C.wi + RAW_TV + 1, (ALD_GLOBAL const int32_t*)C.wd, C.wi + RAW_TV + 1 + RAW_TV_CAP + 1);
    }
    wsync();
    return HC.status == 0;
}

ALD_FN void finish_graph()
{
    {
        COLD;
        ALD_GLOBAL const KernelArgs *A = HC.args; const int g = uni(HC.g);
        const int st = uni(HC.status), np = (st == 0 || st == ALD_ST_SKIPPED_LARGE) ? uni(HC.n_paths) : 0;
        if(lane_id() == 0) {
            long long base = -1;
            if(np > 0) { const unsigned long long b0 = atomic_add_u64(A->out.index_used, (unsigned long long)np); if(ALD_UNLIKELY(b0 + (unsigned long long)np > A->out.index_cap)) HC.status = ALD_ST_POOL_FULL; else base = (long long)b0; }
            A->out.graph_first[g] = base;
            HC.scr_i[0] = (int32_t)(uint32_t)((unsigned long long)base & 0xFFFFFFFFull); HC.scr_i[1] = (int32_t)(uint32_t)((unsigned long long)base >> 32);
        }
        wsync_mem();
        const long long base = (long long)(((unsigned long long)(uint32_t)uni(HC.scr_i[1]) << 32) | (unsigned long long)(uint32_t)uni(HC.scr_i[0]));
        if(base >= 0) for(int i = lane_id(); i < np; i += ALD_WAVE) A->out.index[base + i] = C.po[i];
        wsync_mem();
    }
    if(lane_id() == 0) {
        ALD_GLOBAL const KernelArgs *A = HC.args; const int g = HC.g;
        A->out.status[g] = HC.status; A->out.n_paths[g] = (HC.status == 0 || HC.status == ALD_ST_SKIPPED_LARGE) ? HC.n_paths : 0; A->out.n_iters[g] = HC.n_iters;
#ifdef ALD_PROF
        if(HC.p_trace_cap > 0) for(int k = 0; k < PF_COUNT; k++) { int q = HC.n_trace++; if(q < A->out.trace_cap) { int64_t o = (int64_t)g * A->out.trace_cap + q; A->out.trace_codes[3 * o] = 100 + k; A->out.trace_codes[3 * o + 1] = 0; A->out.trace_codes[3 * o + 2] = 0; A->out.trace_vals[o] = (double)HC.prof[k]; } }
#endif
        if(A->out.trace_cap > 0) A->out.trace_n[g] = HC.n_trace;
    }
    wsync_mem();
}

#ifndef ALD_RAW_VARIANT
ALD_INL void run_graph()
#else
ALD_FN void run_graph()
#endif
{
    PROF_DECL;
#ifdef ALD_PROF
    if(lane_id() == 0) for(int k = 0; k < 32; k++) HC.prof[k] = 0;
    wsync();
#endif
    if(!uni(load_graph())) { finish_graph(); return; }
    PROF_ADD(PF_LOAD);
    bool skipped = false;
#ifndef ALD_SGPR_DIET
    const double r_triv = uni(HC.p_ratio[7]), r_small = uni(HC.p_ratio[0]), r_single = uni(HC.p_ratio[5]), r_pure = uni(HC.p_ratio[4]);
    const int max_exons = uni(HC.p_max_exons);
#else
    #define r_triv uni(HC.p_ratio[7])
    #define r_small uni(HC.p_ratio[0])
    #define r_single uni(HC.p_ratio[5])
    #define r_pure uni(HC.p_ratio[4])
    #define max_exons uni(HC.p_max_exons)
#endif
    int guard = 64 * MAXE;
    while(guard-- > 0) {
        bool brk = false;
        { const int nvq = HC.nv, stq = HC.status, mbq = HC.maybe_broken;
          if(uni(nvq) > max_exons) { skipped = true; break; }
          if(uni(stq)) break;
          PROF_RESET();
          brk = uni(mbq) != 0 && uni(resolve_broken_vertex()); }
        PROF_ADD(PF_BROKEN);
        if(brk) continue;
        bool fired = false;
        for(int stage = (r_triv > 1.0) ? 0 : 1; stage <= 4 && !fired; stage++) {
            if(stage == 0 || stage == 1 || stage == 4) fired = uni(sweep_trivial(stage == 0 ? 0 : 1, stage == 4 ? 2 : 1, r_triv));
            else if(stage == 2) fired = uni(sweep_smallest(r_small));
            else {
                PROF_RESET();
                memo_clear();
                for(int pass = 0; pass < 6 && !fired; pass++)
                    fired = uni(sweep_unsplittable((pass & 1) ? T_SPLITTABLE_PURE : T_UNSPLITTABLE_SINGLE, pass < 2 ? 1 : INT_MAX,
                                                   pass < 2 ? 0.01 : (pass == 2 ? r_single : (pass == 3 ? r_pure : DBL_MAX))));
                PROF_ADD(PF_UNSPLIT);
            }
        }
        if(fired) continue;
        break;
    }
    if(lane_id() == 0 && HC.status == 0 && guard <= 0) fail(ALD_ST_INVARIANT + ALD_INV_OTHER);
    wsync();
    if(uni(HC.status) == 0) {
        PROF_RESET();
        collect_existing_st_paths();
        PROF_ADD(PF_COLLECT0);
        if(lane_id() == 0) {
            if(HC.status == 0) greedy_decompose();
            if(HC.status == 0 && skipped) HC.status = ALD_ST_SKIPPED_LARGE;
        }
        PROF_ADD(PF_S7);
    }
    wsync();
    finish_graph();
#ifdef ALD_SGPR_DIET
    #undef r_triv
    #undef r_small
    #undef r_single
    #undef r_pure
    #undef max_exons
#endif
}
// ... 44 lines not shown
```

Measured before the change: 2.742 million.

## Track exposed vertices in maybe_triv to avoid full trivial-vertex scans

Turns the maybe_triv flag into a word that can name up to two vertices whose degree dropped to one or less, set when edges are killed. The trivial-vertex sweep then evaluates only those named vertices and falls back to the full scan when a neighbour or an occupancy flag could change the answer. Star merges now raise the flag from the net degree instead of the transient unlink, so fewer full rescans are triggered. This adds bookkeeping and a fast path whose decision has to match the full scan exactly (tie-breaking and ratio thresholds), which brings correctness risk and more code size.

```diff
diff --git a/aletsch_amd/csrc/decomp_device.h b/aletsch_amd/csrc/decomp_device.h
--- a/aletsch_amd/csrc/decomp_device.h
+++ b/aletsch_amd/csrc/decomp_device.h
@@ -26,7 +26,9 @@
 using namespace ald;
 #ifdef ALD_EMU_COUNT
 static long g_cnt_router = 0, g_cnt_unsweep = 0, g_cnt_star[34] = {0}, g_cnt_rdeg[34] = {0}, g_cnt_build = 0, g_cnt_pre[3] = {0}, g_cnt_fix[8] = {0}, g_cnt_fix_declined = 0, g_cnt_x22[3] = {0}, g_cnt_x22s[5] = {0};
-struct CntPrinter { ~CntPrinter() { if(g_cnt_unsweep) { fprintf(stderr, "[emu-count] class %d: unsplittable sweeps %ld router runs %ld (of which reach build(): %ld; prepared at level 0/1/2: %ld %ld %ld)\n", ALD_CLASS_ID, g_cnt_unsweep, g_cnt_router, g_cnt_build, g_cnt_pre[0], g_cnt_pre[1], g_cnt_pre[2]);
+static long g_cnt_scan = 0, g_cnt_scan_empty = 0, g_cnt_scan_star = 0, g_cnt_exposed = 0, g_cnt_exposed_fallback = 0; static int g_triv_why = 0, g_cnt_quiet = 0;
+struct CntPrinter { ~CntPrinter() { if(g_cnt_scan || g_cnt_exposed) fprintf(stderr, "[emu-count] class %d: trivial scans %ld (found nothing: %ld, after a star alone: %ld) exposed-vertex evaluations %ld (went on to the full scan: %ld)\n", ALD_CLASS_ID, g_cnt_scan, g_cnt_scan_empty, g_cnt_scan_star, g_cnt_exposed, g_cnt_exposed_fallback);
+    if(g_cnt_unsweep) { fprintf(stderr, "[emu-count] class %d: unsplittable sweeps %ld router runs %ld (of which reach build(): %ld; prepared at level 0/1/2: %ld %ld %ld)\n", ALD_CLASS_ID, g_cnt_unsweep, g_cnt_router, g_cnt_build, g_cnt_pre[0], g_cnt_pre[1], g_cnt_pre[2]);
     fprintf(stderr, "[emu-count]   stars by fan size:"); for(int i = 0; i < 34; i++) if(g_cnt_star[i]) fprintf(stderr, " %d:%ld", i, g_cnt_star[i]); fprintf(stderr, "\n");
     fprintf(stderr, "[emu-count]   stars through the fixed-size form:"); for(int i = 0; i < 8; i++) if(g_cnt_fix[i]) fprintf(stderr, " %d:%ld", i, g_cnt_fix[i]); fprintf(stderr, " declined:%ld\n", g_cnt_fix_declined);
     fprintf(stderr, "[emu-count]   extends: %ld through the fixed 2x2 form: %ld declined: %ld\n", g_cnt_x22[2], g_cnt_x22[0], g_cnt_x22[1]);
@@ -113,6 +115,37 @@
 #define HC g_HC
 #endif
 
+enum { TRIV_ALL = 1, TRIV_NAMED = 1 << 30, TRIV_VMASK = 0x7FFF };
+#if defined(ALD_NO_TRIV_HINT)
+  #define ALD_TRIV_HINT 0
+  #define ALD_TRIV_NET 0
+#else
+  #define ALD_TRIV_HINT (ALD_KEEP_TRIV ? 0 : 1)
+  #define ALD_TRIV_NET 1
+#endif
+static_assert(!ALD_TRIV_HINT || MAXV <= TRIV_VMASK + 1, "a vertex id of this class does not fit the named form of maybe_triv");
+#ifdef ALD_EMU_COUNT
+#define TRIV_WHY(b) (g_triv_why |= (b))
+#define TRIV_CLEARED() (g_triv_why = 0)
+#else
+#define TRIV_WHY(b) ((void)0)
+#define TRIV_CLEARED() ((void)0)
+#endif
+ALD_INL int triv_merge(int old, int a, int b)
+{
+    if(old != 0 && !(old & TRIV_NAMED)) return TRIV_ALL;
+    int lo = -1, hi = -1;
+    if(old != 0) { lo = old & TRIV_VMASK; hi = (old >> 15) & TRIV_VMASK; }
+    for(int k = 0; k < 2; k++) {
+        const int x = k == 0 ? a : b;
+        if(x < 0 || x == lo || x == hi) continue;
+        if(lo < 0) lo = hi = x;
+        else if(lo == hi) { if(x < lo) lo = x; else hi = x; }
+        else return TRIV_ALL;
+    }
+    return lo < 0 ? old : (TRIV_NAMED | (hi << 15) | lo);
+}
+
 struct ColdVertex { double vw; int32_t lpos, rpos, vtype, v2v, memo, pad_; };
 struct alignas(64) ColdEdge {
     double   med, eabd, econf, s0abd;
@@ -314,7 +347,7 @@
     H.ed[e].lk.onx = cur; *pp = (IDX)e;
     { const int dg = uni((int)H.vx[v].out_deg); H.vx[v].out_deg = (IDX)(dg + 1); ev_degree(v, dg, dg + 1, true); }
 }
-ALD_INL void unlink_in(int v, int e)
+ALD_INL void unlink_in(int v, int e, const bool raise = true)
 {
     v = uni(v); e = uni(e);
     if(v == uni(HC.sinkp) && !uni(HC.special_linked)) { const int dg = uni((int)H.vx[v].in_deg); H.vx[v].in_deg = (IDX)(dg - 1); ev_degree(v, dg, dg - 1, false); return; }
@@ -322,9 +355,9 @@
     while(uni((int)cur != e && cur != NIL) && guard-- > 0) { pp = &H.ed[cur].lk.inx; cur = *pp; }
     if(ALD_UNLIKELY(uni((int)cur != e))) { fail(ALD_ST_INVARIANT + ALD_INV_OTHER); return; }
     *pp = H.ed[e].lk.inx;
-    { int dg = (int)uni(H.vx[v].in_deg) - 1; H.vx[v].in_deg = (IDX)dg; ev_degree(v, dg + 1, dg, false); if(dg <= 1) { HC.maybe_triv = 1; if(dg == 0) HC.maybe_broken = 1; } }
-}
-ALD_INL void unlink_out(int v, int e)
+    { int dg = (int)uni(H.vx[v].in_deg) - 1; H.vx[v].in_deg = (IDX)dg; ev_degree(v, dg + 1, dg, false); if(raise && dg <= 1) { HC.maybe_triv = TRIV_ALL; TRIV_WHY(4); if(dg == 0) HC.maybe_broken = 1; } }
+}
+ALD_INL void unlink_out(int v, int e, const bool raise = true)
 {
     v = uni(v); e = uni(e);
     if(v == 0 && !uni(HC.special_linked)) { const int dg = uni((int)H.vx[v].out_deg); H.vx[v].out_deg = (IDX)(dg - 1); ev_degree(v, dg, dg - 1, true); return; }
@@ -332,7 +365,7 @@
     while(uni((int)cur != e && cur != NIL) && guard-- > 0) { pp = &H.ed[cur].lk.onx; cur = *pp; }
     if(ALD_UNLIKELY(uni((int)cur != e))) { fail(ALD_ST_INVARIANT + ALD_INV_OTHER); return; }
     *pp = H.ed[e].lk.onx;
-    { int dg = (int)uni(H.vx[v].out_deg) - 1; H.vx[v].out_deg = (IDX)dg; ev_degree(v, dg + 1, dg, true); if(dg <= 1) { HC.maybe_triv = 1; if(dg == 0) HC.maybe_broken = 1; } }
+    { int dg = (int)uni(H.vx[v].out_deg) - 1; H.vx[v].out_deg = (IDX)dg; ev_degree(v, dg + 1, dg, true); if(raise && dg <= 1) { HC.maybe_triv = TRIV_ALL; TRIV_WHY(4); if(dg == 0) HC.maybe_broken = 1; } }
 }
 ALD_INL void relink_in(int v, int e, uint32_t ks)
 {
@@ -454,6 +487,9 @@
     e = uni(e);
     const uint64_t w = *(const uint64_t*)&H.ed[e].lk;
     const bool special = HC.special_linked != 0; const int sinkp = HC.sinkp;
+#if ALD_TRIV_HINT
+    uint64_t hitm = 0;
+#endif
     for(int side = lane_id(); side < 2; side += ALD_WAVE) {
         const bool out = (side == 0);
         const int v = out ? (int)(w & 0xFFFF) : (int)((w >> 16) & 0xFFFF);
@@ -468,14 +504,26 @@
         }
         const int dg = (int)*deg - 1; *deg = (IDX)dg;
         ev_degree(v, dg + 1, dg, out);
-        if(!counted && dg <= 1) { HC.maybe_triv = 1; if(dg == 0) HC.maybe_broken = 1; }
+#if ALD_TRIV_HINT
+        { const bool hit = !counted && dg <= 1; hitm |= (ALD_WAVE == 1) ? ((uint64_t)(hit ? 1 : 0) << side) : wballot(hit); }
+        if(!counted && dg == 0) HC.maybe_broken = 1;
+#else
+        if(!counted && dg <= 1) { HC.maybe_triv = TRIV_ALL; TRIV_WHY(1); if(dg == 0) HC.maybe_broken = 1; }
+#endif
     }
     wsync();
     if(lane_id() == 0) {
         H.ed[e].lk.es = NIL;
+#if ALD_TRIV_HINT
+        const int fh = uni(HC.free_head), fc = uni(HC.free_cnt), old = uni(HC.maybe_triv);
+        H.ed[e].lk.onx = fh < 0 ? NIL : (IDX)fh; HC.free_head = e; HC.free_cnt = fc + 1;
+        if(hitm != 0) { HC.maybe_triv = triv_merge(old, (hitm & 1) ? (int)uni((uint32_t)(w & 0xFFFF)) : -1, (hitm & 2) ? (int)uni((uint32_t)((w >> 16) & 0xFFFF)) : -1); TRIV_WHY(1); }
+#else
         const int fh = uni(HC.free_head); H.ed[e].lk.onx = fh < 0 ? NIL : (IDX)fh; HC.free_head = e; HC.free_cnt = uni(HC.free_cnt) + 1;
-    }
-}
+#endif
+    }
+}
+ALD_INL void star_raise_net(int net) { if(net <= 1) { HC.maybe_triv = TRIV_ALL; TRIV_WHY(2); if(net == 0) HC.maybe_broken = 1; } }
 ALD_FN int add_edge(int s, int t) { return add_edge_i(uni(s), uni(t)); }
 ALD_FN void kill_edge(int e) { kill_edge_i(uni(e)); }
 ALD_FN void move_edge(int e, int x, int y)
@@ -546,7 +594,7 @@
 ALD_FN void hs_refresh_flags()
 {
     if(!HC.hs_dirty) return;
-    HC.maybe_triv = 1; ev_mark_all();
+    HC.maybe_triv = TRIV_ALL; TRIV_WHY(4); ev_mark_all();
     COLD;
     for(int e = 0; e < HC.slot_hw; e++) H.hflag[e] = 0;
     int nl = HC.hl_n;
@@ -1133,7 +1181,7 @@
     }
     const bool counted = A ? (far == 0 && !uni(HC.special_linked)) : (far == (int)uni(HC.sinkp) && !uni(HC.special_linked));
     const bool consumed = uni(ctx[SW_SERIAL]) != 0;
-    if(lane == 0 && consumed) { if(A) unlink_out(far, c); else unlink_in(far, c); }
+    if(lane == 0 && consumed) { if(A) unlink_out(far, c, !ALD_TRIV_NET); else unlink_in(far, c, !ALD_TRIV_NET); }
     wsync();
     PROF_ADD(PF_T_MERGE_MASK);
     if(ALD_UNLIKELY(!consumed)) { if(lane == 0) fail(ALD_ST_INVARIANT + (!(dctx[0] <= DBL_MAX) ? ALD_INV_MERGE_EQUAL : ALD_INV_DEGREE)); wsync(); return; }
@@ -1169,7 +1217,8 @@
     unsigned long long prof_s7_ = __builtin_readcyclecounter();
 #endif
     if(lane == 0) {
-        { const int dg = A ? (int)uni(H.vx[far].out_deg) : (int)uni(H.vx[far].in_deg); if(A) H.vx[far].out_deg = (IDX)(dg + n); else H.vx[far].in_deg = (IDX)(dg + n); ev_degree(far, dg, dg + n, A); }
+        { const int dg = A ? (int)uni(H.vx[far].out_deg) : (int)uni(H.vx[far].in_deg); if(A) H.vx[far].out_deg = (IDX)(dg + n); else H.vx[far].in_deg = (IDX)(dg + n); ev_degree(far, dg, dg + n, A);
+          if(ALD_TRIV_NET && !counted) star_raise_net(dg + n); }
         if(any_dup || any_multi || uni(HC.hl_n) != 0) for(int q = 0; q < n; q++) {
             const int f = fe[ord[q]];
             if(any_dup) { if(A) relink_in(oth[q], f, (uint32_t)far); else relink_out(oth[q], f, tkey((uint32_t)far)); }
@@ -1326,7 +1375,7 @@
     const bool any_multi = wballot(multi) != 0;
     PROF_ADD(PF_T_MERGE_LOAD);
     const bool counted = A ? (far == 0 && !uni(HC.special_linked)) : (far == (int)uni(HC.sinkp) && !uni(HC.special_linked));
-    if(lane == 0) { if(A) unlink_out(far, c); else unlink_in(far, c); }
+    if(lane == 0) { if(A) unlink_out(far, c, !ALD_TRIV_NET); else unlink_in(far, c, !ALD_TRIV_NET); }
     wsync();
     PROF_ADD(PF_T_MERGE_MASK);
     if(!counted) {
@@ -1360,7 +1409,8 @@
     PROF_ADD(PF_S6_LINK);
 #endif
     if(lane == 0) {
-        { const int dg = A ? (int)uni(H.vx[far].out_deg) : (int)uni(H.vx[far].in_deg); if(A) H.vx[far].out_deg = (IDX)(dg + n); else H.vx[far].in_deg = (IDX)(dg + n); ev_degree(far, dg, dg + n, A); }
+        { const int dg = A ? (int)uni(H.vx[far].out_deg) : (int)uni(H.vx[far].in_deg); if(A) H.vx[far].out_deg = (IDX)(dg + n); else H.vx[far].in_deg = (IDX)(dg + n); ev_degree(far, dg, dg + n, A);
+          if(ALD_TRIV_NET && !counted) star_raise_net(dg + n); }
         if(any_dup || any_multi || uni(HC.hl_n) != 0) for(int q = 0; q < n; q++) {
             const int fq = fem[q];
             if(any_dup) { if(A) relink_in(othm[q], fq, (uint32_t)far); else relink_out(othm[q], fq, tkey((uint32_t)far)); }
@@ -1564,7 +1614,8 @@
         if(!counted) {
             bool taken = false; ALD_UNROLL for(int k = 0; k < N; k++) if(pred[k] == pc) taken = true;
             if(!taken) { const IDX nx = c_next < 0 ? NIL : (IDX)c_next; if(pc < 0) { if(A) H.vx[far].out_head = nx; else H.vx[far].in_head = nx; } else { if(A) H.ed[pc].lk.onx = nx; else H.ed[pc].lk.inx = nx; } }
-            if(dg <= 1) { HC.maybe_triv = 1; if(dg == 0) HC.maybe_broken = 1; }
+            if(ALD_TRIV_NET) star_raise_net(dg + N);
+            else if(dg <= 1) { HC.maybe_triv = TRIV_ALL; TRIV_WHY(2); if(dg == 0) HC.maybe_broken = 1; }
         }
         *deg = (IDX)(dg + N); ev_degree(far, dg + 1, dg + N, A);
         C.vx[x].vw = vwt;
@@ -1654,7 +1705,7 @@
     int newedges = 0;
     for(int i = 0; i < n; i++) { int u1 = PLOC(a[i]), u2 = PLOC(b[i]); if(mdeg[u1] == 1 && mdeg[u2] == 1) evx[u1] = nn++; else if(mdeg[u1] >= 2 && mdeg[u2] >= 2) newedges++; }
     if(ALD_UNLIKELY(nn > MAXV || free_slots() < newedges)) { fail(ALD_ST_CAPACITY); return; }
-    HC.maybe_broken = 1; HC.maybe_triv = 1; ev_mark_all();
+    HC.maybe_broken = 1; HC.maybe_triv = TRIV_ALL; TRIV_WHY(4); ev_mark_all();
     for(int i = m; i < nn; i++) { H.vx[i].in_head = NIL; H.vx[i].out_head = NIL; H.vx[i].in_deg = 0; H.vx[i].out_deg = 0; H.nz[i] = 1; C.vx[i].vw = 0; C.vx[i].lpos = 0; C.vx[i].rpos = 0; C.vx[i].vtype = -1; C.vx[i].v2v = -1; }
     HC.nv = nn;
     for(int i = 0; i < nin; i++) {
@@ -1863,7 +1914,7 @@
         H.eid[z] = (EID)id; H.hflag[z] = 0; H.ed[z].w = wz;
         H.vx[m].in_head = (IDX)e_is; H.vx[m].out_head = zfirst ? (IDX)z : (IDX)e_op; H.vx[m].in_deg = 1; H.vx[m].out_deg = 2; H.nz[m] = 1;
         H.vx[m + 1].in_head = (IDX)e_ip; H.vx[m + 1].out_head = (IDX)e_os; H.vx[m + 1].in_deg = 2; H.vx[m + 1].out_deg = 1; H.nz[m + 1] = 1;
-        HC.nv = m + 2; HC.maybe_broken = 1; HC.maybe_triv = 1; ev_mark_all();
+        HC.nv = m + 2; HC.maybe_broken = 1; HC.maybe_triv = TRIV_ALL; TRIV_WHY(4); ev_mark_all();
         if(inline_sp) { const double c = (abd_os < abd_is) ? abd_os : abd_is; C.ed[z].sp_off = 0; C.ed[z].sp_len = 1; C.ed[z].ecount = 1; C.ed[z].eabd = 0.0 + c; C.ed[z].s0id = id_is; C.ed[z].s0abd = c; }
         else intersect_samples(e_is, e_os, z);
         C.ed[z].econf = 0; C.ed[z].estrand = (uint8_t)(st_os != 0 ? st_os : st_is);
@@ -2005,7 +2056,7 @@
     if(lane == 0) {
         if(H.vx[x].in_deg + H.vx[x].out_deg == 0) fail(ALD_ST_INVARIANT + ALD_INV_OTHER);
         else {
-            HC.maybe_triv = 1;
+            HC.maybe_triv = TRIV_ALL; TRIV_WHY(4);
             trace(OP_BROKEN, vlog(x), H.vx[x].in_deg + H.vx[x].out_deg, 0);
             int guard = MAXE;
             while(first_in(x) >= 0 && guard-- > 0) { int e = first_in(x); kill_edge(e); hs_remove(e); }
@@ -2026,9 +2077,9 @@
     }
     return pos;
 }
-ALD_INL int classify_with_ratio(int i, bool inr, double &r, bool &bad)
-{
-    int cls = -9; r = 0; bad = false;
+ALD_INL int classify_lane(int i, bool inr, bool fast, int &nb_s, int &nb_t)
+{
+    int cls = -9; nb_s = -1; nb_t = -1;
     const int ii = inr ? i : 0;
     const Hot::VertexHot vr = H.vx[ii];
     const int nzv = H.nz[ii] & NZ_MEMBER, d1 = vr.in_deg, d2 = vr.out_deg; const IDX h1 = vr.in_head, h2 = vr.out_head;
@@ -2040,12 +2091,20 @@
     const int ods = H.vx[s_].out_deg, idt = H.vx[t_].in_deg;
     if(elig) {
         if(d1 == 1 && ods == 1) cls = 1;
-        else if(d1 == 1) cls = (f1 & HF_OCC) ? -2 : 1;
+        else if(d1 == 1 && fast) cls = (f1 & HF_OCC) ? -2 : 1;
         else if(d2 == 1 && idt == 1) cls = 1;
-        else if(d2 == 1) cls = (f2 & HF_OCC) ? -2 : 1;
+        else if(d2 == 1 && fast) cls = (f2 & HF_OCC) ? -2 : 1;
         else cls = 2;
-        bool ok; r = compute_balance_ratio(i, ok); bad = !ok;
-    }
+        if(d1 == 1 && ods == 1) nb_s = s_;
+        if(d2 == 1 && idt == 1) nb_t = t_;
+    }
+    return cls;
+}
+ALD_INL int classify_with_ratio(int i, bool inr, double &r, bool &bad)
+{
+    int nb_s, nb_t; r = 0; bad = false;
+    const int cls = classify_lane(i, inr, true, nb_s, nb_t);
+    if(cls != -9) { bool ok; r = compute_balance_ratio(i, ok); bad = !ok; }
     return cls;
 }
 enum { SC_NONE = 0, SC_HIT = 1, SC_STOP = 2, SC_NEED = 3, SC_BAD = 4 };
@@ -2129,22 +2188,8 @@
         } else
 #endif
         {
-            const bool inr = (i >= start) & (i < vend); const int ii = inr ? i : 0;
-            const Hot::VertexHot vr = H.vx[ii];
-            const int nzv = H.nz[ii] & NZ_MEMBER, d1 = vr.in_deg, d2 = vr.out_deg; const IDX h1 = vr.in_head, h2 = vr.out_head;
-            bool elig = inr & (nzv != 0) & (d1 >= 1) & (d2 >= 1) & !((d1 >= 2) & (d2 >= 2));
-            if(HC.any_strand) elig = elig && !mixed_strand_vertex(i);
-            const int e1 = (elig & (h1 != NIL)) ? (int)h1 : 0, e2 = (elig & (h2 != NIL)) ? (int)h2 : 0;
-            const IDX sv = H.ed[e1].lk.es, tv = H.ed[e2].lk.et; const uint8_t f1 = H.hflag[e1], f2 = H.hflag[e2];
-            const int s_ = (elig & (sv != NIL)) ? (int)sv : 0, t_ = (elig & (tv != NIL)) ? (int)tv : 0;
-            const int ods = H.vx[s_].out_deg, idt = H.vx[t_].in_deg;
-            if(elig) {
-                if(d1 == 1 && ods == 1) cls = 1;
-                else if(d1 == 1 && fast) cls = (f1 & HF_OCC) ? -2 : 1;
-                else if(d2 == 1 && idt == 1) cls = 1;
-                else if(d2 == 1 && fast) cls = (f2 & HF_OCC) ? -2 : 1;
-                else cls = 2;
-            }
+            const bool inr = (i >= start) & (i < vend); int nb_s, nb_t;
+            cls = classify_lane(i, inr, fast, nb_s, nb_t);
         }
         if(cls == -2 && base == dom_base) cls = HC.scr_i[lane];
         uint64_t need = wballot(cls == -2);
@@ -2175,16 +2220,101 @@
     }
     if(lane == 0) { HC.sw_best_r = best_r; HC.sw_best_v = best_v; HC.sw_hit = hit; HC.sw_hit_r = hit_r; HC.sw_ncand = (start == 1 && code == SC_NONE) ? ncand : -1; }
     wsync();
+#ifdef ALD_EMU_COUNT
+    if(code != SC_NEED && !g_cnt_quiet) { g_cnt_scan++; if(code == SC_NONE && ncand == 0) g_cnt_scan_empty++; if(start == 1 && mode == 1 && type == 1 && !HC.any_strand && g_triv_why == 2) g_cnt_scan_star++; }
+#endif
     return code;
 }
-ALD_INL void check_no_trivial_candidate()
+ALD_INL void check_no_trivial_candidate(int word = 0)
 {
 #if defined(ALD_EMU) && defined(ALD_EMU_CHECK)
     for(int v = 1; v < HC.nv; v++) {
         const int d1 = H.vx[v].in_deg, d2 = H.vx[v].out_deg;
+        if((word & TRIV_NAMED) && (v == (word & TRIV_VMASK) || v == ((word >> 15) & TRIV_VMASK))) continue;
         if(!(H.nz[v] & NZ_MEMBER) || d1 < 1 || d2 < 1 || (d1 >= 2 && d2 >= 2) || mixed_strand_vertex(v)) continue;
-        if(classify_trivial_vertex(v, true) == 1) { fprintf(stderr, "[check] graph %d: trivial-vertex scan skipped while vertex %d (degrees %d, %d) is a type-1 candidate\n", HC.g, v, d1, d2); abort(); }
-    }
+        if(classify_trivial_vertex(v, true) == 1) { fprintf(stderr, "[check] graph %d: trivial-vertex scan skipped (maybe_triv %#x) while vertex %d (degrees %d, %d) is a type-1 candidate\n", HC.g, word, v, d1, d2); abort(); }
+    }
+#else
+    (void)word;
+#endif
+}
+#if ALD_TRIV_HINT
+enum { XC_FULL = 0, XC_NONE = 1, XC_HIT = 3, XC_BEST = 4 };
+#if defined(ALD_EMU) && defined(ALD_EMU_CHECK)
+static thread_local double g_chk_ratio = 0;
+#endif
+ALD_FN int exposed_trivial(int word, int vend, double jump_ratio, bool tr)
+{
+    word = uni(word); vend = uni(vend); jump_ratio = uni(jump_ratio); tr = uni(tr);
+    const int lane = lane_id();
+    const int va = word & TRIV_VMASK, vb = (word >> 15) & TRIV_VMASK;
+    const int sinkp = HC.sinkp;
+    int c0 = -9, c1 = -9, x0 = 0, x1 = 0, b0 = 0, b1 = 0; double r0 = 0, r1 = 0;
+    for(int l0 = 0; l0 < 2; l0 += ALD_WAVE) {
+        const int l = l0 + lane, v = l == 0 ? va : vb;
+        const bool inr = (l < 2) & (l == 0 || vb != va) & (v >= 1) & (v < vend);
+        int nb_s, nb_t; double r = 0; bool bad = false;
+        const int cls = classify_lane(v, inr, true, nb_s, nb_t);
+        if(cls == 1) { bool ok; r = compute_balance_ratio(v, ok); bad = !ok; }
+        const bool far_s = (nb_s >= 1) & (nb_s != sinkp) & (nb_s != va) & (nb_s != vb), far_t = (nb_t >= 1) & (nb_t != sinkp) & (nb_t != va) & (nb_t != vb);
+        const int x = ((cls == -2) | far_s | far_t) ? 1 : 0;
+        if(l == 0) { c0 = cls; r0 = r; b0 = bad ? 1 : 0; x0 = x; } else { c1 = cls; r1 = r; b1 = bad ? 1 : 0; x1 = x; }
+    }
+    if(wballot((x0 | x1) != 0) != 0) return XC_FULL;
+    const bool cand0 = uni(wread(c0, 0)) == 1, cand1 = uni(wread(c1, 1)) == 1;
+    const bool bad0 = uni(wread(b0, 0)) != 0, bad1 = uni(wread(b1, 1)) != 0;
+    const double q0 = uni(wread(r0, 0)), q1 = uni(wread(r1, 1));
+    const int ncand = (cand0 ? 1 : 0) + (cand1 ? 1 : 0);
+    const double now_thr = 1.02;
+    if(cand0 && bad0) return XC_FULL;
+    if(cand1 && bad1 && !(cand0 && (q0 < now_thr || q0 < jump_ratio))) return XC_FULL;
+    int code = XC_NONE, target = -1; double rr = 0;
+    if(cand0 && q0 < now_thr) { code = XC_HIT; target = va; rr = q0; }
+    else if(cand0 && q0 < jump_ratio) { code = XC_BEST; target = va; rr = q0; }
+    else if(cand1 && q1 < now_thr) { code = XC_HIT; target = vb; rr = q1; }
+    else if(cand1 && q1 < jump_ratio) { code = XC_BEST; target = vb; rr = q1; }
+    else {
+        double best_r = DBL_MAX;
+        if(cand0 && !(best_r < q0)) { best_r = q0; target = va; }
+        if(cand1 && !(best_r < q1)) { best_r = q1; target = vb; }
+        if(target >= 0) { code = XC_BEST; rr = best_r; }
+    }
+    if(tr && target >= 0) { if(lane == 0) { if(code == XC_HIT) HC.sw_hit_r = rr; else HC.sw_best_r = rr; } wsync(); }
+#if defined(ALD_EMU) && defined(ALD_EMU_CHECK)
+    g_chk_ratio = rr;
+#endif
+    return code | (ncand << 3) | ((target < 0 ? 0 : target) << 8);
+}
+#endif
+ALD_INL void check_exposed_decision(int code, int target, int ncand, int word, int nv_q, double jump_ratio)
+{
+#if ALD_TRIV_HINT && defined(ALD_EMU) && defined(ALD_EMU_CHECK)
+    check_no_trivial_candidate(word);
+  #ifdef ALD_EMU_COUNT
+    g_cnt_quiet = 1;
+  #endif
+    HC.sw_vend = nv_q; HC.sw_best_r = DBL_MAX; HC.sw_best_v = -1; HC.sw_dom_base = -1;
+    int start = 1, sc = SC_NONE;
+    while(start < HC.sw_vend) {
+        sc = scan_trivial(start, 1, 1, jump_ratio);
+        if(sc != SC_NEED) break;
+        uint64_t need = (uint64_t)HC.sw_need_lo | ((uint64_t)HC.sw_need_hi << 32); const int base = HC.sw_dom_base;
+        while(need) { int l = ffs64(need); need &= need - 1; HC.scr_i[l] = classify_trivial_vertex(base + l, true); }
+        if(HC.sw_dom_base > start) start = HC.sw_dom_base;
+    }
+  #ifdef ALD_EMU_COUNT
+    g_cnt_quiet = 0;
+  #endif
+    int fc, ft = 0; double fr = 0;
+    if(sc == SC_BAD) fc = -1;
+    else if(sc == SC_HIT) { fc = XC_HIT; ft = HC.sw_hit; fr = HC.sw_hit_r; }
+    else if(HC.sw_best_v < 0) fc = XC_NONE;
+    else { fc = XC_BEST; ft = HC.sw_best_v; fr = HC.sw_best_r; }
+    const bool same = fc == code && (fc == XC_NONE || (ft == target && memcmp(&fr, &g_chk_ratio, 8) == 0)) && (HC.sw_ncand < 0 || HC.sw_ncand == ncand);
+    if(!same) { fprintf(stderr, "[check] graph %d: exposed-vertex evaluation (maybe_triv %#x) decided %d on vertex %d (%.17g, %d candidates), the full scan %d on vertex %d (%.17g, %d candidates)\n", HC.g, word, code, target, g_chk_ratio, ncand, fc, ft, fr, HC.sw_ncand); abort(); }
+    HC.sw_dom_base = -1;
+#else
+    (void)code; (void)target; (void)ncand; (void)word; (void)nv_q; (void)jump_ratio;
 #endif
 }
 ALD_INL bool sweep_trivial_body(int mode, int type, double jump_ratio, int &fired, const bool tr);
@@ -2203,14 +2333,34 @@
     const int hsd_q = HC.hs_dirty, strand_q = HC.any_strand, triv_q = HC.maybe_triv, nv_q = HC.nv;
     const bool skippable = (mode == 1 && type == 1 && !uni(strand_q));
     if(skippable && !uni(hsd_q) && !uni(triv_q)) { check_no_trivial_candidate(); return false; }
-    if(lane == 0) { if(uni(hsd_q)) hs_refresh_flags(); HC.sw_vend = nv_q; HC.sw_best_r = DBL_MAX; HC.sw_best_v = -1; HC.sw_dom_base = -1; }
-    wsync();
-    if(skippable && !uni(HC.maybe_triv)) { check_no_trivial_candidate(); return false; }
+    int target = -1; bool last = false;
+    bool xp = false;
+#if ALD_TRIV_HINT
+    if(skippable && !uni(hsd_q) && (uni(triv_q) & TRIV_NAMED)) {
+        const int xc = uni(exposed_trivial(uni(triv_q), uni(nv_q), jump_ratio, tr));
+        PROF_ADD(PF_TRIV_EVAL);
+        const int code = xc & 7, ncand = (xc >> 3) & 3;
+  #ifdef ALD_EMU_COUNT
+        if(code == XC_FULL) g_cnt_exposed_fallback++; else g_cnt_exposed++;
+  #endif
+        if(code != XC_FULL) {
+            check_exposed_decision(code, xc >> 8, ncand, uni(triv_q), uni(nv_q), jump_ratio);
+            if(ncand <= 1) { if(lane == 0) { HC.maybe_triv = 0; TRIV_CLEARED(); } wsync(); }
+            if(code == XC_NONE) return false;
+            xp = true; target = xc >> 8; last = (code == XC_BEST);
+        }
+    }
+#endif
+    if(!xp) {
+        if(lane == 0) { if(uni(hsd_q)) hs_refresh_flags(); HC.sw_vend = nv_q; HC.sw_best_r = DBL_MAX; HC.sw_best_v = -1; HC.sw_dom_base = -1; }
+        wsync();
+        if(skippable && !uni(HC.maybe_triv)) { check_no_trivial_candidate(); return false; }
+    }
     bool flag = false;
     int start = 1;
     for(;;) {
-        int target = -1; bool last = false;
-        while(start < uni(HC.sw_vend)) {
+        if(!xp) { target = -1; last = false; }
+        while(!xp && start < uni(HC.sw_vend)) {
             int code = uni(scan_trivial(start, mode, type, jump_ratio));
             PROF_ADD(PF_TRIV_EVAL);
             if(code == SC_NEED) {
@@ -2229,10 +2379,10 @@
         if(target < 0) {
             if(flag) return true;
             if(mode == 0) return false;
-            if(uni(HC.sw_best_v) < 0) { if(skippable) { if(lane == 0) HC.maybe_triv = 0; wsync(); } return false; }
+            if(uni(HC.sw_best_v) < 0) { if(skippable) { if(lane == 0) { HC.maybe_triv = 0; TRIV_CLEARED(); } wsync(); } return false; }
             target = uni(HC.sw_best_v); last = true;
 #ifndef ALD_NO_TRIV_CLEAR
-            if(skippable && uni(HC.sw_ncand) == 1) { if(lane == 0) HC.maybe_triv = 0; wsync(); }
+            if(skippable && uni(HC.sw_ncand) == 1) { if(lane == 0) { HC.maybe_triv = 0; TRIV_CLEARED(); } wsync(); }
 #endif
         }
         fired++;
@@ -2242,11 +2392,18 @@
         if(lane == 0) {
             if(uni(HC.hs_dirty)) hs_refresh_flags();
             HC.sw_dom_base = -1;
+            if(xp) { HC.sw_vend = HC.nv; HC.sw_best_r = DBL_MAX; HC.sw_best_v = -1; }
         }
         wsync();
         PROF_ADD(PF_TRIV_MUT);
         flag = true;
-        if(HC.status) return true;
+        if(xp) {
+            xp = false;
+            const int stq = HC.status, hsq = HC.hs_dirty, trq = HC.maybe_triv;
+            if(uni(stq)) return true;
+            if(!uni(hsq) && !uni(trq)) { check_no_trivial_candidate(); return true; }
+        }
+        else if(HC.status) return true;
         start = target + 1;
     }
 }
@@ -3350,7 +3507,7 @@
     int64_t ov = A->in.off_v[g], ovo = ov + g, oe = A->in.off_e[g], oeo = oe + g, os = A->in.off_s[g], op = A->in.off_p[g], opo = op + g, opv = A->in.off_pv[g];
     if(lane == 0) {
         HC.V0 = V; HC.gstrand = (int)(unsigned char)A->in.graph_strand[g];
-        HC.sinkp = V - 1; HC.special_linked = 0; HC.maybe_broken = 1; HC.maybe_triv = 1; ev_mark_all();
+        HC.sinkp = V - 1; HC.special_linked = 0; HC.maybe_broken = 1; HC.maybe_triv = TRIV_ALL; TRIV_WHY(4); ev_mark_all();
         HC.nv = V; HC.next_id = E; HC.slot_hw = E; HC.free_head = -1; HC.free_cnt = 0; HC.status = 0; HC.any_strand = 0; HC.hs_dirty = 1;
         HC.n_paths = 0; HC.n_iters = 0; HC.n_trace = 0; HC.sp_used = 0; HC.hl_used = 0; HC.hl_n = 0;
     }
```

Result: slower. 2.687 million (-2.0%).
